# AAPPHH/image_recommender

Hardware: AMD Instinct MI355X
Metric: k-NN queries/sec + recall@10 on 1M concat vectors at 1/2/4/8 MI355X (higher is better)
Workload: dtype bf16 candidates (fp32 accumulate) + fp32 rerank, certified exact; 1 GPU; cfg3: 1M x 1968 concat(color48|sift128|dreamsim1792), cosine ranking; rows=1000000, dim=1968, k=10, queries_per_batch=1024, rows_per_gpu=1000000, parallelism=row-shard x1 + RCCL all-gather merge, queries_per_gpu=1024, tile_rows=256, tile_queries=256, row_splits=64, workgroups=256

## Files before the change

### image_recommender_amd/_lib.py

```python
from __future__ import annotations

import ctypes as C
import os
import threading
from pathlib import Path

LIB_PATH = Path(__file__).resolve().parent / "lib" / os.environ.get("IMGREC_LIB_NAME", "libimgrec.so")

KNN_OK, KNN_EINVAL, KNN_EHIP, KNN_ENOMEM, KNN_EIO, KNN_ENOSYS = 0, -1, -2, -3, -4, -5
KNN_METRIC_IP, KNN_METRIC_L2, KNN_METRIC_COSINE = 0, 1, 2
KNN_MAX_K = 32
KNN_MAX_K_LARGE = 1024
KNN_SEARCH_AUTO, KNN_SEARCH_EXACT, KNN_SEARCH_SPLIT, KNN_SEARCH_BF16, KNN_SEARCH_I8 = 0, 1, 2, 3, 4
KNN_FENCE_EAGER, KNN_FENCE_LAZY = 0, 1
COLOR_HIST_MAX_BINS = 32
INGEST_NOT_FAST, INGEST_TOO_SMALL = -1, -2
KMEANS_SPHERICAL = 1
KMEANS_STATS_PER_ITER = 8
VLAD_RAW = 1
VLAD_MAX_NN = 8
VLAD_MAX_D = 16384
VLADENC_MODEL_OUTPUT = 1
VLADENC_MAX_LAYERS = 8
VLADENC_MAX_WIDTH = 4096
VLADENC_MAX_IN = 1 << 20
VLADENC_CHUNK_ROWS = 128
VLADENC_SUPER_ROWS = 2048
VLADTRAIN_MAX_BATCH = 4096
VLADTRAIN_MAX_BATCH_FLOATS = 1 << 28
VLADTRAIN_PARAMS, VLADTRAIN_ADAM_M, VLADTRAIN_ADAM_V, VLADTRAIN_GRADS = 0, 1, 2, 3


class KmeansParams(C.Structure):
    _fields_ = [("niter", C.c_int), ("nredo", C.c_int), ("spherical", C.c_int), ("verbose", C.c_int),
                ("seed", C.c_int64), ("device", C.c_int)]

class VladTrainConfig(C.Structure):
    _fields_ = [("dropout", C.c_double), ("lr", C.c_double), ("beta1", C.c_double), ("beta2", C.c_double),
                ("adam_eps", C.c_double), ("weight_decay", C.c_double), ("corr_weight", C.c_double),
                ("umap_weight", C.c_double), ("temperature", C.c_double), ("ln_eps", C.c_double),
                ("seed", C.c_uint64)]


_vp, _i, _i64, _f, _d = C.c_void_p, C.c_int, C.c_int64, C.c_float, C.c_double
_pi64, _pf, _pi, _pd = C.POINTER(C.c_int64), C.POINTER(C.c_float), C.POINTER(C.c_int), C.POINTER(C.c_double)
SIGNATURES = {
    "knn_create": (_i, [_i, _i, _i, C.POINTER(_vp)]),
    "knn_create_multi": (_i, [_i, _i, _pi, _i, C.POINTER(_vp)]),
    "knn_num_shards": (_i, [_vp]),
    "knn_free": (_i, [_vp]),
    "knn_dim": (_i, [_vp]),
    "knn_metric": (_i, [_vp]),
    "knn_ntotal": (_i64, [_vp]),
    "knn_is_trained": (_i, [_vp]),
    "knn_set_id_offset": (_i, [_vp, _i64]),
    "knn_train": (_i, [_vp, _vp, _i64]),
    "knn_add": (_i, [_vp, _vp, _i64]),
    "knn_add_device": (_i, [_vp, _vp, _i64, _vp]),
    "knn_reserve": (_i, [_vp, _i64]),
    "knn_reset": (_i, [_vp]),
    "knn_remove_ids": (_i, [_vp, _vp, _i64, _pi64]),
    "knn_reconstruct_n": (_i, [_vp, _i64, _i64, _vp]),
    "knn_search": (_i, [_vp, _vp, _i64, _i, _vp, _vp]),
    "knn_search_device": (_i, [_vp, _vp, _i64, _i, _vp, _vp, _vp]),
    "knn_search_filtered": (_i, [_vp, _vp, _i64, _i, _vp, _i64, _vp, _vp]),
    "knn_search_filtered_device": (_i, [_vp, _vp, _i64, _i, _vp, _i64, _vp, _vp, _vp]),
    "knn_range_search": (_i, [_vp, _vp, _i64, _f, C.POINTER(_vp)]),
    "knn_range_search_device": (_i, [_vp, _vp, _i64, _f, _vp, C.POINTER(_vp)]),
    "knn_range_nq": (_i64, [_vp]),
    "knn_range_size": (_i64, [_vp]),
    "knn_range_copy": (_i, [_vp, _vp, _vp, _vp]),
    "knn_range_device": (_i, [_vp, C.POINTER(_vp), C.POINTER(_vp), C.POINTER(_vp)]),
    "knn_range_free": (_i, [_vp]),
    "knn_merge_device": (_i, [_vp, _vp, _i, _i64, _i, _i, _i, _vp, _vp, _vp]),
    "knn_packed_bytes": (_i64, [_i64, _i]),
    "knn_merge_packed_device": (_i, [_vp, _i, _i64, _i, _i, _i, _vp, _vp, _vp]),
    "ivfpq_lut_device": (_i, [_vp, _i64, _i, _i, _i, _vp, _vp, _vp]),
    "ivfpq_scan_device": (_i, [_vp, _vp, _i64, _i, _vp, _vp, _vp, _i, _i, _i, _vp, _vp, _vp]),
    "ivfpq_scan_all_device": (_i, [_vp, _vp, _i64, _i, _vp, _vp, _vp, _i, _i, _vp, _vp, _i64, _i, _vp,
                                   _vp, _vp]),
    "knn_write": (_i, [_vp, C.c_char_p]),
    "knn_read": (_i, [C.c_char_p, _i, C.POINTER(_vp)]),
    "knn_read_multi": (_i, [C.c_char_p, _pi, _i, C.POINTER(_vp)]),
    "knn_normalize_L2": (_i, [_vp, _i64, _i]),
    "knn_set_timing": (_i, [_vp, _i]),
    "knn_set_fence_mode": (_i, [_vp, _i]),
    "knn_kernel_time": (_i, [_vp, _pd, _pi]),
    "knn_plan": (_i, [_vp, _i64, _i, _pi, _pi, _pi, _pi]),
    "knn_plan_kernel": (_i, [_vp, _i64, _i, C.c_char_p, _i]),
    "knn_set_search_mode": (_i, [_vp, _i]),
    "knn_search_stats": (_i, [_vp, _pi64, _pi64, _pf]),
    "knn_search_stats2": (_i, [_vp, _pi64, _pi64, _pi64, _pf]),
    "knn_last_path": (_i, [_vp]),
    "knn_debug_i8tail": (_i, [_vp, _pi, _pi, _i64, _i64, _vp, _vp, _vp]),
    "knn_large_k_fallbacks": (_i, [_vp, C.POINTER(_i64)]),
    "knn_last_error": (C.c_char_p, []),
    "knn_version": (C.c_char_p, []),
    "kmeans_step_device": (_i, [_vp, _i64, _i, _vp, _i, _i, _vp, _vp, _vp, _vp, _vp, _vp]),
    "kmeans_split_device": (_i, [_vp, _i, _i, _vp, _pi, _vp]),
    "kmeans_train": (_i, [_vp, _i64, _i, _i, _vp, _vp, _vp, _pd, _vp]),
    "kmeans_train_device": (_i, [_vp, _i64, _i, _i, _vp, _vp, _vp, _pd, _vp, _vp]),
    "vlad_encode_device": (_i, [_vp, _i64, _vp, _i64, _i, _vp, _i, _i, _f, _i, _vp, _vp, _vp, _vp]),
    "vlad_encode": (_i, [_vp, _i64, _vp, _i64, _i, _vp, _i, _i, _f, _i, _vp, _vp, _vp, _i]),
    "vladenc_create": (_i, [_i, _pi, C.POINTER(_vp), C.POINTER(_vp), C.POINTER(_vp), C.POINTER(_vp), _f, _i,
                            C.POINTER(_vp)]),
    "vladenc_free": (_i, [_vp]),
    "vladenc_widths": (_i, [_vp, _pi, _pi]),
    "vladenc_forward_device": (_i, [_vp, _vp, _i64, _i, _vp, _vp, _vp]),
    "vladenc_forward": (_i, [_vp, _vp, _i64, _i, _vp, _vp]),
    "vladtrain_default_config": (_i, [C.POINTER(VladTrainConfig)]),
    "vladtrain_create": (_i, [_i, _pi, C.POINTER(_vp), C.POINTER(_vp), C.POINTER(_vp), C.POINTER(_vp),
                              C.POINTER(VladTrainConfig), _i, C.POINTER(_vp)]),
    "vladtrain_free": (_i, [_vp]),
    "vladtrain_step_device": (_i, [_vp, _vp, _i64, _vp, _i64, _vp, _vp]),
    "vladtrain_step": (_i, [_vp, _vp, _i64, _vp, _i64, _vp]),
    "vladtrain_grads_device": (_i, [_vp, _vp, _i64, _vp, _i64, _vp, _vp, _vp, _vp]),
    "vladtrain_grads": (_i, [_vp, _vp, _i64, _vp, _i64, _vp, _vp, _vp]),
    "vladtrain_eval_device": (_i, [_vp, _vp, _i64, _vp, _i64, _vp, _vp]),
    "vladtrain_eval": (_i, [_vp, _vp, _i64, _vp, _i64, _vp]),
    "vladtrain_get_state": (_i, [_vp, _i, C.POINTER(_vp), C.POINTER(_vp), C.POINTER(_vp), C.POINTER(_vp)]),
    "vladtrain_set_state": (_i, [_vp, _i, C.POINTER(_vp), C.POINTER(_vp), C.POINTER(_vp), C.POINTER(_vp)]),
    "vladtrain_get_step": (_i, [_vp, _pi64]),
    "vladtrain_set_step": (_i, [_vp, _i64]),
    "vladtrain_product_device": (_i, [_vp, _i64, _vp, _i64, _i64, _vp, _vp]),
    "vladtrain_workspace_bytes": (_i64, [_i, _pi, _i64]),
    "color_hist_device": (_i, [_vp, _vp, _vp, _i64, _i, _vp, _vp, _vp]),
    "color_hist_host": (_i, [_vp, _i64, _vp, _vp, _i64, _i, _i, _vp, _vp]),
    "color_hist_last_error": (C.c_char_p, []),
    "color_host_register": (_i, [_vp, _i64]),
    "color_host_unregister": (_i, [_vp]),
    "vit_add_layernorm_bf16": (_i, [_vp, _vp, _vp, _vp, _vp, _i64, _i, C.c_float, _vp]),
    "vit_quick_gelu_bf16": (_i, [_vp, _i64, _vp]),
    "vit_gelu_bf16": (_i, [_vp, _i64, _vp]),
    "vit_patchify_bf16": (_i, [_vp, _i64, _i, _i, _i, _vp, _vp, _vp, _vp]),
    "vit_tokens_f32": (_i, [_vp, _vp, _vp, _i64, _i, _i, _vp, _vp]),
    "vit_attention_bf16": (_i, [_vp, _i64, _i, _i, _i, C.c_float, _vp, _vp]),
    "vit_linear_bf16": (_i, [_vp, _vp, _vp, _i64, _i, _i, _i, _vp, _vp]),
    "vit_linear_bf16_split": (_i, [_vp, _vp, _vp, _i64, _i, _i, _i, _i, _vp, _vp]),
    "vit_linear_splits": (_i, [_i64, _i]),
    "color_hist_batch_async": (_i, [_vp, _i64, _vp, _i64, _i, _vp, _vp, _vp, _vp, _vp]),
    "ingest_parse_f32": (_i64, [_vp, _i64, _vp, _i64]),
    "ingest_concat_rows": (_i64, [C.POINTER(_vp), _pi64, _i64, _i, _pi64, _vp, _vp]),
    "ingest_concat_packed": (_i64, [_vp, _vp, _vp, _i64, _i, _vp, _vp, _vp]),
    "ingest_scan_open": (_i, [C.c_char_p, C.c_char_p, _i, _pi64, C.POINTER(_vp)]),
    "ingest_scan_next": (_i64, [_vp, _i64, _vp, _vp, _vp]),
    "ingest_scan_close": (_i, [_vp]),
    "ingest_scan_error": (C.c_char_p, []),
}


class NativeLibraryError(RuntimeError):
    """libimgrec.so is missing or failed to load — the HIP path is mandatory."""


class KnnError(RuntimeError):
    """A C-ABI call returned an error code (the message is knn_last_error())."""


_lock = threading.Lock()
_lib = None


def load() -> C.CDLL:
    global _lib
    if _lib is not None:
        return _lib
    with _lock:
        if _lib is not None:
            return _lib
        if not LIB_PATH.exists():
            raise NativeLibraryError(
                f"{LIB_PATH} not found: build it with `python -m image_recommender_amd.build` "
                "(hipcc --offload-arch=gfx950); there is no CPU fallback")
        if os.environ.get("IMGREC_NO_TORCH_PRELOAD") != "1":
            try:
                import torch
            except Exception:
                pass
        try:
            lib = C.CDLL(str(LIB_PATH), mode=C.RTLD_GLOBAL)
        except OSError as e:
            raise NativeLibraryError(f"cannot load {LIB_PATH}: {e}") from e
        for name, (res, args) in SIGNATURES.items():
            fn = getattr(lib, name)
            fn.restype = res
            fn.argtypes = args
        _lib = lib
        return lib


def last_error() -> str:
    msg = load().knn_last_error()
    return msg.decode() if msg else ""


def check(rc: int, what: str) -> int:
    if rc < 0:
        raise KnnError(f"{what} failed (code {rc}): {last_error()}")
    return rc
```

### image_recommender_amd/csrc/knn_b16w.hip

```cpp

#include <hip/hip_runtime.h>
#include <stdint.h>
#include <math.h>

#include <type_traits>

#include "knn_kernels.h"
#include "lds_dma.h"
#include "wave_ops.h"

namespace imgrec {
namespace {

typedef float f32x4 __attribute__((ext_vector_type(4)));
typedef __bf16 bf16x8 __attribute__((ext_vector_type(8)));
typedef unsigned u32x4 __attribute__((ext_vector_type(4)));
typedef float f32x2 __attribute__((ext_vector_type(2)));
typedef int i32x4 __attribute__((ext_vector_type(4)));

constexpr int kNW = 8;
constexpr int kBM = kB16BigRows;
constexpr int kBQ = kB16BigQueries;
constexpr int kQW = kBQ / kNW;
constexpr int kRB = kBM / 16;
constexpr int kBKW = 32;
constexpr int kNS = 2;
constexpr int kRowB = kBKW * 4;
constexpr int kCPR = kBKW / 4;
constexpr int kRPP = 64 / kCPR;
constexpr int kRPB = 64 / kBKW;
constexpr int kGPT = kBM / kRPP;
constexpr int kSA = kBM * kRowB;
constexpr int kSB = kBQ * kRowB;
constexpr int kStage = kSA + kSB;
constexpr int kLPW = (kBM + kBQ) / kRPP / kNW;
constexpr int kNormSlots = 4;
constexpr int kNormOff = kNS * kStage;
constexpr int kRecOff = kNormOff + kNormSlots * kBM * 4;
constexpr int kLuOff = kRecOff + kNW * kQW * kSBWords * 4;
constexpr int kLDS = kLuOff + kBQ * 2 * 4;
static_assert(kQW * kSBWords * 4 == 2048 && kSBWords == 16, "a wave's records: one dma2_agent of 2 KiB");
static_assert(kLDS == 153600, "LDS image");
constexpr int kScaleOff = kLDS;
constexpr int kQScaleOff = kScaleOff + kNormSlots * kBM * 4;
constexpr int kQNormOff = kQScaleOff + kBQ * 4;
constexpr int kLDST = kQNormOff + kBQ * 4;
static_assert(kLDST <= 160 * 1024, "LDS budget (int8 tail)");
constexpr int kQuads = 8;
#ifndef IMGREC_B16W_DEFER_Q
#define IMGREC_B16W_DEFER_Q 3
#endif
constexpr int kDeferQ = IMGREC_B16W_DEFER_Q;
static_assert(kBKW == 32 && kCPR == 8, "stage depth: two 32-deep k-steps per stage");
static_assert(kLDS <= 160 * 1024, "LDS budget");
static_assert(kLPW % 4 == 0, "pieces go out in dma4x groups of four");
static_assert(kDeferQ >= 0 && kDeferQ < kQuads - 1, "deferred DMA inside the stage's first quads");
#ifndef IMGREC_B16W_EPI_EXP
#define IMGREC_B16W_EPI_EXP 0
#endif

template <int K>
__device__ __forceinline__ void insert_mono(float (&kd)[K], int (&ki)[K], float d, int id) {
    bool c[K];
#pragma unroll
    for (int p = 0; p < K; ++p) c[p] = d < kd[p];
#pragma unroll
    for (int p = K - 1; p > 0; --p) {
        kd[p] = __builtin_amdgcn_fmed3f(kd[p - 1], d, kd[p]);
        const int nx = __builtin_unpredictable(c[p]) ? id : ki[p];
        ki[p] = __builtin_unpredictable(c[p - 1]) ? ki[p - 1] : nx;
    }
    kd[0] = __builtin_unpredictable(c[0]) ? d : kd[0];
    ki[0] = __builtin_unpredictable(c[0]) ? id : ki[0];
}

__device__ __forceinline__ bool rank_lt(float d1, int i1, float d2, int i2) {
    return i2 < 0 || d1 < d2 || (d1 == d2 && i1 < i2);
}

template <int K>
__device__ __forceinline__ void insert_any(float (&kd)[K], int (&ki)[K], float d, int id) {
#pragma unroll
    for (int p = K - 1; p > 0; --p) {
        const bool shift = rank_lt(d, id, kd[p - 1], ki[p - 1]);
        const bool here = !shift && rank_lt(d, id, kd[p], ki[p]);
        kd[p] = shift ? kd[p - 1] : (here ? d : kd[p]);
        ki[p] = shift ? ki[p - 1] : (here ? id : ki[p]);
    }
    const bool here0 = rank_lt(d, id, kd[0], ki[0]);
    kd[0] = here0 ? d : kd[0];
    ki[0] = here0 ? id : ki[0];
}

__device__ __forceinline__ float quarter_min(float x) {
    const auto r = __builtin_amdgcn_permlane16_swap(__float_as_uint(x), __float_as_uint(x), false, false);
    x = fminf(__uint_as_float(r[0]), __uint_as_float(r[1]));
    const auto s = __builtin_amdgcn_permlane32_swap(__float_as_uint(x), __float_as_uint(x), false, false);
    return fminf(__uint_as_float(s[0]), __uint_as_float(s[1]));
}
__device__ __forceinline__ float quarter_max(float x) {
    const auto r = __builtin_amdgcn_permlane16_swap(__float_as_uint(x), __float_as_uint(x), false, false);
    x = fmaxf(__uint_as_float(r[0]), __uint_as_float(r[1]));
    const auto s = __builtin_amdgcn_permlane32_swap(__float_as_uint(x), __float_as_uint(x), false, false);
    return fmaxf(__uint_as_float(s[0]), __uint_as_float(s[1]));
}

__device__ __forceinline__ uint32_t quarter_min_u(uint32_t x) {
    const auto r = __builtin_amdgcn_permlane16_swap(x, x, false, false);
    x = min(r[0], r[1]);
    const auto s = __builtin_amdgcn_permlane32_swap(x, x, false, false);
    return min(s[0], s[1]);
}
__device__ __forceinline__ uint32_t quarter_max_u(uint32_t x) {
    const auto r = __builtin_amdgcn_permlane16_swap(x, x, false, false);
    x = max(r[0], r[1]);
    const auto s = __builtin_amdgcn_permlane32_swap(x, x, false, false);
    return max(s[0], s[1]);
}

__device__ __forceinline__ uint32_t ord_bits(float k) {
    const uint32_t u = __float_as_uint(k);
    return (u & 0x80000000u) ? ~u : (u | 0x80000000u);
}
__device__ __forceinline__ float ord_float(uint32_t u) {
    return __uint_as_float((u & 0x80000000u) ? (u & 0x7fffffffu) : ~u);
}
__device__ __forceinline__ float sel8(int r, float x0, float x1, float x2, float x3, float x4, float x5,
                                      float x6, float x7) {
    const bool b0 = r & 1, b1 = r & 2, b2 = r & 4;
    const float a0 = b0 ? x1 : x0, a1 = b0 ? x3 : x2, a2 = b0 ? x5 : x4, a3 = b0 ? x7 : x6;
    const float c0 = b1 ? a1 : a0, c1 = b1 ? a3 : a2;
    return b2 ? c1 : c0;
}
__device__ __forceinline__ uint32_t umed3(uint32_t a, uint32_t b, uint32_t c) {
    return max(min(a, b), min(max(a, b), c));
}
template <int K>
__device__ __forceinline__ void insert_packed(uint32_t (&kp)[K], uint32_t u) {
#pragma unroll
    for (int p = K - 1; p > 0; --p) kp[p] = umed3(kp[p - 1], u, kp[p]);
    kp[0] = min(kp[0], u);
}
__device__ __forceinline__ float bucket_end(uint32_t u, uint32_t lowmask) {
    return u == ~0u ? INFINITY : ord_float((u | lowmask) + 1u);
}

}

#ifdef IMGREC_B16_STAMPS
__device__ unsigned long long g_b16w_stamps[8 * 256];
__device__ unsigned long long g_b16w_wg[2 * 1024];
#define B16W_STAMP(slot) do { if (stamp_on && lane == 0) { \
    unsigned long long v_ = __builtin_amdgcn_s_memtime(); g_b16w_stamps[wave * 256 + (slot)] = v_; } } while (0)
#else
#define B16W_STAMP(slot) do {} while (0)
#endif

struct I8TailArgs {
    const uint32_t* xt = nullptr;
    const float* xts = nullptr;
    const uint32_t* qt = nullptr;
    const float* qts = nullptr;
    int dwt = 0, nst_t = 0, nst_h = 0;
};

template <int KM, int L2, bool PACK>
__global__ void __launch_bounds__(512, 2)
knn_b16w_tile_kernel(const uint32_t* __restrict__ xh, const float* __restrict__ xnorm, int nrows,
                     int dw, const uint32_t* __restrict__ qh, const float* __restrict__ qnorm, int nq,
                     int nsplit, int nqb, int64_t id_offset, float* __restrict__ cand_d,
                     int64_t* __restrict__ cand_i, int ncand, int ib, uint32_t* sbound) {
    __shared__ __attribute__((aligned(16))) char smem[kLDS];
#define B16W_I8T 0
#include "knn_b16w_body.inc"
#undef B16W_I8T
}

template <int KM, int L2, bool PACK>
__global__ void __launch_bounds__(512, 2)
knn_b16w_tile_kernel_i8t(const uint32_t* __restrict__ xh, const float* __restrict__ xnorm, int nrows,
                         int dw, const uint32_t* __restrict__ qh, const float* __restrict__ qnorm, int nq,
                         int nsplit, int nqb, int64_t id_offset, float* __restrict__ cand_d,
                         int64_t* __restrict__ cand_i, int ncand, int ib, uint32_t* sbound,
                         const I8TailArgs ta) {
    __shared__ __attribute__((aligned(16))) char smem[kLDST];
#define B16W_I8T 1
    constexpr bool I8T = true;
#include "knn_b16w_body.inc"
#undef B16W_I8T
}

hipError_t launch_b16_big(const TileArgs& a, hipStream_t st) {
    if (a.wr != 2 || a.wq != 4 || a.dp % kBKW != 0 || a.nsplit < 1) return hipErrorInvalidValue;
    const auto off_ok = [&](int64_t row_bytes) {
        return ((int64_t)(kGPT - 1) * a.nsplit * kRPP + kBQ) * row_bytes + 8192 < ((int64_t)1 << 32);
    };
    if (!off_ok((int64_t)a.dp * 4)) return hipErrorInvalidValue;
    const bool i8t = a.xt != nullptr;
    I8TailArgs ta;
    if (i8t) {
        if (a.t_head < 0 || a.t_head % 64 != 0 || a.t_head > 2 * a.dp || a.t_dpt < 128 || a.t_dpt % 128 != 0 ||
            !a.xts || !a.qt || !a.qts || !off_ok(a.t_dpt))
            return hipErrorInvalidValue;
        ta.xt = reinterpret_cast<const uint32_t*>(a.xt);
        ta.xts = a.xts;
        ta.qt = reinterpret_cast<const uint32_t*>(a.qt);
        ta.qts = a.qts;
        ta.dwt = a.t_dpt / 4;
        ta.nst_t = a.t_dpt / 128;
        ta.nst_h = a.t_head / 64;
    }
    const dim3 grid((unsigned)(a.nqb * a.nsplit)), block(kNW * 64);
    const uint32_t* xh = reinterpret_cast<const uint32_t*>(a.xb);
    const uint32_t* qh = reinterpret_cast<const uint32_t*>(a.qp);
    if (a.ib < 0 || a.ib > kB16PackMaxIB) return hipErrorInvalidValue;
#define IMGREC_LAUNCH_B16W(KMV, L2V, PK)                                                             \
    do {                                                                                             \
        if (i8t)                                                                                     \
            hipLaunchKernelGGL((knn_b16w_tile_kernel_i8t<KMV, L2V, PK>), grid, block, 0, st, xh,    \
                               a.xnorm, a.nrows, a.dp, qh, a.qnorm, a.nq, a.nsplit, a.nqb,           \
                               a.id_offset, a.cand_d, a.cand_i, a.ncand, a.ib, a.sbound, ta);        \
        else                                                                                         \
            hipLaunchKernelGGL((knn_b16w_tile_kernel<KMV, L2V, PK>), grid, block, 0, st, xh,        \
                               a.xnorm, a.nrows, a.dp, qh, a.qnorm, a.nq, a.nsplit, a.nqb,           \
                               a.id_offset, a.cand_d, a.cand_i, a.ncand, a.ib, a.sbound);            \
    } while (0)
#define IMGREC_LAUNCH_B16W_K(KMV, PK)                                                               \
    do { if (a.metric == 1) IMGREC_LAUNCH_B16W(KMV, 1, PK); else IMGREC_LAUNCH_B16W(KMV, 0, PK); } while (0)
    if (a.km == 8) {
        if (a.ib > 0) IMGREC_LAUNCH_B16W_K(8, true); else IMGREC_LAUNCH_B16W_K(8, false);
    } else if (a.km == 10) {
        if (a.ib > 0) IMGREC_LAUNCH_B16W_K(10, true); else IMGREC_LAUNCH_B16W_K(10, false);
    } else {
        return hipErrorInvalidValue;
    }
#undef IMGREC_LAUNCH_B16W_K
#undef IMGREC_LAUNCH_B16W
    return hipGetLastError();
}

}


#ifdef IMGREC_B16_STAMPS
extern "C" int knn_b16w_stamps_read(unsigned long long* host) {
    return (int)hipMemcpyFromSymbol(host, HIP_SYMBOL(imgrec::g_b16w_stamps), sizeof(imgrec::g_b16w_stamps));
}
extern "C" int knn_b16w_wg_read(unsigned long long* host) {
    return (int)hipMemcpyFromSymbol(host, HIP_SYMBOL(imgrec::g_b16w_wg), sizeof(imgrec::g_b16w_wg));
}
#endif
```

### image_recommender_amd/csrc/knn_b16w_body.inc

```
#if B16W_I8T
#else

#endif
#ifdef IMGREC_B16_STAMPS
    const int wg = blockIdx.x;
    if (threadIdx.x == 0 && wg < 1024) g_b16w_wg[2 * wg] = __builtin_amdgcn_s_memrealtime();
#endif
    const int wgid = xcd_wgid();
    constexpr int kG = 4;
    const int G = (nqb % kG == 0) ? kG : nqb;
    const int qbg = wgid / (nsplit * G), rem = wgid - qbg * (nsplit * G);
    const int split = rem / G;
    const int qb = qbg * G + rem % G;
    const int ngroups = (nrows + kRPP - 1) / kRPP;
    const int cnt = split < ngroups ? (ngroups - split + nsplit - 1) / nsplit : 0;
    const int t0 = 0, t1 = (cnt + kGPT - 1) / kGPT;
    auto trow = [&](int t, int tr) {
        const int m = t * kGPT + tr / kRPP;
        return (split + (m < cnt ? m : t * kGPT) * nsplit) * kRPP + tr % kRPP;
    };

    const int lane = threadIdx.x & 63;
    const int wave = __builtin_amdgcn_readfirstlane(threadIdx.x >> 6);
    const int lc = lane & 15, lq = lane >> 4;
    int qcol[2];
    qcol[0] = qb * kBQ + wave * kQW + lc;
    qcol[1] = qcol[0] + 16;
#if B16W_I8T
    auto qcol_of = [&](int h) __attribute__((always_inline)) {
        if constexpr (!I8T) return qcol[h];
        int l = lc;
        asm volatile("" : "+v"(l));
        return qb * kBQ + wave * kQW + l + 16 * h;
    };
#endif
    float qn[2] = {0.f, 0.f};
#if B16W_I8T
    if constexpr (!I8T) {
        if (L2) { qn[0] = qnorm[qcol[0]]; qn[1] = qnorm[qcol[1]]; }
        asm volatile("" : "+v"(qn[0]), "+v"(qn[1]));
    }
    float* const lsq = reinterpret_cast<float*>(smem + (I8T ? kQScaleOff : 0)) + wave * kQW;
    float* const lqn = reinterpret_cast<float*>(smem + (I8T ? kQNormOff : 0)) + wave * kQW;
    if constexpr (I8T)
        if (lane < kQW) {
            lsq[lane] = ta.qts[qb * kBQ + wave * kQW + lane];
            lqn[lane] = L2 ? qnorm[qb * kBQ + wave * kQW + lane] : 0.f;
        }
#else
    if (L2) { qn[0] = qnorm[qcol[0]]; qn[1] = qnorm[qcol[1]]; }
    asm volatile("" : "+v"(qn[0]), "+v"(qn[1]));
#endif

    const bool isA = wave < 4;
    if (!isA) __builtin_amdgcn_s_setprio(1);
    const int pbase = (isA ? wave : wave - 4) * kLPW;
    const int prow = lane / kCPR, pchk = lane % kCPR;
    static_assert(kRPP == 8 && kRPB == 2 && kLPW % 2 == 0, "piece offset form");
#if B16W_I8T
    auto vpar_of = [&](int e, int words) {
        int ln = lane;
        asm volatile("" : "+v"(ln));
        const int prow = ln / kCPR, pchk = ln % kCPR;
#else
    uint32_t vpar[2];
#pragma unroll
    for (int e = 0; e < 2; ++e) {
#endif
        const int P = pbase + e, r = P * kRPP + prow;
        const int srow = isA ? P * nsplit * kRPP + prow : r;
#if B16W_I8T
        return (uint32_t)srow * (uint32_t)(words * 4) + 16u * (uint32_t)(pchk ^ ((r / kRPB) % kCPR));
    };
    uint32_t vpar[2] = {0u, 0u};
    if constexpr (!I8T) { vpar[0] = vpar_of(0, dw); vpar[1] = vpar_of(1, dw); }
#else
        vpar[e] = (uint32_t)srow * (uint32_t)(dw * 4) + 16u * (uint32_t)(pchk ^ ((r / kRPB) % kCPR));
    }
#endif
    const uint32_t kPS = (uint32_t)((isA ? nsplit : 1) * kRPP * dw * 4);
    auto voff_of = [&](int j) {
        return vpar[j & 1] + (uint32_t)(j & ~1) * kPS - 1024u * (uint32_t)(j & 3);
    };
    const uint32_t smem0 = lds_u32(smem);
    const uint32_t pdst = (uint32_t)((isA ? 0 : kSA) + pbase * 1024);

    const int fsw = (lc / kRPB) % kCPR;
    int aoff[2];
#pragma unroll
    for (int c = 0; c < 2; ++c) aoff[c] = lc * kRowB + 16 * ((4 * c + lq) ^ fsw);
    const int boff = kSA + wave * kQW * kRowB;

    float kd[2][KM];
    int ki[2][KM];
    uint32_t kp[2][KM];
    const uint32_t lowm = PACK ? (1u << ib) - 1u : 0u;
#pragma unroll
    for (int h = 0; h < 2; ++h)
#pragma unroll
        for (int p = 0; p < KM; ++p) {
            if constexpr (PACK) kp[h][p] = ~0u;
            else { kd[h][p] = INFINITY; ki[h][p] = -1; }
        }

    const bool sb_on = sbound != nullptr;
    uint32_t* const wrec = sbound + (size_t)(qb * kBQ + wave * kQW) * kSBWords;
    const uint32_t* const lrec = reinterpret_cast<const uint32_t*>(smem + kRecOff) + wave * (kQW * kSBWords);
    uint2* const lst = reinterpret_cast<uint2*>(smem + kLuOff) + wave * kQW;
    if (sb_on && lq == 0) {
        lst[lc] = make_uint2(__float_as_uint(INFINITY), ~0u);
        lst[lc + 16] = make_uint2(__float_as_uint(INFINITY), ~0u);
    }
    auto rec_dma = [&]() __attribute__((always_inline)) {
        dma2_agent(wrec, smem0 + (uint32_t)(kRecOff + wave * (kQW * kSBWords * 4)), (uint32_t)lane * 16u);
    };

#if B16W_I8T
    const int nst_t = I8T ? ta.nst_t : 0;
    const int nst = I8T ? ta.nst_t + ta.nst_h : dw / kBKW;
#else
    const int nst = dw / kBKW;
#endif
    const int total = (t1 - t0) * nst;
    const uint32_t* qblk = qh + (size_t)qb * kBQ * dw;
#if B16W_I8T
    const uint32_t* qblk_t = I8T ? ta.qt + (size_t)qb * kBQ * ta.dwt : nullptr;
#endif

    int c_it = t0, c_is = 0;
    const uint32_t* c_tile = isA ? xh + (size_t)trow(t0, 0) * dw : qblk;
#if B16W_I8T
    const uint32_t* c_tile_t = !I8T ? nullptr : isA ? ta.xt + (size_t)trow(t0, 0) * ta.dwt : qblk_t;
#endif
    int c_ng = (isA && t0 == t1 - 1) ? cnt - t0 * kGPT : kGPT;
    auto issue = [&](int g) __attribute__((always_inline)) {
#if B16W_I8T
        const bool tl = I8T && c_is < nst_t;
        const uint32_t* src;
        uint32_t vp0 = 0u, vp1 = 0u, ps = 0u;
        if constexpr (I8T) {
            const int rw = tl ? ta.dwt : dw;
            src = tl ? c_tile_t + c_is * kBKW : c_tile + (c_is - nst_t) * kBKW;
            vp0 = vpar_of(0, rw);
            vp1 = vpar_of(1, rw);
            ps = (uint32_t)((isA ? nsplit : 1) * kRPP * rw * 4);
        } else {
            src = c_tile + c_is * kBKW;
        }
        auto voff = [&](int j) {
            if constexpr (I8T) return ((j & 1) ? vp1 : vp0) + (uint32_t)(j & ~1) * ps - 1024u * (uint32_t)(j & 3);
            else return voff_of(j);
        };
#else
        const uint32_t* src = c_tile + c_is * kBKW;
#endif
        const uint32_t dst = smem0 + (uint32_t)((g & (kNS - 1)) * kStage) + pdst;
        if (pbase + kLPW <= c_ng || !isA) {
#pragma unroll
            for (int h = 0; h < kLPW / 4; ++h)
#if B16W_I8T
                dma4x(src, dst + 4096u * h, voff(4 * h), voff(4 * h + 1), voff(4 * h + 2),
                      voff(4 * h + 3));
#else
                dma4x(src, dst + 4096u * h, voff_of(4 * h), voff_of(4 * h + 1), voff_of(4 * h + 2),
                      voff_of(4 * h + 3));
#endif
        } else {
#pragma unroll
            for (int j = 0; j < kLPW; ++j)
                if (pbase + j < c_ng) {
                    const uint32_t d = dst + 4096u * (j / 4);
                    switch (j & 3) {
#if B16W_I8T
                        case 0: dma1<0>(src, d, voff(j)); break;
                        case 1: dma1<1024>(src, d, voff(j)); break;
                        case 2: dma1<2048>(src, d, voff(j)); break;
                        default: dma1<3072>(src, d, voff(j)); break;
#else
                        case 0: dma1<0>(src, d, voff_of(j)); break;
                        case 1: dma1<1024>(src, d, voff_of(j)); break;
                        case 2: dma1<2048>(src, d, voff_of(j)); break;
                        default: dma1<3072>(src, d, voff_of(j)); break;
#endif
                    }
                }
        }
        if (c_is == 0 && wave < 4)
            dma4_norm(xnorm + trow(c_it, wave * 64 + lane),
                      smem0 + (uint32_t)(kNormOff + ((c_it - t0) & (kNormSlots - 1)) * kBM * 4 + wave * 256));
#if B16W_I8T
        if constexpr (I8T)
            if (c_is == 0 && wave < 4)
                dma4_norm(ta.xts + trow(c_it, wave * 64 + lane),
                          smem0 + (uint32_t)(kScaleOff + ((c_it - t0) & (kNormSlots - 1)) * kBM * 4 + wave * 256));
#endif
        if (++c_is == nst) {
            c_is = 0;
            ++c_it;
            if (isA) {
                c_tile = xh + (size_t)trow(c_it, 0) * dw;
#if B16W_I8T
                if constexpr (I8T) c_tile_t = ta.xt + (size_t)trow(c_it, 0) * ta.dwt;
#endif
                c_ng = c_it == t1 - 1 ? cnt - c_it * kGPT : kGPT;
            }
        }
    };
    static_assert(kNS == 2 && kNormSlots == 4, "power-of-two ring slots");

    constexpr int kJ = (KM + 3) / 4;
    constexpr float kLo = 1.0f / 1048576.f;

    auto read_a = [&](const char* sb, int q, u32x4 (&fa)[4]) __attribute__((always_inline)) {
#pragma unroll
        for (int j = 0; j < 4; ++j)
            fa[j] = *reinterpret_cast<const u32x4*>(sb + aoff[q >> 2] + (4 * (q & 3) + j) * 16 * kRowB);
    };
    auto read_b = [&](const char* sb, int c, u32x4 (&fb)[2]) __attribute__((always_inline)) {
#pragma unroll
        for (int h = 0; h < 2; ++h) fb[h] = *reinterpret_cast<const u32x4*>(sb + aoff[c] + boff + h * 16 * kRowB);
    };
#if B16W_I8T
    auto mfma_quad = [&](auto tl_tag, f32x4 (&acc)[kRB][2], const u32x4 (&fa)[4], const u32x4 (&fb)[2], int q) __attribute__((always_inline)) {
#else
    auto mfma_quad = [&](f32x4 (&acc)[kRB][2], const u32x4 (&fa)[4], const u32x4 (&fb)[2], int q) __attribute__((always_inline)) {
#endif
#pragma unroll
        for (int j = 0; j < 4; ++j)
#pragma unroll
#if B16W_I8T
            for (int h = 0; h < 2; ++h) {
                if constexpr (decltype(tl_tag)::value)
                    acc[4 * (q & 3) + j][h] = __builtin_bit_cast(f32x4, __builtin_amdgcn_mfma_i32_16x16x64_i8(
                        __builtin_bit_cast(i32x4, fa[j]), __builtin_bit_cast(i32x4, fb[h]),
                        __builtin_bit_cast(i32x4, acc[4 * (q & 3) + j][h]), 0, 0, 0));
                else
                    acc[4 * (q & 3) + j][h] = __builtin_amdgcn_mfma_f32_16x16x32_bf16(
                        __builtin_bit_cast(bf16x8, fa[j]), __builtin_bit_cast(bf16x8, fb[h]), acc[4 * (q & 3) + j][h], 0, 0, 0);
            }
#else
            for (int h = 0; h < 2; ++h)
                acc[4 * (q & 3) + j][h] = __builtin_amdgcn_mfma_f32_16x16x32_bf16(
                    __builtin_bit_cast(bf16x8, fa[j]), __builtin_bit_cast(bf16x8, fb[h]), acc[4 * (q & 3) + j][h], 0, 0, 0);
#endif
    };

    u32x4 fa[2][4], fb[2][2];
    int g = 0;
    int pend = -1;
    if (total > 0) {
        issue(0);
        asm volatile("s_waitcnt vmcnt(0)" ::: "memory");
        barrier_lds();
        if (total > 1) issue(1);
        read_a(smem, 0, fa[0]);
        read_b(smem, 0, fb[0]);
    }
    for (int t = t0; t < t1; ++t) {
#ifdef IMGREC_B16_STAMPS
        const bool stamp_on = blockIdx.x == 100 && t - t0 < 120;
        int nit = 0;
        unsigned long long ins_cyc = 0;
#endif
        f32x4 acc[kRB][2];
#pragma unroll
        for (int rb = 0; rb < kRB; ++rb)
#pragma unroll
            for (int h = 0; h < 2; ++h) acc[rb][h] = (f32x4){0.f, 0.f, 0.f, 0.f};
        const bool rec_due = sb_on && (t - t0 < 4 || ((t - t0) & 3) == 0);
        const int nlive = (t + 1) * kGPT <= cnt ? 4 : (((cnt - t * kGPT) * kRPP + 63) >> 6);
#if B16W_I8T
        auto stage_loop = [&](auto nr_tag, auto tl_tag, int ns, int s0, bool more) __attribute__((always_inline)) {
#else
        auto stage_loop = [&](auto nr_tag) __attribute__((always_inline)) {
#endif
            constexpr int NR = decltype(nr_tag)::value, L = 2 * NR;
#if B16W_I8T
            for (int s = 0; s < ns; ++s, ++g) {
#else
            for (int s = 0; s < nst; ++s, ++g) {
#endif
                const char* sb = smem + (g & 1) * kStage;
#pragma unroll
                for (int i = 0; i + 1 < L; ++i) {
                    read_a(sb, 4 * ((i + 1) / NR) + (i + 1) % NR, fa[(i + 1) & 1]);
                    if (i == NR - 1) read_b(sb, 1, fb[1]);
#if B16W_I8T
                    mfma_quad(tl_tag, acc, fa[i & 1], fb[i / NR], 4 * (i / NR) + i % NR);
#else
                    mfma_quad(acc, fa[i & 1], fb[i / NR], 4 * (i / NR) + i % NR);
#endif
#pragma unroll
                    for (int j = 0; j < 4; ++j) {
                        __builtin_amdgcn_sched_group_barrier(0x008, 1, 0);
                        __builtin_amdgcn_sched_group_barrier(0x100, 1, 0);
                    }
                    if (i == NR - 1) {
                        __builtin_amdgcn_sched_group_barrier(0x008, 1, 0);
                        __builtin_amdgcn_sched_group_barrier(0x100, 1, 0);
                        __builtin_amdgcn_sched_group_barrier(0x008, 1, 0);
                        __builtin_amdgcn_sched_group_barrier(0x100, 1, 0);
                        __builtin_amdgcn_sched_group_barrier(0x008, 2, 0);
                    } else {
                        __builtin_amdgcn_sched_group_barrier(0x008, 4, 0);
                    }
                    __builtin_amdgcn_sched_barrier(0);
                    if (i == (kDeferQ < L - 2 ? kDeferQ : L - 2) && pend >= 0) {
                        __builtin_amdgcn_sched_barrier(0);
                        issue(pend);
                        pend = -1;
                        __builtin_amdgcn_sched_barrier(0);
                    }
                }
                __builtin_amdgcn_sched_barrier(0);
                asm volatile("s_waitcnt vmcnt(0) lgkmcnt(0)" ::: "memory");
                __builtin_amdgcn_sched_barrier(0);
                barrier_lds();
                __builtin_amdgcn_sched_barrier(0);
#if B16W_I8T
                if (s + 1 < ns || more) {
#else
                if (s + 1 < nst) {
#endif
                    const char* nb = smem + ((g + 1) & 1) * kStage;
                    read_a(nb, 0, fa[0]);
                    read_b(nb, 0, fb[0]);
                }
                if (g + 2 < total) {
                    if (isA) issue(g + 2);
                    else pend = g + 2;
                }
#if B16W_I8T
                if (rec_due && s0 + s + 2 == nst) rec_dma();
                mfma_quad(tl_tag, acc, fa[1], fb[1], 4 + NR - 1);
            }
        };
        auto tile_stages = [&](auto nr_tag) __attribute__((always_inline)) {
            if constexpr (I8T) {
                constexpr int NR = decltype(nr_tag)::value;
                stage_loop(nr_tag, std::true_type{}, nst_t, 0, nst > nst_t);
                const float* scl = reinterpret_cast<const float*>(smem + kScaleOff + ((t - t0) % kNormSlots) * kBM * 4);
                const float sq[2] = {lsq[lc], lsq[lc + 16]};
#pragma unroll
                for (int rb = 0; rb < (IMGREC_B16W_EPI_EXP == 3 ? 0 : 4 * NR); ++rb) {
                    const float4 s4 = *reinterpret_cast<const float4*>(scl + rb * 16 + 4 * lq);
                    const float sr[4] = {s4.x, s4.y, s4.z, s4.w};
#pragma unroll
                    for (int h = 0; h < 2; ++h) {
                        const i32x4 ai = __builtin_bit_cast(i32x4, acc[rb][h]);
#pragma unroll
                        for (int i = 0; i < 4; ++i) acc[rb][h][i] = (float)ai[i] * sr[i] * sq[h];
                    }
                    asm volatile("" : "+v"(acc[rb][0]), "+v"(acc[rb][1]));
                }
                stage_loop(nr_tag, std::false_type{}, nst - nst_t, nst_t, false);
            } else {
                stage_loop(nr_tag, std::false_type{}, nst, 0, false);
#else
                if (rec_due && s + 2 == nst) rec_dma();
                mfma_quad(acc, fa[1], fb[1], 4 + NR - 1);
#endif
            }
        };
        if (rec_due && nst < 2) rec_dma();
#if B16W_I8T
        if (nlive >= 4) tile_stages(std::integral_constant<int, 4>{});
        else if (nlive == 3) tile_stages(std::integral_constant<int, 3>{});
        else if (nlive == 2) tile_stages(std::integral_constant<int, 2>{});
        else tile_stages(std::integral_constant<int, 1>{});
#else
        if (nlive >= 4) stage_loop(std::integral_constant<int, 4>{});
        else if (nlive == 3) stage_loop(std::integral_constant<int, 3>{});
        else if (nlive == 2) stage_loop(std::integral_constant<int, 2>{});
        else stage_loop(std::integral_constant<int, 1>{});
#endif

        B16W_STAMP(2 * (t - t0));
#if IMGREC_B16W_EPI_EXP != 0
#pragma unroll
        for (int rb = 0; rb < kRB; ++rb)
#pragma unroll
            for (int h = 0; h < 2; ++h) asm volatile("" :: "v"(acc[rb][h]));
#endif
        const float* nrm = reinterpret_cast<const float*>(smem + kNormOff + ((t - t0) % kNormSlots) * kBM * 4);
        const bool full = (t + 1) * kGPT <= cnt && trow(t, kBM - 1) < nrows;
        auto row_ok = [&](int tr) { return t * kGPT + tr / kRPP < cnt && trow(t, tr) < nrows; };
#if B16W_I8T
        if constexpr (I8T && L2 != 0) { qn[0] = lqn[lc]; qn[1] = lqn[lc + 16]; }
#endif
        float lu[2] = {INFINITY, INFINITY};
        if (sb_on) {
#pragma unroll
            for (int h = 0; h < 2; ++h) {
                const uint4 c = *reinterpret_cast<const uint4*>(lrec + (lc + 16 * h) * kSBWords + 4 * lq);
                const uint32_t ub = quarter_max_u(lq < 3 ? max(max(c.x, c.y), max(c.z, c.w)) : 0u);
                const float cA = __uint_as_float(quarter_max_u(lq == 3 ? c.x : 0u));
                const float cB = __uint_as_float(quarter_max_u(lq == 3 ? c.y : 0u));
                const float U = ord_float(ub);
                const float L = ub >= 0xff800000u ? INFINITY : U + fmaf(cB, fabsf(U), cA);
                lu[h] = fminf(__uint_as_float(lst[lc + 16 * h].x), L);
            }
        }
        float cth[2];
        auto screen = [&]() __attribute__((always_inline)) {
#pragma unroll
            for (int h = 0; h < 2; ++h) {
                float T;
                if constexpr (PACK) T = bucket_end(min(quarter_min_u(kp[h][KM - 1]), quarter_max_u(kp[h][kJ - 1])), lowm);
                else T = fminf(quarter_min(kd[h][KM - 1]), quarter_max(kd[h][kJ - 1]));
                T = fminf(T, lu[h]);
                const float c = L2 ? 0.5f * (qn[h] - T) - kLo * (qn[h] + fabsf(T)) : -T;
#if B16W_I8T
                cth[h] = qcol_of(h) < nq ? c : INFINITY;
#else
                cth[h] = qcol[h] < nq ? c : INFINITY;
#endif
            }
        };
#pragma unroll
        for (int rg = 0; rg < 4; ++rg) {
            if (rg >= nlive || IMGREC_B16W_EPI_EXP == 1) break;
            screen();
            unsigned live = 0xffffu;
            if (!full) {
                live = 0;
#if B16W_I8T
                int lq_c = lq;
                asm volatile("" : "+v"(lq_c));
#pragma unroll
                for (int b = 0; b < 16; ++b) live |= (unsigned)row_ok((4 * rg + (b >> 2)) * 16 + 4 * lq_c + (b & 3)) << b;
#else
#pragma unroll
                for (int b = 0; b < 16; ++b) live |= (unsigned)row_ok((4 * rg + (b >> 2)) * 16 + 4 * lq + (b & 3)) << b;
#endif
            }
            unsigned msk[2] = {0u, 0u};
            float4 nr4[4];
#pragma unroll
            for (int j = 3; j >= 0; --j) {
                const int rb = 4 * rg + j;
                float4 n4 = make_float4(0.f, 0.f, 0.f, 0.f);
                if (L2) n4 = *reinterpret_cast<const float4*>(nrm + rb * 16 + 4 * lq);
                nr4[j] = n4;
                const f32x2 half2 = (f32x2){0.5f - kLo, 0.5f - kLo};
                const f32x2 hlo = (f32x2){n4.x, n4.y} * half2, hhi = (f32x2){n4.z, n4.w} * half2;
#pragma unroll
                for (int h = 0; h < 2; ++h) {
                    const f32x2 c2 = (f32x2){cth[h], cth[h]};
                    const f32x2 dhi = (L2 ? hhi + c2 : c2) - (f32x2){acc[rb][h][2], acc[rb][h][3]};
                    const f32x2 dlo = (L2 ? hlo + c2 : c2) - (f32x2){acc[rb][h][0], acc[rb][h][1]};
                    msk[h] = __builtin_amdgcn_alignbit(msk[h], __float_as_uint(dhi.y), 31);
                    msk[h] = __builtin_amdgcn_alignbit(msk[h], __float_as_uint(dhi.x), 31);
                    msk[h] = __builtin_amdgcn_alignbit(msk[h], __float_as_uint(dlo.y), 31);
                    msk[h] = __builtin_amdgcn_alignbit(msk[h], __float_as_uint(dlo.x), 31);
                }
            }
#ifdef IMGREC_B16_STAMPS
            const unsigned long long ins0 = __builtin_amdgcn_s_memtime();
#endif
#if IMGREC_B16W_EPI_EXP == 2
            asm volatile("" :: "v"(msk[0] & live), "v"(msk[1] & live));
            continue;
#endif
#pragma unroll
            for (int h = 0; h < 2; ++h) {
                const unsigned m = msk[h] & live;
                if (!__any(m != 0)) continue;
#pragma unroll
                for (int hf = 0; hf < 2; ++hf) {
                    unsigned mh = (m >> (8 * hf)) & 0xffu;
                    if (!__any(mh != 0)) continue;
                    const int rb0 = 4 * rg + 2 * hf;
                    while (__any(mh != 0)) {
#ifdef IMGREC_B16_STAMPS
                        ++nit;
#endif
                        const bool act = mh != 0u;
                        const int r8 = act ? __builtin_ctz(mh) : 0;
                        mh &= mh - 1u;
                        const int tr = (rb0 + (r8 >> 2)) * 16 + 4 * lq + (r8 & 3);
                        const float a = sel8(r8, acc[rb0][h][0], acc[rb0][h][1], acc[rb0][h][2], acc[rb0][h][3],
                                             acc[rb0 + 1][h][0], acc[rb0 + 1][h][1], acc[rb0 + 1][h][2],
                                             acc[rb0 + 1][h][3]);
                        const float4 na = nr4[2 * hf], nb = nr4[2 * hf + 1];
                        const float xn = L2 ? sel8(r8, na.x, na.y, na.z, na.w, nb.x, nb.y, nb.z, nb.w) : 0.f;
                        float kv = L2 ? fmaf(-2.f, a, qn[h] + xn) : -a;
                        if constexpr (PACK) {
                            const uint32_t ob = L2 ? ((uint32_t)max((int)__float_as_uint(kv), 0) | 0x80000000u)
                                                   : ord_bits(kv);
                            const uint32_t u = (ob & ~lowm) | (uint32_t)(t * kBM + tr);
                            insert_packed<KM>(kp[h], __builtin_unpredictable(act) ? u : ~0u);
                        } else {
                            if (L2) kv = kv < 0.f ? 0.f : kv;
                            kv = __builtin_unpredictable(act && kv < kd[h][KM - 1]) ? kv : INFINITY;
                            insert_mono<KM>(kd[h], ki[h], kv, trow(t, tr));
                        }
                    }
                }
            }
#ifdef IMGREC_B16_STAMPS
            ins_cyc += __builtin_amdgcn_s_memtime() - ins0;
#endif
        }
        if (sb_on) {
#pragma unroll
            for (int h = 0; h < 2; ++h) {
                const uint32_t best = quarter_min_u(PACK ? kp[h][0] : ord_bits(kd[h][0]));
                uint32_t pubd = lst[lc + 16 * h].y;
                const uint32_t pub = PACK ? (best | lowm) + 1u : best;
                if (lq == 0) {
#if B16W_I8T
                    const int qc = qcol_of(h);
                    if (qc < nq && pub != 0u && pub < 0xff800000u && pub < pubd) {
                        __hip_atomic_fetch_min(sbound + (size_t)qc * kSBWords + split % KM, pub,
#else
                    if (qcol[h] < nq && pub != 0u && pub < 0xff800000u && pub < pubd) {
                        __hip_atomic_fetch_min(sbound + (size_t)qcol[h] * kSBWords + split % KM, pub,
#endif
                                               __ATOMIC_RELAXED, __HIP_MEMORY_SCOPE_AGENT);
                        pubd = pub;
                    }
                    lst[lc + 16 * h] = make_uint2(__float_as_uint(lu[h]), pubd);
                }
            }
        }
        B16W_STAMP(2 * (t - t0) + 1);
#ifdef IMGREC_B16_STAMPS
        if (stamp_on && lane == 0) g_b16w_stamps[wave * 256 + 128 + (t - t0)] = (unsigned long long)nit;
        if (stamp_on && lane == 0 && t - t0 < 64) g_b16w_stamps[wave * 256 + 192 + (t - t0)] = ins_cyc;
#endif
        if (g < total) {
            read_a(smem + (g & 1) * kStage, 0, fa[0]);
            read_b(smem + (g & 1) * kStage, 0, fb[0]);
        }
    }

#ifdef IMGREC_B16_STAMPS
    if (threadIdx.x == 0 && wg < 1024) g_b16w_wg[2 * wg + 1] = __builtin_amdgcn_s_memrealtime();
#endif
#pragma unroll
    for (int x = 32; x >= 16; x >>= 1) {
#pragma unroll
        for (int h = 0; h < 2; ++h) {
            if constexpr (PACK) {
                uint32_t o[KM];
#pragma unroll
                for (int p = 0; p < KM; ++p) o[p] = (uint32_t)__shfl_xor((int)kp[h][p], x, 64);
#pragma unroll
                for (int p = 0; p < KM; ++p) insert_packed<KM>(kp[h], o[p]);
                continue;
            }
#pragma unroll
            for (int p = 0; p < KM; ++p) {
                const float od = __shfl_xor(kd[h][p], x, 64);
                const int oi = __shfl_xor(ki[h][p], x, 64);
                if (lq < x / 16 && oi >= 0 && rank_lt(od, oi, kd[h][KM - 1], ki[h][KM - 1]))
                    insert_any<KM>(kd[h], ki[h], od, oi);
            }
        }
    }
    if (lq != 0) return;
    const float lu[2] = {sb_on ? __uint_as_float(lst[lc].x) : INFINITY, sb_on ? __uint_as_float(lst[lc + 16].x) : INFINITY};
#pragma unroll
    for (int h = 0; h < 2; ++h) {
#if B16W_I8T
        const int qc = qcol_of(h);
        if (qc >= nq) continue;
#else
        if (qcol[h] >= nq) continue;
#endif
        if (sb_on && lu[h] != INFINITY)
#if B16W_I8T
            __hip_atomic_fetch_min(sbound + (size_t)qc * kSBWords + kSBFloor, ord_bits(lu[h]),
#else
            __hip_atomic_fetch_min(sbound + (size_t)qcol[h] * kSBWords + kSBFloor, ord_bits(lu[h]),
#endif
                                   __ATOMIC_RELAXED, __HIP_MEMORY_SCOPE_AGENT);
#if B16W_I8T
        const size_t base = (size_t)qc * ncand + (size_t)split * KM;
#else
        const size_t base = (size_t)qcol[h] * ncand + (size_t)split * KM;
#endif
#pragma unroll
        for (int p = 0; p < KM; ++p) {
            if constexpr (PACK) {
                const uint32_t u = kp[h][p];
                const int j = (int)(u & lowm);
                cand_d[base + p] = u == ~0u ? INFINITY : ord_float(u & ~lowm);
                cand_i[base + p] = u == ~0u ? (int64_t)-1
                                            : (int64_t)((split + (j >> 3) * nsplit) * kRPP + (j & 7)) + id_offset;
            } else {
                cand_d[base + p] = kd[h][p];
                cand_i[base + p] = ki[h][p] < 0 ? (int64_t)-1 : (int64_t)ki[h][p] + id_offset;
            }
        }
    }
```

### image_recommender_amd/csrc/knn_capi.cpp

```cpp

#include <cstdarg>
#include <cstdio>
#include <cstdlib>
#include <cstring>
#include <mutex>
#include <string>

#include "knn_index.h"
#include "knn_multi.h"

namespace imgrec {

namespace {
thread_local std::string g_err;
}

const char* test_knob(const char* name) {
    const char* e = std::getenv(name);
    if (e && *e) {
        static std::mutex mu;
        static std::string seen;
        std::lock_guard<std::mutex> lk(mu);
        const std::string tag = std::string("|") + name + "|";
        if (seen.find(tag) == std::string::npos) {
            seen += tag;
            std::fprintf(stderr, "[imgrec] %s=%s overrides a launch default (test / A-B knob, "
                                 "INTEGRATION.md)\n", name, e);
        }
    }
    return e && *e ? e : nullptr;
}

void set_err(const char* fmt, ...) {
    char buf[512];
    va_list ap;
    va_start(ap, fmt);
    vsnprintf(buf, sizeof(buf), fmt, ap);
    va_end(ap);
    g_err = buf;
}

const char* last_error() { return g_err.c_str(); }

int corpus_columns(knn_index* ix, Column<DeviceSpace>* cols, bool all) {
    int n = 0;
    cols[n++] = {&ix->xb, (size_t)ix->dp * sizeof(float)};
    cols[n++] = {&ix->xn, sizeof(float)};
    if (all || ix->xs) cols[n++] = {&ix->xs, (size_t)ix->dp * sizeof(uint32_t)};
    if (all || ix->b16_ok) cols[n++] = {&ix->xh, (size_t)ix->dpb * sizeof(uint16_t)};
    if (all || ix->b16_ok) cols[n++] = {&ix->xr, sizeof(float)};
    if (all || ix->x8) cols[n++] = {&ix->x8, (size_t)i8_row_bytes(ix->nblk8)};
    if (all || ix->x8) cols[n++] = {&ix->x8s, (size_t)ix->nblk8 * sizeof(float)};
    if (all || ix->x8) cols[n++] = {&ix->x8r, sizeof(float)};
    if (all || ix->xt) cols[n++] = {&ix->xt, (size_t)ix->xt_dpt};
    if (all || ix->xt) cols[n++] = {&ix->xts, sizeof(float)};
    if (all || ix->xt) cols[n++] = {&ix->xtm, sizeof(float4)};
    return n;
}

int reserve_rows(knn_index* ix, int64_t need, hipStream_t st) {
    if (need <= ix->cap) return KNN_OK;
    const int64_t ncap = round_up(std::max(need, ix->cap + ix->cap / 2), kTileRowsMax);
    Column<DeviceSpace> live[kCorpusColumns];
    const int n_all = corpus_columns(ix, live);
    const int n_tail = ix->xt ? 3 : 0, n = n_all - n_tail;
    const size_t old = (size_t)ix->ntotal;
    hipError_t e = hipSuccess;
    const Column<DeviceSpace>* grp = live;
    auto fill_rows = [&](int i, void* dst, const void* src) {
        const size_t row = grp[i].stride;
        if (old && src) e = hipMemcpyAsync(dst, src, old * row, hipMemcpyDeviceToDevice, st);
        if (e == hipSuccess) e = hipMemsetAsync((char*)dst + old * row, 0, ((size_t)ncap - old) * row, st);
        return e == hipSuccess ? KNN_OK : KNN_EHIP;
    };
    auto wait_rows = [&]() {
        const hipError_t es = hipStreamSynchronize(st);
        if (e == hipSuccess) e = es;
        return e == hipSuccess ? KNN_OK : KNN_EHIP;
    };
    const int rc = regrow_columns(live, n, (size_t)ncap, fill_rows, wait_rows);
    if (rc != KNN_OK && e == hipSuccess) {
        (void)hipGetLastError();
        KNN_FAIL(KNN_ENOMEM, "hipMalloc of the %lld-row corpus buffers failed", (long long)ncap);
    }
    if (rc != KNN_OK) KNN_FAIL(KNN_EHIP, "corpus regrowth failed: %s", hipGetErrorString(e));
    ix->cap = ncap;
    if (n_tail > 0) {
        grp = live + n;
        if (regrow_columns(grp, n_tail, (size_t)ncap, fill_rows, wait_rows) != KNN_OK) {
            (void)hipGetLastError();
            drop_i8tail(ix, TailCopy::Undecided);
        }
    }
    return KNN_OK;
}

static int materialise_columns(knn_index* ix, int c0, int n) {
    Column<DeviceSpace> all[kCorpusColumns];
    corpus_columns(ix, all, true);
    const int rc = regrow_columns(all + c0, n, (size_t)std::max<int64_t>(ix->cap, 1),
                                  [](int, void*, const void*) { return KNN_OK; }, []() { return KNN_OK; });
    if (rc != KNN_OK) (void)hipGetLastError();
    return rc;
}

int add_device_locked(knn_index* ix, const float* x, int64_t n, hipStream_t st) {
    if ((int64_t)(ix->ntotal + n) > (int64_t)INT32_MAX)
        KNN_FAIL(KNN_EINVAL, "a single index shard holds at most 2^31-1 rows");
    int rc = reserve_rows(ix, ix->ntotal + n, st);
    if (rc != KNN_OK) return rc;
    Column<DeviceSpace> c[kCorpusColumns];
    corpus_columns(ix, c, true);
    auto at = [&](int col) { return (char*)c[col].buf->data() + (size_t)ix->ntotal * c[col].stride; };
    float* const xb = (float*)at(kColXb);
    KNN_HIP(launch_rows_ingest(x, n, ix->d, ix->dp, n, ix->metric == KNN_METRIC_COSINE ? 1 : 0, xb,
                               (float*)at(kColXn), st));
    if (ix->xs) KNN_HIP(launch_split_rows(xb, n, ix->dp, kSplitBK, (uint32_t*)at(kColXs), st));
    if (ix->b16_ok)
        KNN_HIP(launch_bf16_rows(xb, n, ix->dp, ix->dpb, (uint16_t*)at(kColXh), (float*)at(kColXr), st));
    if (ix->x8)
        KNN_HIP(launch_i8_rows(xb, n, ix->dp, ix->nblk8, (int8_t*)at(kColX8), (float*)at(kColX8s),
                               (float*)at(kColX8r), st));
    if (ix->xt) {
        KNN_HIP(launch_i8tail_rows(xb, n, ix->dp, ix->dpb, ix->xt_head, ix->xt_dpt, (int8_t*)at(kColXt),
                                   (float*)at(kColXts), (float4*)at(kColXtm), st));
        ix->xt_tried = false;
    }
    ix->ntotal += n;
    ix->xn_max_stale = true;
    return KNN_OK;
}

int ensure_split(knn_index* ix, hipStream_t st) {
    if (ix->xs) return KNN_OK;
    if (!ix->split_ok) KNN_FAIL(KNN_EINVAL, "split search needs d >= 256; d = %d", ix->d);
    if (materialise_columns(ix, kColXs, 1) != KNN_OK)
        KNN_FAIL(KNN_ENOMEM, "hipMalloc of the %lld-row split copy failed", (long long)ix->cap);
    if (ix->ntotal > 0)
        KNN_HIP(launch_split_rows(ix->xb, ix->ntotal, ix->dp, kSplitBK, ix->xs, st));
    return KNN_OK;
}

int ensure_i8(knn_index* ix, hipStream_t st) {
    if (ix->x8) return KNN_OK;
    if (ix->nblk8 <= 0) KNN_FAIL(KNN_EINVAL, "int8 search needs 64 <= d <= 4096; d = %d", ix->d);
    if (materialise_columns(ix, kColX8, 3) != KNN_OK)
        KNN_FAIL(KNN_ENOMEM, "hipMalloc of the %lld-row int8 copy failed", (long long)ix->cap);
    ix->xn_max_stale = true;
    if (ix->ntotal > 0)
        KNN_HIP(launch_i8_rows(ix->xb, ix->ntotal, ix->dp, ix->nblk8, ix->x8, ix->x8s, ix->x8r, st));
    return KNN_OK;
}

int ensure_i8tail(knn_index* ix, hipStream_t st) {
    if (ix->xt_state != TailCopy::Undecided) return KNN_OK;
    if (ix->ntotal <= 0 || !ix->b16_ok || ix->dpb > 4096) { ix->xt_state = TailCopy::Ineligible; return KNN_OK; }
    const int nblk = ix->dpb / kB16Pad;
    DevBuf<float> dmax;
    int rc;
    if ((rc = dmax.reserve((size_t)nblk)) != KNN_OK) return rc;
    std::vector<float> hmax((size_t)nblk);
    KNN_HIP(launch_block_absmax(ix->xb, ix->ntotal, ix->dp, nblk, dmax, st));
    KNN_HIP(hipMemcpyAsync(hmax.data(), dmax, (size_t)nblk * sizeof(float), hipMemcpyDeviceToHost, st));
    KNN_HIP(hipStreamSynchronize(st));
    const int head = i8t_pick_head(hmax.data(), nblk);
    if (head < 0) { ix->xt_state = TailCopy::Ineligible; return KNN_OK; }
    ix->xt_head = head;
    ix->xt_dpt = (int)round_up(ix->dpb - head, 128);
    if (materialise_columns(ix, kColXt, 3) != KNN_OK) {
        drop_i8tail(ix, TailCopy::Ineligible);
        return KNN_OK;
    }
    KNN_HIP(hipMemsetAsync(ix->xt, 0, (size_t)ix->cap * ix->xt_dpt, st));
    KNN_HIP(hipMemsetAsync(ix->xts, 0, (size_t)ix->cap * sizeof(float), st));
    KNN_HIP(hipMemsetAsync(ix->xtm, 0, (size_t)ix->cap * sizeof(float4), st));
    ix->xn_max_stale = true;
    KNN_HIP(launch_i8tail_rows(ix->xb, ix->ntotal, ix->dp, ix->dpb, head, ix->xt_dpt, ix->xt, ix->xts,
                               ix->xtm, st));
    ix->xt_state = TailCopy::Built;
    return KNN_OK;
}

void drop_i8tail(knn_index* ix, TailCopy next) {
    ix->xt.reset(); ix->xts.reset(); ix->xtm.reset();
    ix->xt_head = ix->xt_dpt = 0;
    ix->xt_tried = false; ix->xt_state = next;
}

int create_single(int d, int metric, int device, knn_index** out) {
    *out = nullptr;
    int ndev = 0;
    if (hipGetDeviceCount(&ndev) != hipSuccess || ndev <= 0)
        KNN_FAIL(KNN_ENOSYS, "no HIP device visible");
    if (device < 0) KNN_HIP(hipGetDevice(&device));
    if (device >= ndev) KNN_FAIL(KNN_EINVAL, "device %d out of range (%d visible)", device, ndev);
    DeviceGuard g(device);
    knn_index* ix = new knn_index();
    ix->d = d;
    ix->dp = (int)round_up(d, d >= 256 ? 2 * kDepthPad : kDepthPad);
    ix->metric = metric;
    ix->device = device;
    ix->split_ok = ix->dp % 32 == 0 && d >= 256;
    ix->b16_ok = d >= 64;
    ix->dpb = (int)round_up(d, kB16Pad);
    ix->nblk8 = d >= 64 && d <= 4096 ? (d + 63) / 64 : 0;
    int cus = 0;
    if (hipDeviceGetAttribute(&cus, hipDeviceAttributeMultiprocessorCount, device) == hipSuccess &&
        cus > 0)
        ix->cus = cus;
    if (const char* e = test_knob("IMGREC_CUS")) {
        const int v = std::atoi(e);
        if (v > 0 && v < ix->cus) ix->cus = v;
    }
    if (const char* e = test_knob("IMGREC_I8_WGPCU")) {
        const int v = std::atoi(e);
        if (v > 0 && v <= 16) ix->i8_wgpcu = v;
    }
    if (const char* e = test_knob("IMGREC_MERGE_FUSE")) {
        ix->merge_fuse = *e != '0';
        ix->merge_fuse1 = *e != '0' && *e != '1';
    }
    if (const char* e = test_knob("IMGREC_CHANCE_SKIP")) ix->chance_skip = *e != '0';
    if (const char* e = test_knob("IMGREC_CHANCE_DIRECT")) ix->chance_direct_max = std::max(0, std::atoi(e));
    if (const char* e = test_knob("IMGREC_I8_HALF_K")) {
        const int v = std::atoi(e);
        ix->i8_half_k = v >= 2 ? v : 0;
    }
    if (const char* e = test_knob("IMGREC_I8_POOL")) {
        ix->i8_pool64 = std::min(64, std::max(0, std::atoi(e)));
        ix->i8_pool_forced = true;
    }
    if (const char* e = test_knob("IMGREC_I8_POOL_CH")) ix->i8_pool_ch = std::min(64, std::max(1, std::atoi(e)));
    if (const char* e = test_knob("IMGREC_DIRECT_RAW")) ix->direct_raw = std::min(2, std::max(0, std::atoi(e)));
    if (const char* e = test_knob("IMGREC_I8_FUSED_PREP")) ix->i8_fused_prep = *e != '0';
    if (const char* e = test_knob("IMGREC_RERANK_P1")) ix->rerank_p1k = *e != '0';
    if (const char* e = test_knob("IMGREC_RERANK_NW4")) ix->rerank_nw4 = *e != '0';
    if (const char* e = test_knob("IMGREC_MERGE_SINGLE")) ix->merge_single = *e != '0';
    if (const char* e = test_knob("IMGREC_STREAM_LISTS")) ix->stream_lists = *e != '0';
    if (const char* e = test_knob("IMGREC_B16W_SHARED_BOUND")) ix->shared_bound = *e != '0';
    if (const char* e = test_knob("IMGREC_B16W_I8TAIL")) {
        ix->i8tail = *e != '0';
        ix->xt_no_trial = *e == '2';
    }
    if (const char* e = test_knob("IMGREC_RANGE_CAP")) {
        const long long v = std::atoll(e);
        if (v > 0) ix->range_cap0 = (size_t)v;
    }
    if (const char* e = test_knob("IMGREC_REMOVE_CHUNK")) {
        const long long v = std::atoll(e);
        if (v > 0) ix->remove_chunk = (int64_t)v;
    }
    if (hipStreamCreateWithFlags(&ix->stream, hipStreamNonBlocking) != hipSuccess ||
        ix->fence.create() != KNN_OK) {
        if (ix->stream) (void)hipStreamDestroy(ix->stream);
        delete ix;
        KNN_FAIL(KNN_EHIP, "hipStreamCreate / hipEventCreate failed");
    }
    *out = ix;
    return KNN_OK;
}

void free_single(knn_index* ix) {
    DeviceGuard g(ix->device);
    (void)hipDeviceSynchronize();
    for (hipEvent_t e : ix->ev) (void)hipEventDestroy(e);
    (void)hipStreamDestroy(ix->stream);
    delete ix;
}

constexpr size_t kPinnedSearchBytes = 1 << 20;

int stage_queries(knn_index* ix, const float* q, int64_t nq, int k, bool pinned) {
    int rc;
    const size_t nqd = (size_t)nq * ix->d, nk = (size_t)nq * k;
    if ((rc = ix->hq.reserve(nqd)) != KNN_OK) return rc;
    if (k > 0 && (rc = ix->hd.reserve(nk)) != KNN_OK) return rc;
    if (k > 0 && (rc = ix->hi.reserve(nk)) != KNN_OK) return rc;
    if (pinned) {
        if ((rc = ix->pq.reserve(nqd)) != KNN_OK) return rc;
        if ((rc = ix->pd.reserve(nk)) != KNN_OK) return rc;
        if ((rc = ix->pi.reserve(nk)) != KNN_OK) return rc;
        std::memcpy(ix->pq, q, nqd * sizeof(float));
    }
    KNN_HIP(hipMemcpyAsync(ix->hq, pinned ? ix->pq : q, nqd * sizeof(float), hipMemcpyHostToDevice, ix->stream));
    return KNN_OK;
}

int stage_bitmap(knn_index* ix, const uint8_t* bitmap, int64_t* nbits) {
    *nbits = std::min(*nbits, ix->ntotal);
    const size_t nbytes = (size_t)((*nbits + 7) / 8);
    const int rc = ix->ft_bits.reserve(std::max<size_t>(nbytes, 1));
    if (rc != KNN_OK) return rc;
    if (nbytes) KNN_HIP(hipMemcpyAsync(ix->ft_bits, bitmap, nbytes, hipMemcpyHostToDevice, ix->stream));
    return KNN_OK;
}

int fetch_results(knn_index* ix, int64_t nq, int k, float* D, int64_t* I) {
    const size_t nk = (size_t)nq * k;
    KNN_HIP(hipMemcpyAsync(D, ix->hd, nk * sizeof(float), hipMemcpyDeviceToHost, ix->stream));
    KNN_HIP(hipMemcpyAsync(I, ix->hi, nk * sizeof(int64_t), hipMemcpyDeviceToHost, ix->stream));
    return KNN_OK;
}

int set_metric(knn_index* ix, int metric) {
    if (ix->multi) return multi_set_metric(ix, metric);
    ix->metric = metric;
    return KNN_OK;
}

int set_trained(knn_index* ix, bool trained) {
    ix->trained = trained;
    if (ix->multi) return multi_set_trained(ix, trained);
    return KNN_OK;
}

}

using namespace imgrec;

extern "C" {

const char* knn_last_error(void) { return imgrec::last_error(); }
const char* knn_version(void) {
    return "imgrec-knn 0.2 (gfx950: bf16 / split-bf16 / f32 MFMA candidates, fused top-k, "
           "device-side certificate)";
}

int knn_create(int d, int metric, int device, knn_index_t** out) {
    if (!out) KNN_FAIL(KNN_EINVAL, "out is NULL");
    *out = nullptr;
    if (d <= 0) KNN_FAIL(KNN_EINVAL, "d must be positive (got %d)", d);
    if (metric != KNN_METRIC_L2 && metric != KNN_METRIC_IP && metric != KNN_METRIC_COSINE)
        KNN_FAIL(KNN_EINVAL, "unknown metric %d", metric);
    return create_single(d, metric, device, out);
}

int knn_free(knn_index_t* ix) {
    if (!ix) return KNN_OK;
    if (ix->multi) return multi_free(ix);
    free_single(ix);
    return KNN_OK;
}

int knn_dim(const knn_index_t* ix) { return ix ? ix->d : KNN_EINVAL; }
int knn_metric(const knn_index_t* ix) { return ix ? ix->metric : KNN_EINVAL; }
int64_t knn_ntotal(const knn_index_t* ix) { return ix ? ix->ntotal : KNN_EINVAL; }
int knn_is_trained(const knn_index_t* ix) { return ix ? (ix->trained ? 1 : 0) : KNN_EINVAL; }

int knn_set_id_offset(knn_index_t* ix, int64_t off) {
    if (!ix) KNN_FAIL(KNN_EINVAL, "index is NULL");
    std::lock_guard<std::mutex> lk(ix->mu);
    ix->id_offset = off;
    return KNN_OK;
}

int knn_train(knn_index_t* ix, const float* x, int64_t n) {
    (void)x;
    if (!ix) KNN_FAIL(KNN_EINVAL, "index is NULL");
    if (n < 0) KNN_FAIL(KNN_EINVAL, "n must be >= 0");
    return set_trained(ix, true);
}

int knn_reserve(knn_index_t* ix, int64_t n) {
    if (!ix) KNN_FAIL(KNN_EINVAL, "index is NULL");
    if (ix->multi) return multi_reserve(ix, n);
    IndexOp op(ix);
    int rc = op.begin(ix->stream);
    if (rc == KNN_OK) rc = reserve_rows(ix, n, ix->stream);
    return op.finish(rc);
}

static int add_args_ok(knn_index_t* ix, const float* x, int64_t n) {
    if (!ix) KNN_FAIL(KNN_EINVAL, "index is NULL");
    if (n < 0 || (n > 0 && !x)) KNN_FAIL(KNN_EINVAL, "bad rows (n=%lld)", (long long)n);
    return KNN_OK;
}

int knn_add_device(knn_index_t* ix, const float* x, int64_t n, void* stream) {
    int rc;
    if ((rc = add_args_ok(ix, x, n)) != KNN_OK || n == 0) return rc;
    if (ix->multi) return multi_add_device(ix, x, n, (hipStream_t)stream);
    IndexOp op(ix);
    if ((rc = op.begin((hipStream_t)stream)) == KNN_OK) rc = add_device_locked(ix, x, n, op.stream());
    return op.finish(rc);
}

int knn_add(knn_index_t* ix, const float* x, int64_t n) {
    int rc;
    if ((rc = add_args_ok(ix, x, n)) != KNN_OK || n == 0) return rc;
    if (ix->multi) return multi_add(ix, x, n);
    IndexOp op(ix);
    if ((rc = op.begin_host()) != KNN_OK) return rc;
    if ((rc = reserve_rows(ix, ix->ntotal + n, ix->stream)) != KNN_OK) return rc;
    const int64_t chunk = std::max<int64_t>(1, (int64_t)(64 << 20) / ((int64_t)ix->d * 4));
    for (int64_t r0 = 0; r0 < n; r0 += chunk) {
        const int64_t cn = std::min(chunk, n - r0);
// ... 224 lines not shown
                                 (hipStream_t)stream));
        return KNN_OK;
    }
    KNN_HIP(launch_merge_strided(cD, cI, nq, nlists, kin, kin, nf + 2 * n, nf / 2 + n, k, kmetric,
                                 kmetric ? 0 : 1, D, I, (hipStream_t)stream));
    return KNN_OK;
}

int knn_set_timing(knn_index_t* ix, int enable) {
    if (!ix) KNN_FAIL(KNN_EINVAL, "index is NULL");
    if (ix->multi) return multi_set_timing(ix, enable);
    IndexOp op(ix);
    ix->timing = enable != 0;
    ix->ev_used = 0;
    return KNN_OK;
}

int knn_set_fence_mode(knn_index_t* ix, int mode) {
    if (!ix) KNN_FAIL(KNN_EINVAL, "index is NULL");
    if (mode != KNN_FENCE_EAGER && mode != KNN_FENCE_LAZY) KNN_FAIL(KNN_EINVAL, "unknown fence mode %d", mode);
    std::lock_guard<std::mutex> lk(ix->mu);
    if (ix->multi) {
        int rc = multi_set_fence_mode(ix, mode);
        if (rc != KNN_OK) return rc;
    }
    ix->fence.lazy = mode == KNN_FENCE_LAZY;
    return KNN_OK;
}

int knn_kernel_time(knn_index_t* ix, double* total_ms, int* launches) {
    if (!ix || !total_ms || !launches) KNN_FAIL(KNN_EINVAL, "NULL argument");
    if (ix->multi) return multi_kernel_time(ix, total_ms, launches);
    IndexOp op(ix);
    double tot = 0.0;
    for (size_t i = 0; i + 1 < ix->ev_used; i += 2) {
        KNN_HIP(hipEventSynchronize(ix->ev[i + 1]));
        float ms = 0.f;
        KNN_HIP(hipEventElapsedTime(&ms, ix->ev[i], ix->ev[i + 1]));
        tot += ms;
    }
    *total_ms = tot;
    *launches = (int)(ix->ev_used / 2);
    ix->ev_used = 0;
    return KNN_OK;
}

int knn_set_search_mode(knn_index_t* ix, int mode) {
    if (!ix) KNN_FAIL(KNN_EINVAL, "index is NULL");
    if (mode != KNN_SEARCH_AUTO && mode != KNN_SEARCH_EXACT && mode != KNN_SEARCH_SPLIT &&
        mode != KNN_SEARCH_BF16 && mode != KNN_SEARCH_I8)
        KNN_FAIL(KNN_EINVAL, "unknown search mode %d", mode);
    if (ix->multi) return multi_set_search_mode(ix, mode);
    std::lock_guard<std::mutex> lk(ix->mu);
    if (mode == KNN_SEARCH_SPLIT && !ix->split_ok)
        KNN_FAIL(KNN_EINVAL, "split search needs d >= 256; d = %d", ix->d);
    if (mode == KNN_SEARCH_BF16 && !ix->b16_ok)
        KNN_FAIL(KNN_EINVAL, "bf16 search needs d >= 64; d = %d", ix->d);
    if (mode == KNN_SEARCH_I8 && ix->nblk8 <= 0)
        KNN_FAIL(KNN_EINVAL, "int8 search needs 64 <= d <= 4096; d = %d", ix->d);
    ix->mode = mode;
    return KNN_OK;
}

int knn_search_stats(knn_index_t* ix, int64_t* split_queries, int64_t* fallback_queries,
                     float* max_err_ratio) {
    return knn_search_stats2(ix, split_queries, fallback_queries, nullptr, max_err_ratio);
}

int knn_search_stats2(knn_index_t* ix, int64_t* split_queries, int64_t* fallback_queries,
                      int64_t* second_chance_queries, float* max_err_ratio) {
    if (!ix || !split_queries || !fallback_queries) KNN_FAIL(KNN_EINVAL, "NULL argument");
    if (ix->multi)
        return multi_search_stats(ix, split_queries, fallback_queries, second_chance_queries,
                                  max_err_ratio);
    IndexOp op(ix);
    int64_t first_fail = 0;
    *fallback_queries = 0;
    int rc = ix->stat_valid ? op.begin_host() : KNN_OK;
    if (rc == KNN_OK) rc = read_search_stats(ix, split_queries, fallback_queries, &first_fail, max_err_ratio);
    if (second_chance_queries) *second_chance_queries = first_fail - *fallback_queries;
    return op.finish_synced(rc);
}

int knn_last_path(const knn_index_t* ix) {
    if (!ix) return KNN_EINVAL;
    return ix->multi ? multi_last_path(ix) : ix->last_path;
}

static int large_k_fallbacks_one(knn_index* ix, int64_t* n) {
    IndexOp op(ix);
    int rc = ix->lk_fail ? op.begin_host() : KNN_OK;
    if (rc == KNN_OK) rc = largek_fallbacks(ix, n);
    return op.finish_synced(rc);
}

int knn_large_k_fallbacks(const knn_index_t* cix, int64_t* n) {
    if (!cix || !n) KNN_FAIL(KNN_EINVAL, "NULL argument");
    knn_index* ix = const_cast<knn_index*>(cix);
    if (!ix->multi) return large_k_fallbacks_one(ix, n);
    *n = 0;
    for (int s = 0; s < multi_num_shards(ix); ++s) {
        int64_t v = 0;
        const int rc = large_k_fallbacks_one(const_cast<knn_index*>(multi_shard(ix, s)), &v);
        if (rc != KNN_OK) return rc;
        *n += v;
    }
    return KNN_OK;
}

static_assert((int)Route::Exact == kModeF32 && (int)Route::Split == kModeSplit && (int)Route::B16 == kModeBF16,
              "knn_plan_kernel prints a generic tile's route as its kMode");

int knn_plan(const knn_index_t* cix, int64_t nq, int k, int* tr, int* tq, int* splits, int* wgs) {
    if (!cix || !tr || !tq || !splits || !wgs) KNN_FAIL(KNN_EINVAL, "NULL argument");
    const knn_index* ix = cix->multi ? multi_shard(cix, 0) : cix;
    const Plan p = choose_route(*ix, std::min(nq, kQueryChunk), k).plan;
    *tr = p.bm; *tq = p.bq;
    *splits = p.nsplit; *wgs = p.wgs;
    return KNN_OK;
}

int knn_plan_kernel(const knn_index_t* cix, int64_t nq, int k, char* name, int cap) {
    if (!cix || !name || cap < 1) KNN_FAIL(KNN_EINVAL, "NULL argument");
    const knn_index* ix = cix->multi ? multi_shard(cix, 0) : cix;
    const int l2 = ix->metric == KNN_METRIC_L2 ? 1 : 0;
    const RoutePlan rp = choose_route(*ix, std::min(nq, kQueryChunk), k);
    const Plan& p = rp.plan;
    if (rp.route == Route::I8)
        std::snprintf(name, cap, "knn_i8_scan_kernel<%d, %d, %d>", rp.i8_inst, p.km, (ix->nblk8 + 15) / 16);
    else if (p.big)
        std::snprintf(name, cap, "knn_b16w_tile_kernel%s<%d, %d, %s>",
                      ix->xt_state == TailCopy::Built && rp.tail_ok ? "_i8t" : "", p.km, l2,
                      p.ib > 0 ? "true" : "false");
    else
        std::snprintf(name, cap, "knn_tile_topk_kernel<%d, %d, ..., %d, ...>", p.wr, p.wq, (int)rp.route);
    return KNN_OK;
}

int knn_debug_i8tail(knn_index_t* ix, int* head, int* dpt, int64_t i0, int64_t n, int8_t* codes,
                     float* scales, float* stats) {
    if (!ix) KNN_FAIL(KNN_EINVAL, "index is NULL");
    if (ix->multi) KNN_FAIL(KNN_EINVAL, "knn_debug_i8tail: single-device indexes only");
    IndexOp op(ix);
    if (ix->xt_state != TailCopy::Built || !ix->xt) KNN_FAIL(KNN_EINVAL, "the index has no int8 tail copy");
    if (i0 < 0 || n < 0 || i0 + n > ix->ntotal) KNN_FAIL(KNN_EINVAL, "rows outside [0, ntotal)");
    if (head) *head = ix->xt_head;
    if (dpt) *dpt = ix->xt_dpt;
    int rc = op.begin_host();
    auto down = [&](void* dst, const void* src, size_t row) {
        if (rc == KNN_OK && dst && n > 0)
            rc = HipStreams::fail(hipMemcpyAsync(dst, (const char*)src + (size_t)i0 * row, (size_t)n * row,
                                                 hipMemcpyDeviceToHost, ix->stream), "hipMemcpyAsync");
    };
    down(codes, ix->xt.get(), (size_t)ix->xt_dpt);
    down(scales, ix->xts.get(), sizeof(float));
    down(stats, ix->xtm.get(), sizeof(float4));
    return op.finish(rc);
}

}
```

### image_recommender_amd/csrc/knn_index.h

```cpp
#pragma once

#include <hip/hip_runtime.h>

#include <algorithm>
#include <cstdint>
#include <mutex>
#include <string>
#include <vector>

#include "dev_buf.h"
#include "knn_kernels.h"
#include "knn_plan.h"
#include "stream_fence.h"

namespace imgrec {

void set_err(const char* fmt, ...) __attribute__((format(printf, 1, 2)));
const char* test_knob(const char* name);

#define KNN_FAIL(code, ...)              \
    do {                                 \
        ::imgrec::set_err(__VA_ARGS__);  \
        return (code);                   \
    } while (0)

#define KNN_HIP(expr)                                                                  \
    do {                                                                               \
        hipError_t e_ = (expr);                                                        \
        if (e_ != hipSuccess) {                                                        \
            ::imgrec::set_err("%s failed: %s", #expr, hipGetErrorString(e_));          \
            return e_ == hipErrorOutOfMemory ? KNN_ENOMEM : KNN_EHIP;                  \
        }                                                                              \
    } while (0)

struct DeviceGuard {
    int old = -1;
    explicit DeviceGuard(int dev) {
        if (hipGetDevice(&old) != hipSuccess) old = -1;
        if (dev >= 0 && dev != old) (void)hipSetDevice(dev);
    }
    ~DeviceGuard() {
        int cur = -1;
        if (old >= 0 && hipGetDevice(&cur) == hipSuccess && cur != old) (void)hipSetDevice(old);
    }
};

inline int64_t round_up(int64_t v, int64_t m) { return (v + m - 1) / m * m; }

inline int hip_result(hipError_t e, const char* call) {
    if (e == hipSuccess) return KNN_OK;
    set_err("%s failed: %s", call, hipGetErrorString(e));
    return e == hipErrorOutOfMemory ? KNN_ENOMEM : KNN_EHIP;
}
struct DeviceSpace {
    static constexpr bool kSlack = true;
    static int alloc(void** p, size_t bytes) {
        return hip_result(hipMalloc(p, bytes), "hipMalloc((void**)p, n * sizeof(T))");
    }
    static void free(void* p) { (void)hipFree(p); }
};
struct PinnedSpace {
    static constexpr bool kSlack = false;
    static int alloc(void** p, size_t bytes) {
        return hip_result(hipHostMalloc(p, bytes, hipHostMallocDefault),
                            "hipHostMalloc(p, need_bytes, hipHostMallocDefault)");
    }
    static void free(void* p) { (void)hipHostFree(p); }
};
template <typename T> using DevBuf = Buf<T, DeviceSpace>;
template <typename T> using PinBuf = Buf<T, PinnedSpace>;
struct HipStreams {
    using Stream = hipStream_t;
    using Event = hipEvent_t;
    using DeviceScope = DeviceGuard;
    static int create_event(Event* e) { return hipEventCreateWithFlags(e, hipEventDisableTiming); }
    static void destroy_event(Event e) { (void)hipEventDestroy(e); }
    static int record(Event e, Stream s) { return hipEventRecord(e, s); }
    static int wait(Stream s, Event e) { return hipStreamWaitEvent(s, e, 0); }
    static int sync_stream(Stream s) { return hipStreamSynchronize(s); }
    static int sync_device() { return hipDeviceSynchronize(); }
    static void clear_error() { (void)hipGetLastError(); }
    static int fail(int e, const char* call) { return hip_result((hipError_t)e, call); }
};

}

using imgrec::DevBuf;
using imgrec::PinBuf;

struct knn_index : imgrec::IndexShape {
    int device = 0;
    bool merge_fuse = true;
    bool chance_skip = true;
    int chance_direct_max = 4;
    int direct_raw = 1;
    int i8_half_k = 12;
    int i8_pool64 = 4;
    int i8_pool_ch = 2;
    bool i8_pool_forced = false;
    DevBuf<int> i8_dyn;
    bool stream_lists = true;
    bool merge_single = false;
    bool shared_bound = true;
    bool rerank_nw4 = false;
    bool rerank_p1k = true;
    bool i8_fused_prep = true;
    bool merge_fuse1 = true;
    int64_t cap = 0, id_offset = 0;
    bool trained = true;
    DevBuf<float> xb;
    DevBuf<float> xn;
    DevBuf<uint32_t> xs;
    DevBuf<uint16_t> xh;
    DevBuf<float> xr;
    DevBuf<int8_t> x8;
    DevBuf<float> x8s;
    DevBuf<float> x8r;
    DevBuf<float> x8r_max;
    DevBuf<int8_t> xt;
    DevBuf<float> xts;
    DevBuf<float4> xtm;
    DevBuf<float> xt_max;
    int xt_head = 0, xt_dpt = 0;
    bool xt_tried = false;
    bool xt_no_trial = false;
    DevBuf<int8_t> qt;
    DevBuf<float> qts;
    DevBuf<float> q_eip;
    DevBuf<int8_t> q8;
    DevBuf<float> q8s;
    DevBuf<float> q8r;
    DevBuf<float> xn_max;
    DevBuf<float> xr_max;
    bool xn_max_stale = true;
    int last_path = 0;
    int64_t last_split_queries = 0;
    hipStream_t stream = nullptr;
    std::mutex mu;
    imgrec::Fence<imgrec::HipStreams> fence;
    DevBuf<float> qpad;
    DevBuf<float> qnorm;
    DevBuf<float> cand_d;
    DevBuf<int64_t> cand_i;
    DevBuf<uint32_t> qsplit;
    DevBuf<float> cand2_d;
    DevBuf<int64_t> cand2_i;
    DevBuf<int> fail;
    DevBuf<int> chance;
    DevBuf<float> sc_key;
    DevBuf<int64_t> sc_lab;
    DevBuf<unsigned> sc_meta;
    DevBuf<int> sc_done;
    DevBuf<int> stat;
    int stat_seq = 0;
    bool stat_valid = false;
    DevBuf<uint16_t> qb16;
    DevBuf<float> q_resid;
    DevBuf<float> floor;
    DevBuf<float> heads;
    DevBuf<float> mws_d;
    DevBuf<int64_t> mws_i;
    DevBuf<float> mws_f;
    DevBuf<uint32_t> sbound;
    DevBuf<float> fb_q;
    DevBuf<float> fb_qn;
    DevBuf<float> fb_cd;
    DevBuf<int64_t> fb_ci;
    DevBuf<int> tail_ctl;
    PinBuf<float> pq;
    PinBuf<float> pd;
    PinBuf<int64_t> pi;
    DevBuf<float> hq;
    DevBuf<float> hd;
    DevBuf<int64_t> hi;
    bool timing = false;
    std::vector<hipEvent_t> ev;
    size_t ev_used = 0;
    struct knn_multi* multi = nullptr;
    DevBuf<uint64_t> lk_run;
    DevBuf<int> lk_fail;
    DevBuf<uint64_t> hk_a;
    DevBuf<uint64_t> hk_b;
    DevBuf<unsigned> hk_off;
    DevBuf<char> hk_tmp;
    size_t range_cap0 = size_t(1) << 20;
    DevBuf<uint64_t> rg_ent;
    DevBuf<uint32_t> rg_entq;
    DevBuf<uint64_t> rg_seg;
    DevBuf<uint32_t> rg_cnt;
    DevBuf<uint32_t> rg_off;
    DevBuf<uint32_t> rg_cur;
    DevBuf<unsigned long long> rg_total;
    PinBuf<unsigned long long> rg_total_h;
    DevBuf<uint32_t> ft_list;
    DevBuf<uint32_t> ft_blk;
    DevBuf<uint32_t> ft_m;
    PinBuf<uint32_t> ft_m_h;
    DevBuf<uint8_t> ft_bits;
    int64_t remove_chunk = 0;
    PinBuf<uint32_t> rm_h;
    DevBuf<uint32_t> rm_pref;
};

struct knn_range_result {
    int device = 0;
    int64_t nq = 0, size = 0;
    DevBuf<int64_t> lims;
    DevBuf<float> D;
    DevBuf<int64_t> I;
    hipEvent_t done = nullptr;
};

namespace imgrec {

const char* last_error();
int set_metric(knn_index* ix, int metric);
int set_trained(knn_index* ix, bool trained);
struct IndexOp : OpScope<HipStreams> {
    explicit IndexOp(knn_index* ix) : OpScope(ix->mu, ix->device, ix->fence, ix->stream) {}
};
int stage_queries(knn_index* ix, const float* q, int64_t nq, int k, bool pinned = false);
int stage_bitmap(knn_index* ix, const uint8_t* bitmap, int64_t* nbits);
int fetch_results(knn_index* ix, int64_t nq, int k, float* D, int64_t* I);
enum { kColXb, kColXn, kColXs, kColXh, kColXr, kColX8, kColX8s, kColX8r, kColXt, kColXts, kColXtm, kCorpusColumns };
int corpus_columns(knn_index* ix, Column<DeviceSpace>* cols, bool all = false);
int reserve_rows(knn_index* ix, int64_t need, hipStream_t st);
int add_device_locked(knn_index* ix, const float* x, int64_t n, hipStream_t st);
int ensure_split(knn_index* ix, hipStream_t st);
int ensure_i8(knn_index* ix, hipStream_t st);
int ensure_i8tail(knn_index* ix, hipStream_t st);
void drop_i8tail(knn_index* ix, imgrec::TailCopy next);
int create_single(int d, int metric, int device, knn_index** out);
void free_single(knn_index* ix);
int search_locked(knn_index* ix, const float* q, int64_t nq, int k, float* D, int64_t* I,
                  hipStream_t st);
int timed_begin(knn_index* ix, hipStream_t st, hipEvent_t* e1);
int read_search_stats(knn_index* ix, int64_t* split_q, int64_t* fallback_q, int64_t* first_fail,
                      float* ratio);
int largek_search(knn_index* ix, const float* q, int64_t nq, int k, float* D, int64_t* I,
                  hipStream_t st);
bool stream_lists_ok(const knn_index* ix, int64_t nq);
int stream_splits(const knn_index* ix);
hipError_t launch_stream_lists(const knn_index* ix, const float* qpad, const float* qnorm, int64_t nq,
                               int metric, int sp, float* cd, int64_t* ci, hipStream_t st);
int largek_fallbacks(knn_index* ix, int64_t* n);
hipError_t launch_merge_large(const float* cD, const int64_t* cI, int nlists, int64_t nq, int kin,
                              int64_t sd, int64_t si, int k, int metric, float* D, int64_t* I,
                              hipStream_t st);
int hugek_search(knn_index* ix, const float* q, int64_t nq, int k, float* D, int64_t* I,
                 hipStream_t st);
hipError_t sort_u64_segments(uint64_t* in, uint64_t* out, int64_t total, int nseg, const unsigned* off,
                             unsigned end_bit, DevBuf<char>& tmp, hipStream_t st);
hipError_t sort_equal_segments(uint64_t* in, uint64_t* out, int nseg, int64_t seg, unsigned end_bit,
                               unsigned* off, DevBuf<char>& tmp, hipStream_t st);
hipError_t launch_merge_huge(const float* cD, const int64_t* cI, int nlists, int64_t nq, int kin,
                             int64_t sd, int64_t si, int k, int metric, float* D, int64_t* I,
                             hipStream_t st);
hipError_t launch_merge_any(const float* cD, const int64_t* cI, int nlists, int64_t nq, int kin,
                            int64_t sd, int64_t si, int k, int metric, float* D, int64_t* I,
                            hipStream_t st);
int range_search_locked(knn_index* ix, const float* q, int64_t nq, float radius, hipStream_t st,
                        knn_range_result** out);
int range_result_from_host(int device, int64_t nq, const int64_t* lims, const float* D, const int64_t* I,
                           hipStream_t st, knn_range_result** out);
void range_result_free(knn_range_result* r);
int filtered_search_locked(knn_index* ix, const float* q, int64_t nq, int k, const uint8_t* bits,
                           int64_t nbits, const int64_t* lmap, float* D, int64_t* I, hipStream_t st);
int compact_rows(knn_index* ix, const uint8_t* bits, int64_t nbits, const int64_t* lmap, bool invert,
                 hipStream_t st);
int remove_rows_locked(knn_index* ix, const uint8_t* bits, int64_t nbits, const int64_t* lmap,
                       int64_t* extra, hipStream_t st, int64_t* nremoved);
hipError_t launch_renumber_labels(int64_t* lab, int64_t n, const uint32_t* words, const uint32_t* pref,
                                  int64_t nbits, int64_t removed, hipStream_t st);

}
```

### image_recommender_amd/csrc/knn_kernels.h

```cpp
#pragma once

#include <hip/hip_runtime.h>
#include <stdint.h>

#include "knn_consts.h"

namespace imgrec {

constexpr int kModeF32 = 0;
constexpr int kModeSplit = 1;
constexpr int kModeBF16 = 2;
constexpr int kModeI8 = 3;

struct TileArgs {
    int wr, wq, km;
    int wb = 4;
    int sbk = 0;
    int mode = kModeF32;
    const float* xb;
    const float* xnorm;
    int nrows, dp;
    const float* qp;
    const float* qnorm;
    int nq;
    int metric;
    int ntiles, nsplit, nqb;
    int64_t id_offset;
    float* cand_d;
    int64_t* cand_i;
    int ncand;
    int ib = 0;
    uint32_t* sbound = nullptr;
    const int8_t* xt = nullptr;
    const float* xts = nullptr;
    const int8_t* qt = nullptr;
    const float* qts = nullptr;
    int t_head = 0, t_dpt = 0;
};

constexpr int kSBWords = 16, kSBCoef = 12, kSBFloor = 14;

struct SharedBoundPrep {
    uint32_t* rec = nullptr;
    const float* qnorm = nullptr;
    const float* xn_max = nullptr;
    const float* xr_max = nullptr;
    float c_acc = 0.f, c_fp = 0.f, c_trunc = 0.f;
    int metric = 0, km = 0;
};

struct I8TailPrep {
    int8_t* codes = nullptr;
    float* scale = nullptr;
    float* e_ip = nullptr;
    const float* xt_max = nullptr;
    const float* xn_max = nullptr;
    int head = 0, dpt = 0;
    float c_acc = 0.f;
};

constexpr int kRerankWavesHost = 8;

struct RerankArgs {
    int mode;
    const float* qp;
    const float* qnorm;
    int dp;
    const float* xb;
    const float* xn;
    const float* xn_max;
    int64_t id_offset;
    float* cd;
    int64_t* ci;
    int kc;
    int64_t nq;
    int k, metric;
    float c_trunc = 0.f;
    float c_split, c_fp;
    const float* q_resid;
    const float* xr_max;
    const float* e_ip = nullptr;
    float* floor;
    const uint32_t* sbound = nullptr;
    const float* l1_d = nullptr;
    const int64_t* l1_i = nullptr;
    const float* l1_floor = nullptr;
    int l1_G = 0;
    int l0_lists = 0;
    int s_lists = 0;
    int nw = 0;
    int p1 = 0;
    int chance_skip = 0;
    int direct = 0;
    const float* heads = nullptr;
    int heads_n = 0;
    float* D;
    int64_t* I;
    int* stats;
    int* fail_list;
    int* chance_list = nullptr;
    const float* raw_d = nullptr;
    const int64_t* raw_i = nullptr;
    int raw_lists = 0, raw_km = 0;
    int64_t raw_stride_q = 0;
    int* tail_ctl = nullptr;
    int sc_slices = 1;
    float* sc_key = nullptr;
    int64_t* sc_lab = nullptr;
    unsigned* sc_meta = nullptr;
    int* sc_done = nullptr;
};

struct TailArgs {
    RerankArgs r;
    int parity, first;
    int* stat;
    const float* qpad;
    const float* qnorm;
    int dp, nrows, ntiles, metric;
    const float* xb;
    const float* xn;
    int64_t id_offset;
    float* fq;
    float* fqn;
    float* fcd;
    int64_t* fci;
    int* ticket;
    int km, lists_km;
};

struct I8Args {
    const int8_t* codes;
    const float* scales;
    const float* xnorm;
    int nrows, nblk;
    const int8_t* qcodes;
    const float* qscales;
    const float* qnorm;
    int nq, km, nsplit, l2;
    int64_t id_offset;
    float* cand_d;
    int64_t* cand_i;
    int ncand;
    const float* qsrc;
    int d, dp, normalize;
    float* qpad;
    float* qnorm_out;
    float* qresid;
    int* zero_ctl = nullptr;
    float* heads = nullptr;
    int raw16 = 0;
    int half_k = 0;
    int* dyn = nullptr;
    int pool = 0, pool_ch = 1;
};
__host__ __device__ inline int i8_slot(int nblk, int b, int c) {
    const int g = b >> 4, m = nblk - 16 * g < 16 ? nblk - 16 * g : 16;
    return 64 * g + m * c + (b & 15);
}
hipError_t launch_i8_rows(const float* xb, int64_t n, int dp, int nblk, int8_t* codes, float* scales,
                          float* resid, hipStream_t st);
hipError_t launch_i8_scan(const I8Args& a, hipStream_t st);
hipError_t launch_i8_query_prep(const float* src, int64_t n, int d, int dp, int64_t n_pad,
                                int normalize, int nblk, float* dst, float* norms, int8_t* codes,
                                float* scales, float* resid, hipStream_t st);

hipError_t launch_rows_ingest(const float* src, int64_t n, int d, int dp, int64_t n_pad,
                              int normalize, float* dst, float* norms, hipStream_t st);
hipError_t launch_tile_topk(const TileArgs& a, hipStream_t st);
hipError_t launch_b16_big(const TileArgs& a, hipStream_t st);
hipError_t launch_merge(const float* cd, const int64_t* ci, int64_t nq, int nlists, int kin,
                        int64_t stride_q, int64_t stride_l, int k, int metric, int negate_in,
                        float* D, int64_t* I, hipStream_t st);
hipError_t launch_merge_strided(const float* cd, const int64_t* ci, int64_t nq, int nlists, int kin,
                                int64_t stride_q, int64_t stride_l, int64_t stride_li, int k,
                                int metric, int negate_in, float* D, int64_t* I, hipStream_t st);
hipError_t launch_merge_candidates(const float* cd, const int64_t* ci, int64_t nq, int nlists,
                                   int kin, int64_t stride_q, int64_t stride_l, int kout,
                                   int64_t id_offset, float* D, int64_t* I, float* floor,
                                   float* ws_d, int64_t* ws_i, float* ws_floor, hipStream_t st,
                                   int* l1_G = nullptr);
hipError_t launch_fill_empty(float* D, int64_t* I, int64_t n, int metric, hipStream_t st);
hipError_t launch_iota64(int64_t* dst, int64_t n, int64_t start, hipStream_t st);
hipError_t launch_map_labels(int64_t* I, int64_t n, const int64_t* lmap, int64_t offset,
                             hipStream_t st);

hipError_t launch_split_rows(const float* src, int64_t n, int dp, int bk, uint32_t* dst,
                             hipStream_t st);
hipError_t launch_rerank_certify(const RerankArgs& a, hipStream_t st);
hipError_t launch_cert_tail(const TailArgs& a, int grid, hipStream_t st);
constexpr int kTailWGPerCU = 1;
hipError_t launch_gather_rows(const float* src, const float* src_norm, int dp, const int* list,
                              int64_t n, int64_t n_pad, float* dst, float* dst_norm, hipStream_t st);
hipError_t launch_scatter_results(const float* sd, const int64_t* si, const int* list, int64_t n,
                                  int k, float* D, int64_t* I, hipStream_t st);
hipError_t launch_bf16_rows(const float* src, int64_t n, int dp, int dpb, uint16_t* dst,
                            float* resid, hipStream_t st, const SharedBoundPrep* sb = nullptr);
hipError_t launch_query_prep_b16(const float* src, int64_t n, int d, int dp, int dpb, int64_t n_pad,
                                 int normalize, float* dst, float* norms, uint16_t* qb, float* resid,
                                 hipStream_t st, const SharedBoundPrep* sb = nullptr,
                                 const I8TailPrep* tp = nullptr);
hipError_t launch_block_absmax(const float* xb, int64_t n, int dp, int nblk, float* out, hipStream_t st);
hipError_t launch_i8tail_rows(const float* xb, int64_t n, int dp, int dpb, int head, int dpt,
                              int8_t* codes, float* scale, float4* stat, hipStream_t st);
hipError_t launch_i8tail_max(const float4* stat, int64_t n, float* out, hipStream_t st);
hipError_t launch_max_norm(const float* xn, int64_t n, float* out, hipStream_t st);

hipError_t sort_u64_segments(uint64_t* in, uint64_t* out, int64_t total, int nseg, const unsigned* off,
                             unsigned end_bit, void** tmp, size_t* tmp_cap, bool async_tmp, hipStream_t st);
hipError_t launch_sorted_write(const uint64_t* sorted, int64_t seg, int nq, int k, int metric, int rb,
                               int64_t id_offset, bool label_is_row, float* D, int64_t* I, hipStream_t st);
hipError_t launch_ivfpq_scan_all(const float* lut, const int64_t* probes, int64_t nq, int nprobe,
                                 const int64_t* list_off, const uint16_t* codes, const int64_t* ids,
                                 int m, int ksub, const int64_t* probe_off, const uint32_t* seg_off,
                                 int64_t total, int k, float* D, int64_t* I, hipStream_t st);
hipError_t launch_ivfpq_lut(const float* resid, int64_t nr, int d, int m, int ksub,
                            const float* cbt, float* lut, hipStream_t st);
hipError_t launch_ivfpq_scan(const float* lut, const int64_t* probes, int64_t nq, int nprobe,
                             const int64_t* list_off, const uint16_t* codes, const int64_t* ids,
                             int m, int ksub, int k, float* D, int64_t* I, hipStream_t st);

}
```

### image_recommender_amd/csrc/knn_plan.cpp

```cpp
#include <algorithm>
#include <cmath>
#include <cstdlib>
#include <vector>

#include "knn_plan.h"

namespace imgrec {

static Plan tiled(Plan p, int64_t ntotal, int64_t nq, int target, int lists) {
    p.nqb = (int)((nq + p.bq - 1) / p.bq);
    p.nq_pad = p.nqb * p.bq;
    p.ntiles = (int)((ntotal + p.bm - 1) / p.bm);
    p.nsplit = std::max(1, std::min((target + p.nqb - 1) / p.nqb, p.ntiles));
    p.ncand = p.nsplit * lists * p.km;
    p.wgs = p.nqb * p.nsplit;
    return p;
}

Plan make_plan(int64_t ntotal, int64_t nq, int k, int cus) {
    Plan p{};
    p.km = fallback_km(k);
    int wg_per_cu;
    if (nq <= 32) { p.wr = 2; p.wq = 1; wg_per_cu = 3; }
    else if (nq <= 128) { p.wr = 2; p.wq = 2; wg_per_cu = 2; }
    else { p.wr = 1; p.wq = 4; wg_per_cu = 2; }
    p.bm = p.wr * 128; p.bq = p.wq * 32;
    return tiled(p, ntotal, nq, cus * wg_per_cu, p.wr * 2);
}

int fallback_km(int k) { return k <= 8 ? 8 : (k <= 10 ? 10 : (k <= 16 ? 16 : 32)); }

Plan make_split_plan(int64_t ntotal, int64_t nq, int kc, int cus) {
    Plan p{};
    p.km = kc; p.wr = 1; p.wq = 4;
    p.bm = p.wr * 32 * kSplitWB; p.bq = p.wq * 32;
    return tiled(p, ntotal, nq, cus * 2, p.wr * 2);
}

int split_kc(int k) { return k <= 10 ? 16 : (k <= 16 ? 32 : 0); }

float split_coef(int dp) {
    return (float)(3.1 * std::ldexp(1.0, -16) + 1.02 * (15.0 * (dp / 16) + 16.0) * std::ldexp(1.0, -23));
}
float rerank_coef(int dp) {
    return (float)(1.02 * (4.0 * ((dp + 255) / 256) + 8.0) * std::ldexp(1.0, -24));
}

float b16_acc_coef(int dpb) {
    return (float)(1.02 * (5.0 * (dpb / 16) + 16.0) * std::ldexp(1.0, -23));
}
float i8t_acc_coef(int head) {
    return (float)(1.02 * (5.0 * (head / 16) + 16.0 + 3.0) * std::ldexp(1.0, -23));
}

int i8t_pick_head(const float* blkmax, int nblk) {
    for (int j = 0; j < nblk; ++j) {
        std::vector<float> v(blkmax + j, blkmax + nblk);
        std::nth_element(v.begin(), v.begin() + (v.size() - 1) / 2, v.end());
        const float med = v[(v.size() - 1) / 2];
        bool ok = true;
        for (int b = j; b < nblk && ok; ++b) ok = blkmax[b] <= 2.f * med && 2.f * blkmax[b] >= med;
        if (!ok) continue;
        const int head = 64 * j, dpb = 64 * nblk;
        return dpb - head >= kI8TMinTail && head <= dpb / 2 ? head : -1;
    }
    return -1;
}

float i8_acc_coef(int nblk) {
    return (float)(1.02 * (16.0 + 4.0 * ((nblk + 15) / 16)) * std::ldexp(1.0, -23));
}

Plan make_i8_plan(int64_t ntotal, int64_t nq, int k, int cus, int wgpcu, int nblk) {
    const int kI8WGPCU = wgpcu > 0 ? wgpcu : (nq == 1 && nblk >= 24 ? 1 : nq <= 2 ? 2 : 3);
    Plan p{};
    p.km = b16_km(k);
    p.wr = 1; p.wq = 1; p.bm = 8;
    p.bq = (int)nq; p.nqb = 1; p.nq_pad = (int)nq;
    const int64_t groups = (ntotal + 7) / 8;
    p.ntiles = (int)groups;
    p.nsplit = (int)std::max<int64_t>(1, std::min<int64_t>((int64_t)cus * kI8WGPCU, groups));
    p.ncand = p.nsplit * p.km;
    p.wgs = p.nsplit;
    return p;
}

int b16_km(int k) { return k <= 16 ? 16 : 32; }

constexpr int kB16NarrowQ = 32;

Plan make_b16_plan(int64_t ntotal, int64_t nq, int k, int cus, int dpb) {
    Plan p{};
    if (nq >= kB16BigMinQ && k <= 10 && dpb <= 16384) {
        p.big = true;
        p.km = k <= 8 ? 8 : 10;
        p.wr = 2; p.wq = 4;
        p.bm = kB16BigRows; p.bq = kB16BigQueries;
        p = tiled(p, ntotal, nq, cus, 1);
        const int64_t groups = (ntotal + 7) / 8, cnt = (groups + p.nsplit - 1) / p.nsplit;
        const int64_t idx_max = (cnt + 31) / 32 * 256 - 1;
        int ib = 1;
        while ((int64_t{1} << ib) <= idx_max) ++ib;
        p.ib = ib <= kB16PackMaxIB ? ib : 0;
        return p;
    }
    p.km = b16_km(k);
    const bool narrow = nq <= kB16NarrowQ;
    p.wr = narrow ? 2 : kB16WR;
    p.wq = narrow ? 1 : kB16WQ;
    p.bm = p.wr * 32 * kB16WB; p.bq = p.wq * 32;
    return tiled(p, ntotal, nq, cus * kB16WGPCU, p.wr * 2);
}

namespace {

bool b16_serves(const IndexShape& ix) {
    return ix.b16_ok && (ix.mode == KNN_SEARCH_BF16 || ix.mode == KNN_SEARCH_AUTO || ix.mode == KNN_SEARCH_I8);
}

constexpr int kI8AutoQ = 8;
constexpr int kI8MinBlocks = 8;
bool i8_wins_8q(int nblk) { return (nblk >= 14 && nblk <= 16) || nblk >= 23; }
constexpr int64_t kI8SmallCopyBytes = 64ll << 20;
bool i8_serves(const IndexShape& ix, int64_t nq) {
    if (ix.nblk8 <= 0 || nq > kI8MaxQ) return false;
    if (ix.mode == KNN_SEARCH_I8) return true;
    if (ix.mode != KNN_SEARCH_AUTO || nq > kI8AutoQ) return false;
    const int64_t i8_row = i8_row_bytes(ix.nblk8) + 4 * ix.nblk8;
    const bool wide_enough = nq <= 2 ? true : nq <= 4 ? ix.nblk8 >= kI8MinBlocks : i8_wins_8q(ix.nblk8);
    return !ix.b16_ok || wide_enough || ix.ntotal * i8_row <= kI8SmallCopyBytes;
}

bool split_serves(const IndexShape& ix, int64_t nq, int k) {
    if (!ix.split_ok || ix.mode == KNN_SEARCH_EXACT || split_kc(k) == 0) return false;
    if (ix.mode == KNN_SEARCH_SPLIT) return true;
    return (ix.mode == KNN_SEARCH_AUTO || ix.mode == KNN_SEARCH_I8) && nq > 128 && ix.ntotal >= 16384;
}

}

RoutePlan choose_route(const IndexShape& ix, int64_t nq, int k) {
    RoutePlan r{};
    const bool cand = k <= KNN_MAX_K;
    if (cand && i8_serves(ix, nq)) {
        r.route = Route::I8;
        r.plan = make_i8_plan(ix.ntotal, nq, k, ix.cus, ix.i8_wgpcu, ix.nblk8);
        r.i8_inst = nq <= 2 ? (int)nq : (nq <= 4 ? 4 : 8);
    } else if (cand && b16_serves(ix)) {
        r.route = Route::B16;
        r.plan = make_b16_plan(ix.ntotal, nq, k, ix.cus, ix.dpb);
        r.tail_ok = r.plan.big && ix.i8tail && ix.xt_state != TailCopy::Ineligible && ix.dpb <= 4096 &&
                    ix.ntotal > 0 && (ix.mode == KNN_SEARCH_AUTO || ix.mode == KNN_SEARCH_I8);
    } else if (split_serves(ix, nq, k)) {
        r.route = Route::Split;
        r.plan = make_split_plan(ix.ntotal, nq, split_kc(k), ix.cus);
    } else {
        r.route = Route::Exact;
        r.plan = make_plan(ix.ntotal, nq, k, ix.cus);
    }
    return r;
}

}
```

### image_recommender_amd/csrc/knn_plan.h

```cpp
#pragma once

#include <cstdint>

#include "../../include/imgrec_knn.h"
#include "knn_consts.h"

namespace imgrec {

struct Plan {
    int wr, wq, km, bm, bq;
    int nqb, nq_pad, ntiles, nsplit, ncand, wgs;
    bool big;
    int ib;
};
constexpr int64_t kQueryChunk = 8192;
Plan make_plan(int64_t ntotal, int64_t nq, int k, int cus);
Plan make_split_plan(int64_t ntotal, int64_t nq, int kc, int cus);
Plan make_b16_plan(int64_t ntotal, int64_t nq, int k, int cus, int dpb);
constexpr int kFallbackWR = 2;
int fallback_km(int k);
int split_kc(int k);
float split_coef(int dp);
float rerank_coef(int dp);
float b16_acc_coef(int dpb);
float i8t_acc_coef(int head);
int i8t_pick_head(const float* blkmax, int nblk);
constexpr int kI8TMinTail = 512;
constexpr int kI8MaxQ = 8;
float i8_acc_coef(int nblk);
Plan make_i8_plan(int64_t ntotal, int64_t nq, int k, int cus, int wgpcu, int nblk);
constexpr int kI8WGPCUDefault = 0;
constexpr int kB16Cand = 64;
int b16_km(int k);

enum class TailCopy { Undecided, Built, Ineligible };

struct IndexShape {
    int d = 0, dp = 0, metric = KNN_METRIC_L2, cus = 256, mode = KNN_SEARCH_AUTO;
    int dpb = 0;
    int nblk8 = 0;
    int i8_wgpcu = kI8WGPCUDefault;
    bool split_ok = false, b16_ok = false;
    bool i8tail = true;
    TailCopy xt_state = TailCopy::Undecided;
    int64_t ntotal = 0;
};

enum class Route { Exact = 0, Split = 1, B16 = 2, I8 = 3 };
struct RoutePlan {
    Route route;
    Plan plan;
    bool tail_ok;
    int i8_inst;
};
RoutePlan choose_route(const IndexShape& ix, int64_t nq, int k);

}
```

### image_recommender_amd/csrc/knn_refine.hip

```cpp

#include <hip/hip_runtime.h>
#include <stdint.h>
#include <float.h>
#include <math.h>

#include <algorithm>
#include <type_traits>

#include "knn_certify.h"
#include "knn_kernels.h"
#include "wave_ops.h"

namespace imgrec {

__device__ __forceinline__ uint32_t bf16_rne(float x) {
    const uint32_t u = __float_as_uint(x);
    return (u + 0x7fffu + ((u >> 16) & 1u)) >> 16;
}

__global__ void __launch_bounds__(256)
split_rows_kernel(const float* __restrict__ src, int64_t n, int dp, int bk,
                  uint32_t* __restrict__ dst) {
    const int per_row = dp / 8;
    const int ks = bk / 16;
    const int64_t t = (int64_t)blockIdx.x * blockDim.x + threadIdx.x;
    if (t >= n * per_row) return;
    const int64_t row = t / per_row;
    const int r = (int)(t - row * per_row);
    const int j = r / (2 * ks), h = (r / ks) & 1, s = r % ks;
    const float* x = src + row * dp + j * bk + 16 * s + 8 * h;
    const float4 v0 = *reinterpret_cast<const float4*>(x);
    const float4 v1 = *reinterpret_cast<const float4*>(x + 4);
    const float e[8] = {v0.x, v0.y, v0.z, v0.w, v1.x, v1.y, v1.z, v1.w};
    uint32_t hi[4], lo[4];
#pragma unroll
    for (int p = 0; p < 4; ++p) {
        const uint32_t h0 = bf16_rne(e[2 * p]), h1 = bf16_rne(e[2 * p + 1]);
        const uint32_t l0 = bf16_rne(e[2 * p] - __uint_as_float(h0 << 16));
        const uint32_t l1 = bf16_rne(e[2 * p + 1] - __uint_as_float(h1 << 16));
        hi[p] = h0 | (h1 << 16);
        lo[p] = l0 | (l1 << 16);
    }
    uint32_t* o = dst + row * dp + j * bk + (h * 2 * ks + 2 * s) * 4;
    *reinterpret_cast<uint4*>(o) = make_uint4(hi[0], hi[1], hi[2], hi[3]);
    *reinterpret_cast<uint4*>(o + 4) = make_uint4(lo[0], lo[1], lo[2], lo[3]);
}

__global__ void __launch_bounds__(256)
bf16_rows_kernel(const float* __restrict__ src, int64_t n, int dp, int dpb,
                 uint16_t* __restrict__ dst, float* __restrict__ resid, const SharedBoundPrep sb) {
    const int64_t row = (int64_t)blockIdx.x * 4 + (threadIdx.x >> 6);
    const int lane = threadIdx.x & 63;
    if (row >= n) return;
    const float* x = src + row * dp;
    uint16_t* o = dst + row * dpb;
    float acc = 0.f;
    for (int c = lane; c < dpb / 8; c += 64) {
        float e[8];
        if (8 * c + 8 <= dp) {
            const float4 v0 = *reinterpret_cast<const float4*>(x + 8 * c);
            const float4 v1 = *reinterpret_cast<const float4*>(x + 8 * c + 4);
            e[0] = v0.x; e[1] = v0.y; e[2] = v0.z; e[3] = v0.w;
            e[4] = v1.x; e[5] = v1.y; e[6] = v1.z; e[7] = v1.w;
        } else {
#pragma unroll
            for (int j = 0; j < 8; ++j) e[j] = (8 * c + j < dp) ? x[8 * c + j] : 0.f;
        }
        uint32_t w[4];
#pragma unroll
        for (int p = 0; p < 4; ++p) {
            const uint32_t h0 = bf16_rne(e[2 * p]), h1 = bf16_rne(e[2 * p + 1]);
            const float r0 = e[2 * p] - __uint_as_float(h0 << 16);
            const float r1 = e[2 * p + 1] - __uint_as_float(h1 << 16);
            acc = fmaf(r0, r0, acc);
            acc = fmaf(r1, r1, acc);
            w[p] = h0 | (h1 << 16);
        }
        *reinterpret_cast<uint4*>(o + 8 * c) = make_uint4(w[0], w[1], w[2], w[3]);
    }
#pragma unroll
    for (int off = 32; off > 0; off >>= 1) acc += __shfl_xor(acc, off, 64);
    if (lane == 0) resid[row] = sqrtf(acc);
    if (sb.rec) shared_bound_reset(sb, row, lane, sb.qnorm[row], sqrtf(acc));
}

__global__ void __launch_bounds__(256)
block_absmax_kernel(const float* __restrict__ xb, int64_t n, int dp, int nblk, float* __restrict__ out) {
    const int64_t r0 = (int64_t)blockIdx.x * 256, r1 = r0 + 256 < n ? r0 + 256 : n;
    for (int j = threadIdx.x; j < 64 * nblk; j += 256) {
        float m = 0.f;
        if (j < dp)
            for (int64_t r = r0; r < r1; ++r) m = fmaxf(m, fabsf(xb[r * dp + j]));
#pragma unroll
        for (int off = 32; off > 0; off >>= 1) m = fmaxf(m, __shfl_xor(m, off, 64));
        if ((threadIdx.x & 63) == 0) atomicMax(reinterpret_cast<unsigned*>(out) + j / 64, __float_as_uint(m));
    }
}

__device__ __forceinline__ void load_chunk8(const float* x, int c, int dp, float (&e)[8]) {
    if (8 * c + 8 <= dp) {
        const float4 v0 = *reinterpret_cast<const float4*>(x + 8 * c);
        const float4 v1 = *reinterpret_cast<const float4*>(x + 8 * c + 4);
        e[0] = v0.x; e[1] = v0.y; e[2] = v0.z; e[3] = v0.w;
        e[4] = v1.x; e[5] = v1.y; e[6] = v1.z; e[7] = v1.w;
    } else {
#pragma unroll
        for (int j = 0; j < 8; ++j) e[j] = (8 * c + j < dp) ? x[8 * c + j] : 0.f;
    }
}

__global__ void __launch_bounds__(256)
i8tail_rows_kernel(const float* __restrict__ src, int64_t n, int dp, int dpb, int head, int dpt,
                   int8_t* __restrict__ codes, float* __restrict__ scales, float4* __restrict__ stat) {
    const int64_t row = (int64_t)blockIdx.x * 4 + (threadIdx.x >> 6);
    const int lane = threadIdx.x & 63;
    if (row >= n) return;
    const float* x = src + row * dp;
    const int hc = head / 8;
    float amax = 0.f, nh = 0.f, nt = 0.f, rh = 0.f, rt = 0.f;
    for (int c = lane; c < dpb / 8; c += 64) {
        float e[8];
        load_chunk8(x, c, dp, e);
#pragma unroll
        for (int t = 0; t < 8; ++t) {
            if (c < hc) {
                const float r = e[t] - __uint_as_float(bf16_rne(e[t]) << 16);
                nh = fmaf(e[t], e[t], nh);
                rh = fmaf(r, r, rh);
            } else {
                nt = fmaf(e[t], e[t], nt);
                amax = fmaxf(amax, fabsf(e[t]));
            }
        }
    }
#pragma unroll
    for (int off = 32; off > 0; off >>= 1) amax = fmaxf(amax, __shfl_xor(amax, off, 64));
    const float sc = amax / 127.f, inv = amax > 0.f ? 127.f / amax : 0.f;
    int8_t* oc = codes + row * dpt;
    for (int c = hc + lane; c < hc + dpt / 8; c += 64) {
        uint32_t w[2] = {0u, 0u};
        if (c < dpb / 8) {
            float e[8];
            load_chunk8(x, c, dp, e);
#pragma unroll
            for (int t = 0; t < 8; ++t) {
                const float cf = fminf(fmaxf(rintf(e[t] * inv), -127.f), 127.f);
                const float r = fmaf(-sc, cf, e[t]);
                rt = fmaf(r, r, rt);
                w[t >> 2] |= ((uint32_t)(int)cf & 0xffu) << (8 * (t & 3));
            }
        }
        *reinterpret_cast<uint2*>(oc + 8 * (c - hc)) = make_uint2(w[0], w[1]);
    }
#pragma unroll
    for (int off = 32; off > 0; off >>= 1) {
        nh += __shfl_xor(nh, off, 64);
        nt += __shfl_xor(nt, off, 64);
        rh += __shfl_xor(rh, off, 64);
        rt += __shfl_xor(rt, off, 64);
    }
    if (lane == 0) {
        const float up = 1.f + 1.0f / 512.f;
        scales[row] = sc;
        stat[row] = make_float4(sqrtf(rt) * up, sqrtf(rh) * up, sqrtf(nt) * up, sqrtf(nh) * up);
    }
}

__global__ void i8tail_max_kernel(const float4* __restrict__ stat, int64_t n, float* __restrict__ out) {
    float4 m = make_float4(0.f, 0.f, 0.f, 0.f);
    for (int64_t i = (int64_t)blockIdx.x * blockDim.x + threadIdx.x; i < n;
         i += (int64_t)gridDim.x * blockDim.x) {
        const float4 v = stat[i];
        m = make_float4(fmaxf(m.x, v.x), fmaxf(m.y, v.y), fmaxf(m.z, v.z), fmaxf(m.w, v.w));
    }
#pragma unroll
    for (int off = 32; off > 0; off >>= 1) {
        m.x = fmaxf(m.x, __shfl_xor(m.x, off, 64));
        m.y = fmaxf(m.y, __shfl_xor(m.y, off, 64));
        m.z = fmaxf(m.z, __shfl_xor(m.z, off, 64));
        m.w = fmaxf(m.w, __shfl_xor(m.w, off, 64));
    }
    if ((threadIdx.x & 63) == 0) {
        unsigned* o = reinterpret_cast<unsigned*>(out);
        atomicMax(o, __float_as_uint(m.x));
        atomicMax(o + 1, __float_as_uint(m.y));
        atomicMax(o + 2, __float_as_uint(m.z));
        atomicMax(o + 3, __float_as_uint(m.w));
    }
}

template <int IT>
__global__ void __launch_bounds__(256)
query_prep_b16_kernel(const float* __restrict__ src, int64_t n, int d, int dp, int dpb,
                      int64_t n_pad, int normalize, float* __restrict__ dst,
                      float* __restrict__ norms, uint16_t* __restrict__ qb,
                      float* __restrict__ resid, const SharedBoundPrep sb, const I8TailPrep tp) {
    const int64_t row = (int64_t)blockIdx.x * 4 + (threadIdx.x >> 6);
    const int lane = threadIdx.x & 63;
    if (row >= n_pad) return;
    const bool real = row < n;
    const float* s = src + row * d;
    float e[IT][8];
#pragma unroll
    for (int it = 0; it < IT; ++it) {
        const int j0 = 8 * (lane + 64 * it);
        if (real && (d & 3) == 0 && j0 + 8 <= d) {
            const float4 v0 = *reinterpret_cast<const float4*>(s + j0);
            const float4 v1 = *reinterpret_cast<const float4*>(s + j0 + 4);
            e[it][0] = v0.x; e[it][1] = v0.y; e[it][2] = v0.z; e[it][3] = v0.w;
            e[it][4] = v1.x; e[it][5] = v1.y; e[it][6] = v1.z; e[it][7] = v1.w;
        } else {
#pragma unroll
            for (int t = 0; t < 8; ++t) e[it][t] = (real && j0 + t < d) ? s[j0 + t] : 0.f;
        }
    }
    float scale = 1.f;
    if (normalize) {
        float acc = 0.f;
#pragma unroll
        for (int it = 0; it < IT; ++it)
#pragma unroll
            for (int t = 0; t < 8; ++t) acc = fmaf(e[it][t], e[it][t], acc);
#pragma unroll
        for (int off = 32; off > 0; off >>= 1) acc += __shfl_xor(acc, off, 64);
        if (acc > 0.f) scale = (float)(1.0 / (double)sqrtf(acc));
    }
    float nacc = 0.f, racc = 0.f;
    float* o = dst + row * dp;
    uint16_t* ob = qb + row * dpb;
#pragma unroll
    for (int it = 0; it < IT; ++it) {
        const int c = lane + 64 * it;
        if (8 * c >= dpb) continue;
        float v[8];
        uint32_t w[4];
#pragma unroll
        for (int t = 0; t < 8; ++t) {
            v[t] = normalize ? e[it][t] * scale : e[it][t];
            nacc = fmaf(v[t], v[t], nacc);
        }
#pragma unroll
        for (int p2 = 0; p2 < 4; ++p2) {
            const uint32_t h0 = bf16_rne(v[2 * p2]), h1 = bf16_rne(v[2 * p2 + 1]);
            const float r0 = v[2 * p2] - __uint_as_float(h0 << 16);
            const float r1 = v[2 * p2 + 1] - __uint_as_float(h1 << 16);
            racc = fmaf(r0, r0, racc);
            racc = fmaf(r1, r1, racc);
            w[p2] = h0 | (h1 << 16);
        }
        *reinterpret_cast<uint4*>(ob + 8 * c) = make_uint4(w[0], w[1], w[2], w[3]);
        if (8 * c < dp) {
            *reinterpret_cast<float4*>(o + 8 * c) = make_float4(v[0], v[1], v[2], v[3]);
            *reinterpret_cast<float4*>(o + 8 * c + 4) = make_float4(v[4], v[5], v[6], v[7]);
        }
    }
#pragma unroll
    for (int off = 32; off > 0; off >>= 1) {
        nacc += __shfl_xor(nacc, off, 64);
        racc += __shfl_xor(racc, off, 64);
    }
    if (lane == 0) {
        norms[row] = nacc;
        resid[row] = sqrtf(racc);
    }
    float e_ip_q = -1.f;
    if (tp.codes) {
        const int hc = tp.head / 8;
        float amax = 0.f, nh = 0.f, nt = 0.f, rh = 0.f;
#pragma unroll
        for (int it = 0; it < IT; ++it) {
            const int c = lane + 64 * it;
            if (8 * c >= dpb) continue;
#pragma unroll
            for (int t = 0; t < 8; ++t) {
                const float v = normalize ? e[it][t] * scale : e[it][t];
                if (c < hc) {
                    const float r = v - __uint_as_float(bf16_rne(v) << 16);
                    nh = fmaf(v, v, nh);
                    rh = fmaf(r, r, rh);
                } else {
                    nt = fmaf(v, v, nt);
                    amax = fmaxf(amax, fabsf(v));
                }
            }
        }
#pragma unroll
        for (int off = 32; off > 0; off >>= 1) amax = fmaxf(amax, __shfl_xor(amax, off, 64));
        const float sc = amax / 127.f, inv = amax > 0.f ? 127.f / amax : 0.f;
        float rt = 0.f;
        int8_t* oc = tp.codes + row * tp.dpt;
#pragma unroll
        for (int it = 0; it < IT; ++it) {
            const int c = lane + 64 * it;
            if (8 * c >= dpb || c < hc) continue;
            uint32_t w[2] = {0u, 0u};
#pragma unroll
            for (int t = 0; t < 8; ++t) {
                const float v = normalize ? e[it][t] * scale : e[it][t];
                const float cf = fminf(fmaxf(rintf(v * inv), -127.f), 127.f);
                const float r = fmaf(-sc, cf, v);
                rt = fmaf(r, r, rt);
                w[t >> 2] |= ((uint32_t)(int)cf & 0xffu) << (8 * (t & 3));
            }
            *reinterpret_cast<uint2*>(oc + 8 * (c - hc)) = make_uint2(w[0], w[1]);
        }
        for (int c = dpb / 8 + lane; c < hc + tp.dpt / 8; c += 64)
            *reinterpret_cast<uint2*>(oc + 8 * (c - hc)) = make_uint2(0u, 0u);
#pragma unroll
        for (int off = 32; off > 0; off >>= 1) {
            nh += __shfl_xor(nh, off, 64);
            nt += __shfl_xor(nt, off, 64);
            rh += __shfl_xor(rh, off, 64);
            rt += __shfl_xor(rt, off, 64);
        }
        const float up = 1.f + 1.0f / 512.f;
        const float* m = tp.xt_max;
        e_ip_q = i8tail_e_ip(sqrtf(nacc) * up, sqrtf(nt) * up, sqrtf(nh) * up, sqrtf(rt) * up, sqrtf(rh) * up,
                             m[0], m[1], m[2], m[3], sqrtf(*tp.xn_max) * up, tp.c_acc);
        if (lane == 0) {
            tp.scale[row] = sc;
            tp.e_ip[row] = e_ip_q;
        }
    }
    if (sb.rec) shared_bound_reset(sb, row, lane, nacc, sqrtf(racc), e_ip_q);
}

template <int IT, bool SL, int NW>
__global__ void __launch_bounds__(NW * 64) __attribute__((amdgpu_waves_per_eu(4)))
rerank_certify_kernel(const RerankArgs a) {
    __shared__ float skey[64];
    __shared__ int64_t slab[64];
    const int lane = threadIdx.x & 63;
    const int wave = threadIdx.x >> 6;
    const int64_t q = blockIdx.x;
    const int dp = a.dp, kc = a.kc, k = a.k, metric = a.metric;
    const int64_t id_offset = a.id_offset;
    if (a.tail_ctl && blockIdx.x == 0 && threadIdx.x < 4) a.tail_ctl[threadIdx.x] = 0;
    RR_STAMP(0);
    const int n4 = dp / 4;
    const float4* q4 = reinterpret_cast<const float4*>(a.qp + q * dp);
    float4 qr[IT > 0 ? IT : 1];
    if constexpr (IT > 0) {
#pragma unroll
        for (int it = 0; it < IT; ++it) {
            const int i = lane + 64 * it;
            qr[it] = i < n4 ? q4[i] : make_float4(0.f, 0.f, 0.f, 0.f);
        }
    }
#ifdef IMGREC_TAIL_STAMPS
    asm volatile("s_waitcnt vmcnt(0)" ::: "memory");
    RR_STAMP(5);
#endif
    const bool fused = NW == kRerankWaves && (a.l1_G > 0 || (SL && a.s_lists > 0));
    __shared__ float s_mkey[64];
    __shared__ int64_t s_mlab[64];
    __shared__ __attribute__((aligned(16))) uint64_t s_ent[kRerankWaves * 64];
    __shared__ float s_floor;
    __shared__ uint64_t s_sel[kRerankWaves][64 + 256];
    __shared__ float s_gfl[kRerankWaves];
    if (SL && fused && a.s_lists > 0) {
        constexpr uint64_t kEmpty = ~0ull;
        constexpr int NT = kRerankWaves * 64;
        const int t = threadIdx.x, KIN = a.raw_km, L = a.s_lists, E = L * KIN;
        const float* rd = a.raw_d + q * a.raw_stride_q;
        const int64_t* ri = a.raw_i + q * a.raw_stride_q;
        uint64_t* lead = &s_sel[0][0];
        uint64_t* surv = &s_sel[0][0] + 128;
        __shared__ uint64_t s_U;
        __shared__ int s_cnt;
        uint64_t v[2] = {kEmpty, kEmpty};
        float fl = INFINITY;
        int nlead = 0, nval = 0;
#pragma unroll
        for (int h = 0; h < 2; ++h) {
            const int e = t + NT * h;
            if (e < E) {
                const int64_t lb = ri[e];
                const float kv = rd[e];
                if (lb >= 0) {
                    v[h] = ((uint64_t)key_bits_ordered(kv) << 32) | (uint32_t)(lb - id_offset);
                    ++nval;
                    if (e % KIN == KIN - 1) fl = fminf(fl, kv);
                }
                const int p = e % KIN;
                if (p < 2) {
                    lead[(e / KIN) * 2 + p] = v[h];
                    nlead += v[h] != kEmpty ? 1 : 0;
                }
            }
        }
        if (t == 0) s_cnt = 0;
#pragma unroll
        for (int off = 32; off > 0; off >>= 1) fl = fminf(fl, __shfl_xor(fl, off, 64));
        if (lane == 0) s_gfl[wave] = fl;
        int nlead_all = 0, nval_all = 0;
        {
            __shared__ int s_nl[kRerankWaves], s_nv[kRerankWaves];
            const int wl = wave_sum_i32(nlead), wv = wave_sum_i32(nval);
            if (lane == 0) { s_nl[wave] = wl; s_nv[wave] = wv; }
            __syncthreads();
#pragma unroll
            for (int i = 0; i < kRerankWaves; ++i) { nlead_all += s_nl[i]; nval_all += s_nv[i]; }
        }
        const int K = min(kc, nval_all);
        if (nlead_all >= kc) {
#pragma unroll
            for (int h = 0; h < 2; ++h) {
                const int e = t + NT * h;
                if (e < E && e % KIN < 2 && v[h] != kEmpty) {
                    int r = 0;
                    for (int j = 0; j < 2 * L; ++j) r += lead[j] < v[h] ? 1 : 0;
                    if (r == kc - 1) s_U = v[h];
                }
            }
        } else if (t == 0) {
            s_U = kEmpty - 1;
        }
        __syncthreads();
        const uint64_t U = s_U;
#pragma unroll
        for (int h = 0; h < 2; ++h)
            if (v[h] <= U) surv[atomicAdd(&s_cnt, 1)] = v[h];
        __syncthreads();
        const int C = s_cnt;
#pragma unroll
        for (int h = 0; h < 2; ++h) {
            if (v[h] <= U) {
                int r = 0;
                for (int j = 0; j < C; ++j) r += surv[j] < v[h] ? 1 : 0;
                if (r < K) {
                    const float kv = key_from_ordered((uint32_t)(v[h] >> 32));
                    const int64_t lb = (int64_t)(uint32_t)v[h] + id_offset;
                    s_mkey[r] = kv; s_mlab[r] = lb;
                    a.cd[q * kc + r] = kv; a.ci[q * kc + r] = lb;
                }
            }
        }
        if (t >= K && t < kc) {
            s_mkey[t] = FLT_MAX; s_mlab[t] = -1;
            a.cd[q * kc + t] = FLT_MAX; a.ci[q * kc + t] = -1;
        }
        if (wave == 0) {
            float f = lane < kRerankWaves ? s_gfl[lane] : INFINITY;
// ... 201 lines not shown
#pragma unroll
        for (int off = 32; off > 0; off >>= 1) r = fmaxf(r, __shfl_xor(r, off, 64));
        if (lane == 0 && m > 0) atomicMax(reinterpret_cast<unsigned*>(a.stats + 1), __float_as_uint(r));
    }

    const int lo_tau = __shfl((int)(lab & 0xffffffff), kc - 1, 64);
    const int hi_tau = __shfl((int)(lab >> 32), kc - 1, 64);
    const int64_t lab_tau = ((int64_t)hi_tau << 32) | (uint32_t)lo_tau;
    float tau = (lab_tau >= 0 && nvalid >= kc) ? __shfl(ak, kc - 1, 64) : INFINITY;
    if (fused) tau = fminf(tau, s_floor);
    else if (a.floor) tau = fminf(tau, a.floor[q]);
    tau = fminf(tau, sfloor);
    const float a_out = __shfl(ak, min(m, 63), 64);
    if (m < nvalid) tau = fminf(tau, a_out);
    bool failed = false;
    if (tau != INFINITY) {
        float sk = (inP && rank == k - 1) ? key : -INFINITY;
#pragma unroll
        for (int off = 32; off > 0; off >>= 1) sk = fmaxf(sk, __shfl_xor(sk, off, 64));
        failed = !(m >= k && (tau - B.bound_a(tau)) > (sk + B.bound_f(sk)));
    }
    if (failed && lane == 0) {
        atomicAdd(a.stats + 2, 1);
        if (a.raw_d) a.chance_list[atomicAdd(a.stats + 3, 1)] = (int)q;
        else a.fail_list[atomicAdd(a.stats, 1)] = (int)q;
    }
}

__global__ void __launch_bounds__(256)
gather_rows_kernel(const float* __restrict__ src, const float* __restrict__ src_norm, int dp,
                   const int* __restrict__ list, int64_t n, int64_t n_pad,
                   float* __restrict__ dst, float* __restrict__ dst_norm) {
    const int64_t row = (int64_t)blockIdx.x * 4 + (threadIdx.x >> 6);
    const int lane = threadIdx.x & 63;
    if (row >= n_pad) return;
    float* o = dst + row * dp;
    if (row >= n) {
        for (int j = lane; j < dp; j += 64) o[j] = 0.f;
        if (lane == 0) dst_norm[row] = 0.f;
        return;
    }
    const float* s = src + (int64_t)list[row] * dp;
    for (int j = lane; j < dp; j += 64) o[j] = s[j];
    if (lane == 0) dst_norm[row] = src_norm[list[row]];
}

__global__ void __launch_bounds__(256)
scatter_results_kernel(const float* __restrict__ sd, const int64_t* __restrict__ si,
                       const int* __restrict__ list, int64_t n, int k, float* __restrict__ D,
                       int64_t* __restrict__ I) {
    const int64_t t = (int64_t)blockIdx.x * blockDim.x + threadIdx.x;
    if (t >= n * k) return;
    const int64_t r = t / k;
    const int j = (int)(t - r * k);
    D[(int64_t)list[r] * k + j] = sd[t];
    I[(int64_t)list[r] * k + j] = si[t];
}

__global__ void max_norm_kernel(const float* __restrict__ xn, int64_t n, float* __restrict__ out) {
    float m = 0.f;
    for (int64_t i = (int64_t)blockIdx.x * blockDim.x + threadIdx.x; i < n;
         i += (int64_t)gridDim.x * blockDim.x)
        m = fmaxf(m, xn[i]);
#pragma unroll
    for (int off = 32; off > 0; off >>= 1) m = fmaxf(m, __shfl_xor(m, off, 64));
    if ((threadIdx.x & 63) == 0) atomicMax(reinterpret_cast<unsigned*>(out), __float_as_uint(m));
}

hipError_t launch_split_rows(const float* src, int64_t n, int dp, int bk, uint32_t* dst,
                             hipStream_t st) {
    if (n <= 0) return hipSuccess;
    if ((bk != 16 && bk != 32) || dp % bk != 0) return hipErrorInvalidValue;
    const int64_t threads = n * (dp / 8);
    hipLaunchKernelGGL(split_rows_kernel, dim3((unsigned)((threads + 255) / 256)), dim3(256), 0, st,
                       src, n, dp, bk, dst);
    return hipGetLastError();
}

#ifdef IMGREC_TAIL_STAMPS
extern "C" int knn_rerank_stamps_read(unsigned long long* host) {
    return (int)hipMemcpyFromSymbol(host, HIP_SYMBOL(imgrec::g_rr_stamps), sizeof(imgrec::g_rr_stamps));
}
#endif

hipError_t launch_rerank_certify(const RerankArgs& a, hipStream_t st) {
    if (a.nq <= 0) return hipSuccess;
    if (a.kc > 64 || a.k > a.kc || a.k > 64 || a.dp % 4 != 0 || !a.stats || !a.fail_list)
        return hipErrorInvalidValue;
    if (a.l1_G > 0 && (16 * a.l1_G > kRerankWaves * 64 || !a.floor)) return hipErrorInvalidValue;
    if (a.l1_G > 0 && a.l0_lists == 0 && (!a.l1_d || !a.l1_i || !a.l1_floor)) return hipErrorInvalidValue;
    if (a.l0_lists > 0 && (a.l1_G != (a.l0_lists + 63) / 64 || a.l1_G > kRerankWaves ||
                           a.raw_km != 16 || !a.raw_d || !a.raw_i))
        return hipErrorInvalidValue;
    if (a.raw_d && (!a.raw_i || !a.chance_list || a.raw_km < a.k || a.raw_lists <= 0))
        return hipErrorInvalidValue;
    if (a.s_lists > 0 && (a.s_lists > 64 || a.raw_km > 16 || a.raw_lists != a.s_lists || !a.raw_d ||
                          !a.floor || !a.cd || !a.ci || a.l1_G > 0))
        return hipErrorInvalidValue;
    if (a.nw != 0 && (a.nw != 4 || a.s_lists > 0 || a.l1_G > 0 || a.chance_skip))
        return hipErrorInvalidValue;
#define IMGREC_RERANK(ITV)                                                                          \
    do {                                                                                            \
        if (a.nw == 4)                                                                              \
            hipLaunchKernelGGL((rerank_certify_kernel<ITV, false, 4>), dim3((unsigned)a.nq),         \
                               dim3(4 * 64), 0, st, a);                                             \
        else if (a.s_lists > 0)                                                                     \
            hipLaunchKernelGGL((rerank_certify_kernel<ITV, true, kRerankWaves>), dim3((unsigned)a.nq), \
                               dim3(kRerankWaves * 64), 0, st, a);                                  \
        else                                                                                        \
            hipLaunchKernelGGL((rerank_certify_kernel<ITV, false, kRerankWaves>), dim3((unsigned)a.nq), \
                               dim3(kRerankWaves * 64), 0, st, a);                                  \
    } while (0)
    if (a.dp <= 512) IMGREC_RERANK(2);
    else if (a.dp <= 1024) IMGREC_RERANK(4);
    else if (a.dp <= 2048) IMGREC_RERANK(8);
    else IMGREC_RERANK(0);
#undef IMGREC_RERANK
    return hipGetLastError();
}

hipError_t launch_gather_rows(const float* src, const float* src_norm, int dp, const int* list,
                              int64_t n, int64_t n_pad, float* dst, float* dst_norm, hipStream_t st) {
    if (n_pad <= 0) return hipSuccess;
    hipLaunchKernelGGL(gather_rows_kernel, dim3((unsigned)((n_pad + 3) / 4)), dim3(256), 0, st, src,
                       src_norm, dp, list, n, n_pad, dst, dst_norm);
    return hipGetLastError();
}

hipError_t launch_scatter_results(const float* sd, const int64_t* si, const int* list, int64_t n,
                                  int k, float* D, int64_t* I, hipStream_t st) {
    if (n <= 0) return hipSuccess;
    hipLaunchKernelGGL(scatter_results_kernel, dim3((unsigned)((n * k + 255) / 256)), dim3(256), 0,
                       st, sd, si, list, n, k, D, I);
    return hipGetLastError();
}

hipError_t launch_bf16_rows(const float* src, int64_t n, int dp, int dpb, uint16_t* dst,
                            float* resid, hipStream_t st, const SharedBoundPrep* sb) {
    if (n <= 0) return hipSuccess;
    if (dpb % 8 != 0 || dp % 8 != 0 || dpb < dp) return hipErrorInvalidValue;
    if (sb && sb->rec && !sb->qnorm) return hipErrorInvalidValue;
    hipLaunchKernelGGL(bf16_rows_kernel, dim3((unsigned)((n + 3) / 4)), dim3(256), 0, st, src, n, dp,
                       dpb, dst, resid, sb ? *sb : SharedBoundPrep{});
    return hipGetLastError();
}

hipError_t launch_query_prep_b16(const float* src, int64_t n, int d, int dp, int dpb, int64_t n_pad,
                                 int normalize, float* dst, float* norms, uint16_t* qb, float* resid,
                                 hipStream_t st, const SharedBoundPrep* sb, const I8TailPrep* tp) {
    if (n_pad <= 0) return hipSuccess;
    if (dpb % 8 != 0 || dp % 16 != 0 || dpb < dp || dp < d) return hipErrorInvalidValue;
    if (tp && tp->codes &&
        (tp->head % 64 != 0 || tp->head < 0 || tp->head >= dpb || tp->dpt % 128 != 0 ||
         tp->dpt < dpb - tp->head || !tp->scale || !tp->e_ip || !tp->xt_max || !tp->xn_max))
        return hipErrorInvalidValue;
    const dim3 grid((unsigned)((n_pad + 3) / 4)), block(256);
#define IMGREC_QPREP(ITV) hipLaunchKernelGGL((query_prep_b16_kernel<ITV>), grid, block, 0, st, src, n, \
                                             d, dp, dpb, n_pad, normalize, dst, norms, qb, resid,      \
                                             sb ? *sb : SharedBoundPrep{}, tp ? *tp : I8TailPrep{})
    if (dpb <= 512) IMGREC_QPREP(1);
    else if (dpb <= 1024) IMGREC_QPREP(2);
    else if (dpb <= 2048) IMGREC_QPREP(4);
    else if (dpb <= 4096) IMGREC_QPREP(8);
    else return hipErrorInvalidValue;
#undef IMGREC_QPREP
    return hipGetLastError();
}

hipError_t launch_block_absmax(const float* xb, int64_t n, int dp, int nblk, float* out, hipStream_t st) {
    hipError_t e = hipMemsetAsync(out, 0, (size_t)nblk * sizeof(float), st);
    if (e != hipSuccess || n <= 0) return e;
    hipLaunchKernelGGL(block_absmax_kernel, dim3((unsigned)((n + 255) / 256)), dim3(256), 0, st, xb, n, dp,
                       nblk, out);
    return hipGetLastError();
}

hipError_t launch_i8tail_rows(const float* xb, int64_t n, int dp, int dpb, int head, int dpt,
                              int8_t* codes, float* scale, float4* stat, hipStream_t st) {
    if (n <= 0) return hipSuccess;
    if (dpb % 64 != 0 || dp % 8 != 0 || dpb < dp || head % 64 != 0 || head < 0 || head >= dpb ||
        dpt % 128 != 0 || dpt < dpb - head)
        return hipErrorInvalidValue;
    hipLaunchKernelGGL(i8tail_rows_kernel, dim3((unsigned)((n + 3) / 4)), dim3(256), 0, st, xb, n, dp, dpb,
                       head, dpt, codes, scale, stat);
    return hipGetLastError();
}

hipError_t launch_i8tail_max(const float4* stat, int64_t n, float* out, hipStream_t st) {
    hipError_t e = hipMemsetAsync(out, 0, 4 * sizeof(float), st);
    if (e != hipSuccess || n <= 0) return e;
    const int64_t blocks = std::min<int64_t>(1024, (n + 255) / 256);
    hipLaunchKernelGGL(i8tail_max_kernel, dim3((unsigned)blocks), dim3(256), 0, st, stat, n, out);
    return hipGetLastError();
}

hipError_t launch_max_norm(const float* xn, int64_t n, float* out, hipStream_t st) {
    hipError_t e = hipMemsetAsync(out, 0, sizeof(float), st);
    if (e != hipSuccess || n <= 0) return e;
    const int64_t blocks = std::min<int64_t>(1024, (n + 255) / 256);
    hipLaunchKernelGGL(max_norm_kernel, dim3((unsigned)blocks), dim3(256), 0, st, xn, n, out);
    return hipGetLastError();
}

}
```

### image_recommender_amd/csrc/knn_search.cpp

```cpp
#include <cmath>
#include <cstdlib>
#include <cstring>

#include "knn_index.h"

namespace imgrec {

int timed_begin(knn_index* ix, hipStream_t st, hipEvent_t* e1) {
    *e1 = nullptr;
    if (!ix->timing) return KNN_OK;
    if (ix->ev_used + 2 > ix->ev.size()) {
        for (int i = 0; i < 64; ++i) {
            hipEvent_t e;
            KNN_HIP(hipEventCreate(&e));
            ix->ev.push_back(e);
        }
    }
    KNN_HIP(hipEventRecord(ix->ev[ix->ev_used], st));
    *e1 = ix->ev[ix->ev_used + 1];
    ix->ev_used += 2;
    return KNN_OK;
}

namespace {
// ... 80 lines not shown
    int rc;
    if ((rc = ix->fb_q.reserve((size_t)cap_rows * ix->dp)) != KNN_OK) return rc;
    if ((rc = ix->fb_qn.reserve((size_t)cap_rows)) != KNN_OK) return rc;
    if ((rc = ix->fb_cd.reserve(ncap)) != KNN_OK) return rc;
    if ((rc = ix->fb_ci.reserve(ncap)) != KNN_OK) return rc;
    if ((rc = ix->tail_ctl.reserve((size_t)4 + cap_rows / 32)) != KNN_OK) return rc;
    r.stats = ix->stat + 4 * parity;
    r.fail_list = ix->fail;
    r.chance_list = ix->chance;
    if (r.raw_d) {
        static const int kSlices = [] {
            const char* e = std::getenv("IMGREC_SC_SLICES");
            const int v = e ? std::atoi(e) : 0;
            return v > 0 ? v : 64;
        }();
        r.sc_slices = std::max(1, std::min({kSlices, 64, r.raw_lists, 1024 / k}));
        const size_t ns = (size_t)nq * r.sc_slices * k;
        if ((rc = ix->sc_key.reserve(ns)) != KNN_OK) return rc;
        if ((rc = ix->sc_lab.reserve(ns)) != KNN_OK) return rc;
        if ((rc = ix->sc_meta.reserve((size_t)nq * r.sc_slices * 4)) != KNN_OK) return rc;
        const size_t c0 = ix->sc_done.cap();
        if ((rc = ix->sc_done.reserve((size_t)nq)) != KNN_OK) return rc;
        if (ix->sc_done.cap() != c0)
            KNN_HIP(hipMemsetAsync(ix->sc_done, 0, ix->sc_done.cap() * sizeof(int), st));
        r.sc_key = ix->sc_key; r.sc_lab = ix->sc_lab; r.sc_meta = ix->sc_meta; r.sc_done = ix->sc_done;
    }
    r.tail_ctl = ix->tail_ctl;
    r.chance_skip = ix->chance_skip && r.raw_d && nq <= ix->cus ? 1 : 0;
    r.p1 = ix->rerank_p1k && nq > ix->cus ? k : 0;
    r.nw = ix->rerank_nw4 && nq > ix->cus && r.l1_G == 0 && r.s_lists == 0 && !r.chance_skip ? 4 : 0;
    if (!r.direct) KNN_HIP(launch_rerank_certify(r, st));
    TailArgs t{};
    t.r = r;
    t.parity = parity;
    t.first = first ? 1 : 0;
    t.stat = ix->stat;
    t.qpad = qpad;
    t.qnorm = qnorm;
    t.dp = ix->dp;
    t.nrows = (int)ix->ntotal;
    t.ntiles = (int)((ix->ntotal + bm - 1) / bm);
    t.metric = kmetric_of(ix);
    t.xb = ix->xb;
    t.xn = ix->xn;
    t.id_offset = ix->id_offset;
    t.fq = ix->fb_q;
    t.fqn = ix->fb_qn;
    t.fcd = ix->fb_cd;
    t.fci = ix->fb_ci;
    t.ticket = ix->tail_ctl + 4;
    t.km = km;
    t.lists_km = lists_km;
    const hipError_t e = launch_cert_tail(t, grid, st);
    if (e != hipSuccess) {
        (void)hipMemsetAsync(ix->stat, 0, 12 * sizeof(int), st);
        ix->stat_seq = 0;
        KNN_FAIL(KNN_EHIP, "certificate tail launch failed: %s", hipGetErrorString(e));
    }
    ++ix->stat_seq;
    ix->stat_valid = true;
    ix->last_split_queries += nq;
    return KNN_OK;
}

bool fuse_merge_level2(const knn_index* ix, int64_t nq) {
    return ix->merge_fuse && nq <= ix->cus;
}

bool fuse_merge_level1(const knn_index* ix, int64_t nq, int nlists, int km) {
    return fuse_merge_level2(ix, nq) && ix->merge_fuse1 && km == 16 && nlists > 64 &&
           nlists <= 64 * kRerankWavesHost;
}

bool fuse_merge_single(const knn_index* ix, int nlists, int km) {
    return ix->merge_single && nlists <= 64 && km <= 16;
}

int grow_cand(knn_index* ix, int64_t nq, int ncand, int kc, bool floor) {
    int rc;
    if ((rc = ix->cand_d.reserve((size_t)nq * ncand)) != KNN_OK) return rc;
    if ((rc = ix->cand_i.reserve((size_t)nq * ncand)) != KNN_OK) return rc;
    if ((rc = ix->cand2_d.reserve((size_t)nq * kc)) != KNN_OK) return rc;
    if ((rc = ix->cand2_i.reserve((size_t)nq * kc)) != KNN_OK) return rc;
    return floor ? ix->floor.reserve((size_t)nq) : KNN_OK;
}

RerankArgs rerank_args(const knn_index* ix, int mode, const float* qpad, const float* qnorm,
                       int64_t nq, int k, int kc, float* D, int64_t* I) {
    RerankArgs r{};
    r.mode = mode;
    r.qp = qpad; r.qnorm = qnorm; r.dp = ix->dp; r.xb = ix->xb; r.xn = ix->xn;
    r.xn_max = ix->xn_max; r.id_offset = ix->id_offset; r.kc = kc; r.nq = nq; r.k = k;
    r.metric = kmetric_of(ix); r.c_fp = rerank_coef(ix->dp); r.D = D; r.I = I;
    return r;
}

int merge_for_rerank(knn_index* ix, int64_t nq, int nlists, int km, int ncand, bool single,
                     RerankArgs* r, hipStream_t st) {
    const int kc = r->kc, ngrp = (nlists + 63) / 64;
    int rc;
    if (ngrp > 1) {
        if ((rc = ix->mws_d.reserve((size_t)nq * ngrp * kc)) != KNN_OK) return rc;
        if ((rc = ix->mws_i.reserve((size_t)nq * ngrp * kc)) != KNN_OK) return rc;
        if ((rc = ix->mws_f.reserve((size_t)nq * ngrp)) != KNN_OK) return rc;
    }
    int l1G = 0;
    const bool l0 = !single && fuse_merge_level1(ix, nq, nlists, km);
    if (l0) l1G = ngrp;
    else if (!single)
        KNN_HIP(launch_merge_candidates(ix->cand_d, ix->cand_i, nq, nlists, km, ncand, km, kc,
                                        ix->id_offset, ix->cand2_d, ix->cand2_i, ix->floor,
                                        ix->mws_d, ix->mws_i, ix->mws_f, st,
                                        fuse_merge_level2(ix, nq) ? &l1G : nullptr));
    r->cd = ix->cand2_d; r->ci = ix->cand2_i; r->floor = ix->floor;
    if (single) r->s_lists = nlists;
    if (l1G > 0) { r->l1_d = ix->mws_d; r->l1_i = ix->mws_i; r->l1_floor = ix->mws_f; r->l1_G = l1G; }
    if (l0) r->l0_lists = nlists;
    return KNN_OK;
}

int shared_bound_prep(knn_index* ix, const Plan& p, const float* qnorm, hipStream_t st,
                      SharedBoundPrep* sb) {
    *sb = SharedBoundPrep{};
    if (!ix->shared_bound || !p.big) return KNN_OK;
    int rc;
    if ((rc = refresh_maxima(ix, st)) != KNN_OK) return rc;
    if ((rc = ix->sbound.reserve((size_t)p.nq_pad * kSBWords)) != KNN_OK) return rc;
    sb->rec = ix->sbound;
    sb->qnorm = qnorm;
    sb->xn_max = ix->xn_max;
    sb->xr_max = ix->xr_max;
    sb->c_acc = b16_acc_coef(ix->dpb);
    sb->c_fp = rerank_coef(ix->dp);
    sb->c_trunc = p.ib > 0 ? (float)std::ldexp(1.0, p.ib - 23) : 0.f;
    sb->metric = kmetric_of(ix);
    sb->km = p.km;
    return KNN_OK;
}

bool stream_capturing(hipStream_t st) {
    hipStreamCaptureStatus s = hipStreamCaptureStatusNone;
    if (hipStreamIsCapturing(st, &s) != hipSuccess) { (void)hipGetLastError(); return false; }
    return s != hipStreamCaptureStatusNone;
}

int i8tail_prep(knn_index* ix, const RoutePlan& rp, hipStream_t st, I8TailPrep* tp) {
    *tp = I8TailPrep{};
    if (!rp.tail_ok) return KNN_OK;
    const Plan& p = rp.plan;
    if (ix->xt_state == TailCopy::Undecided && stream_capturing(st)) return KNN_OK;
    int rc;
    if ((rc = ensure_i8tail(ix, st)) != KNN_OK || ix->xt_state != TailCopy::Built) return rc;
    if ((rc = refresh_maxima(ix, st)) != KNN_OK) return rc;
    if ((rc = ix->qt.reserve((size_t)p.nq_pad * ix->xt_dpt)) != KNN_OK) return rc;
    if ((rc = ix->qts.reserve((size_t)p.nq_pad)) != KNN_OK) return rc;
    if ((rc = ix->q_eip.reserve((size_t)p.nq_pad)) != KNN_OK) return rc;
    tp->codes = ix->qt; tp->scale = ix->qts; tp->e_ip = ix->q_eip;
    tp->xt_max = ix->xt_max; tp->xn_max = ix->xn_max;
    tp->head = ix->xt_head; tp->dpt = ix->xt_dpt;
    tp->c_acc = i8t_acc_coef(ix->xt_head);
    return KNN_OK;
}

int i8tail_trial(knn_index* ix, int64_t nq, hipStream_t st) {
    if (stream_capturing(st)) return KNN_OK;
    int acc[4] = {0, 0, 0, 0};
    KNN_HIP(hipMemcpyAsync(acc, ix->stat + 8, sizeof(acc), hipMemcpyDeviceToHost, st));
    KNN_HIP(hipStreamSynchronize(st));
    ix->xt_tried = true;
    const int64_t reruns = acc[0];
    if (reruns * 32 <= nq) return KNN_OK;
    drop_i8tail(ix, TailCopy::Ineligible);
    return KNN_OK;
}

int b16_chunk(knn_index* ix, const Plan& p, const float* qpad, const float* qnorm, int64_t nq, int k,
              float* D, int64_t* I, hipStream_t st, bool q_ready, bool first, bool i8t) {
    const int kmetric = kmetric_of(ix);
    const int kc = kB16Cand;
    const int km = p.km;
    int rc;
    if ((rc = refresh_maxima(ix, st)) != KNN_OK) return rc;
    if ((rc = ix->qb16.reserve((size_t)p.nq_pad * ix->dpb)) != KNN_OK) return rc;
    if ((rc = ix->q_resid.reserve((size_t)p.nq_pad)) != KNN_OK) return rc;
    if ((rc = grow_cand(ix, nq, p.ncand, kc, true)) != KNN_OK) return rc;
    if ((rc = grow_stats(ix, nq, st)) != KNN_OK) return rc;
    SharedBoundPrep sb;
    if ((rc = shared_bound_prep(ix, p, qnorm, st, &sb)) != KNN_OK) return rc;
    if (!q_ready)
        KNN_HIP(launch_bf16_rows(qpad, p.nq_pad, ix->dp, ix->dpb, ix->qb16, ix->q_resid, st, &sb));
    TileArgs a{};
    a.wr = p.wr; a.wq = p.wq; a.km = km; a.wb = kB16WB; a.mode = kModeBF16;
    a.xb = reinterpret_cast<const float*>(ix->xh.get()); a.xnorm = ix->xn; a.nrows = (int)ix->ntotal;
    a.dp = ix->dpb / 2; a.qp = reinterpret_cast<const float*>(ix->qb16.get()); a.qnorm = qnorm;
    a.nq = (int)nq; a.metric = kmetric; a.ntiles = p.ntiles; a.nsplit = p.nsplit; a.nqb = p.nqb;
    a.id_offset = ix->id_offset; a.cand_d = ix->cand_d; a.cand_i = ix->cand_i; a.ncand = p.ncand;
    a.ib = p.big ? p.ib : 0;
    a.sbound = sb.rec;
    if (i8t) {
        if (!p.big || !q_ready || ix->xt_state != TailCopy::Built)
            KNN_FAIL(KNN_EINVAL, "int8 tail without its query prep");
        a.xt = ix->xt; a.xts = ix->xts; a.qt = ix->qt; a.qts = ix->qts;
        a.t_head = ix->xt_head; a.t_dpt = ix->xt_dpt;
    }
    KNN_TIMED(ix, st, p.big ? launch_b16_big(a, st) : launch_tile_topk(a, st));
    const int nlists = p.ncand / km;
    RerankArgs r = rerank_args(ix, kModeBF16, qpad, qnorm, nq, k, kc, D, I);
    r.c_split = b16_acc_coef(ix->dpb);
    r.c_trunc = a.ib > 0 ? (float)std::ldexp(1.0, a.ib - 23) : 0.f;
    r.q_resid = ix->q_resid; r.xr_max = ix->xr_max;
    if (i8t) r.e_ip = ix->q_eip;
    r.sbound = a.sbound;
    if ((rc = merge_for_rerank(ix, nq, nlists, km, p.ncand, fuse_merge_single(ix, nlists, km), &r,
                               st)) != KNN_OK)
        return rc;
    r.raw_d = ix->cand_d; r.raw_i = ix->cand_i; r.raw_lists = nlists; r.raw_km = km;
    r.raw_stride_q = p.ncand;
    return certify_chunk(ix, r, qpad, qnorm, nq, k, D, I, st, first);
}

int i8_chunk(knn_index* ix, const Plan& p, const float* qraw, const float* qpad, const float* qnorm,
             int64_t nq, int k, float* D, int64_t* I, hipStream_t st, bool first) {
    const int kmetric = kmetric_of(ix);
    const int kc = kB16Cand;
    const bool direct = ix->chance_direct_max > 0 && nq <= ix->chance_direct_max && k <= 64;
    const bool raw = direct && nq <= 4 &&
                     (ix->direct_raw == 2 || (ix->direct_raw == 1 && 16 * p.nsplit <= 4096));
    const int ncand = raw ? p.nsplit * 16 * p.km : p.ncand;
    int rc;
    if ((rc = ensure_i8(ix, st)) != KNN_OK) return rc;
    if ((rc = refresh_maxima(ix, st)) != KNN_OK) return rc;
    if ((rc = grow_cand(ix, nq, ncand, kc, true)) != KNN_OK) return rc;
    if ((rc = grow_stats(ix, nq, st)) != KNN_OK) return rc;
    I8Args a{};
    a.codes = ix->x8; a.scales = ix->x8s; a.xnorm = ix->xn; a.nrows = (int)ix->ntotal;
    a.nblk = ix->nblk8; a.nq = (int)nq;
    if (qraw) {
        a.qsrc = qraw; a.d = ix->d; a.dp = ix->dp;
        a.normalize = ix->metric == KNN_METRIC_COSINE ? 1 : 0;
        a.qpad = const_cast<float*>(qpad); a.qnorm_out = const_cast<float*>(qnorm); a.qresid = ix->q8r;
    } else {
        a.qcodes = ix->q8; a.qscales = ix->q8s; a.qnorm = qnorm;
    }
    a.km = p.km;
    a.nsplit = p.nsplit; a.l2 = kmetric; a.id_offset = ix->id_offset; a.cand_d = ix->cand_d;
    a.cand_i = ix->cand_i; a.ncand = ncand; a.raw16 = raw ? 1 : 0;
    if (p.nsplit == 2 * ix->cus) a.half_k = ix->i8_half_k;
    if (ix->i8_pool64 > 0 && nq <= 2 && p.km == 16 &&
        (ix->i8_pool_forced || (nq == 1 && p.nsplit == ix->cus))) {
        if (!ix->i8_dyn) {
            if ((rc = ix->i8_dyn.reserve(2)) != KNN_OK) return rc;
            KNN_HIP(hipMemsetAsync(ix->i8_dyn, 0, 2 * sizeof(int), st));
        }
        a.dyn = ix->i8_dyn;
        a.pool = (int)((ix->ntotal + 7) / 8 * ix->i8_pool64 / 64);
        a.pool_ch = ix->i8_pool_ch;
        a.half_k = 0;
    }
    if (direct) {
        if ((rc = ix->tail_ctl.reserve((size_t)4 + round_up(nq, 32) / 32)) != KNN_OK)
            return rc;
        a.zero_ctl = ix->tail_ctl;
        if ((rc = ix->heads.reserve((size_t)nq * p.nsplit)) != KNN_OK) return rc;
        a.heads = ix->heads;
    }
    KNN_TIMED(ix, st, launch_i8_scan(a, st));
    const int nlists = p.nsplit;
    RerankArgs r = rerank_args(ix, kModeI8, qpad, qnorm, nq, k, kc, D, I);
    r.c_split = i8_acc_coef(ix->nblk8);
    r.q_resid = ix->q8r; r.xr_max = ix->x8r_max;
    r.raw_d = ix->cand_d; r.raw_i = ix->cand_i; r.raw_lists = raw ? 16 * nlists : nlists;
    r.raw_km = p.km;
    r.raw_stride_q = ncand;
    if (direct) {
        r.direct = 1;
        r.heads = ix->heads;
        r.heads_n = nlists;
    } else if ((rc = merge_for_rerank(ix, nq, nlists, p.km, ncand, false, &r, st)) != KNN_OK) {
        return rc;
    }
    return certify_chunk(ix, r, qpad, qnorm, nq, k, D, I, st, first);
}

int split_chunk(knn_index* ix, const Plan& p, const float* qpad, const float* qnorm, int64_t nq, int k,
                float* D, int64_t* I, hipStream_t st, bool first) {
    const int kmetric = kmetric_of(ix);
    const int kc = p.km;
    int rc;
    if ((rc = ensure_split(ix, st)) != KNN_OK) return rc;
    if ((rc = refresh_maxima(ix, st)) != KNN_OK) return rc;
    if ((rc = ix->qsplit.reserve((size_t)p.nq_pad * ix->dp)) != KNN_OK) return rc;
    if ((rc = grow_cand(ix, nq, p.ncand, kc, false)) != KNN_OK) return rc;
    if ((rc = grow_stats(ix, nq, st)) != KNN_OK) return rc;
    KNN_HIP(launch_split_rows(qpad, p.nq_pad, ix->dp, kSplitBK, ix->qsplit, st));
    TileArgs a{};
    a.wr = p.wr; a.wq = p.wq; a.km = kc;
    a.xb = reinterpret_cast<const float*>(ix->xs.get()); a.xnorm = ix->xn; a.nrows = (int)ix->ntotal;
    a.dp = ix->dp; a.qp = reinterpret_cast<const float*>(ix->qsplit.get()); a.qnorm = qnorm;
    a.nq = (int)nq; a.metric = kmetric; a.ntiles = p.ntiles; a.nsplit = p.nsplit; a.nqb = p.nqb;
    a.id_offset = ix->id_offset; a.cand_d = ix->cand_d; a.cand_i = ix->cand_i;
    a.ncand = p.ncand; a.mode = kModeSplit;
    a.wb = kSplitWB; a.sbk = kSplitBK;
    KNN_TIMED(ix, st, launch_tile_topk(a, st));
    KNN_HIP(launch_merge(ix->cand_d, ix->cand_i, nq, p.ncand / kc, kc, p.ncand, kc, kc, 1, 0,
                         ix->cand2_d, ix->cand2_i, st));
    RerankArgs r = rerank_args(ix, kModeSplit, qpad, qnorm, nq, k, kc, D, I);
    r.cd = ix->cand2_d; r.ci = ix->cand2_i;
    r.c_split = split_coef(ix->dp);
    r.raw_d = ix->cand_d; r.raw_i = ix->cand_i; r.raw_lists = p.ncand / kc; r.raw_km = kc;
    r.raw_stride_q = p.ncand;
    return certify_chunk(ix, r, qpad, qnorm, nq, k, D, I, st, first);
}
// ... 92 lines not shown
```

### include/imgrec_knn.h

```cpp
#ifndef IMGREC_KNN_H
#define IMGREC_KNN_H

#include <stdint.h>

#ifdef __cplusplus
extern "C" {
#endif

typedef struct knn_index knn_index_t;

enum knn_metric {
    KNN_METRIC_IP = 0,
    KNN_METRIC_L2 = 1,
    KNN_METRIC_COSINE = 2
};

enum knn_error {
    KNN_OK = 0,
    KNN_EINVAL = -1,
    KNN_EHIP = -2,
    KNN_ENOMEM = -3,
    KNN_EIO = -4,
    KNN_ENOSYS = -5
};

enum knn_search_mode {
    KNN_SEARCH_AUTO = 0,
    KNN_SEARCH_EXACT = 1,
    KNN_SEARCH_SPLIT = 2,
    KNN_SEARCH_BF16 = 3,
    KNN_SEARCH_I8 = 4
};

#define KNN_MAX_K 32
#define KNN_MAX_K_LARGE 1024

int knn_create(int d, int metric, int device, knn_index_t** out);
int knn_create_multi(int d, int metric, const int* devices, int ndev, knn_index_t** out);
int knn_num_shards(const knn_index_t* index);
int knn_free(knn_index_t* index);

int knn_dim(const knn_index_t* index);
int knn_metric(const knn_index_t* index);
int64_t knn_ntotal(const knn_index_t* index);
int knn_is_trained(const knn_index_t* index);

int knn_set_id_offset(knn_index_t* index, int64_t id_offset);

int knn_train(knn_index_t* index, const float* x, int64_t n);

int knn_add(knn_index_t* index, const float* x_host, int64_t n);
int knn_add_device(knn_index_t* index, const float* x_dev, int64_t n, void* stream);
int knn_reserve(knn_index_t* index, int64_t n);
int knn_reset(knn_index_t* index);

int knn_remove_ids(knn_index_t* index, const uint8_t* bitmap_host, int64_t nbits, int64_t* nremoved);

int knn_reconstruct_n(const knn_index_t* index, int64_t i0, int64_t n, float* x_host);

int knn_search(knn_index_t* index, const float* q_host, int64_t nq, int k,
               float* D_host, int64_t* I_host);
int knn_search_device(knn_index_t* index, const float* q_dev, int64_t nq, int k,
                      float* D_dev, int64_t* I_dev, void* stream);

typedef struct knn_range_result knn_range_result_t;
int knn_range_search(knn_index_t* index, const float* q_host, int64_t nq, float radius,
                     knn_range_result_t** out);
int knn_range_search_device(knn_index_t* index, const float* q_dev, int64_t nq, float radius,
                            void* stream, knn_range_result_t** out);
int64_t knn_range_nq(const knn_range_result_t* result);
int64_t knn_range_size(const knn_range_result_t* result);
int knn_range_copy(const knn_range_result_t* result, int64_t* lims, float* D, int64_t* I);
int knn_range_device(const knn_range_result_t* result, const int64_t** lims, const float** D,
                     const int64_t** I);
int knn_range_free(knn_range_result_t* result);

int knn_search_filtered(knn_index_t* index, const float* q_host, int64_t nq, int k,
                        const uint8_t* bitmap_host, int64_t nbits, float* D_host, int64_t* I_host);
int knn_search_filtered_device(knn_index_t* index, const float* q_dev, int64_t nq, int k,
                               const uint8_t* bitmap_dev, int64_t nbits, float* D_dev,
                               int64_t* I_dev, void* stream);

int knn_merge_device(const float* cand_D, const int64_t* cand_I, int nlists, int64_t nq, int kin,
                     int k, int metric, float* D_dev, int64_t* I_dev, void* stream);

int64_t knn_packed_bytes(int64_t nq, int k);
int knn_merge_packed_device(const void* packed, int nlists, int64_t nq, int kin, int k, int metric,
                            float* D_dev, int64_t* I_dev, void* stream);

int knn_write(const knn_index_t* index, const char* path);
int knn_read(const char* path, int device, knn_index_t** out);
int knn_read_multi(const char* path, const int* devices, int ndev, knn_index_t** out);

int knn_normalize_L2(float* x_host, int64_t n, int d);

int knn_set_timing(knn_index_t* index, int enable);

enum knn_fence_mode { KNN_FENCE_EAGER = 0, KNN_FENCE_LAZY = 1 };
int knn_set_fence_mode(knn_index_t* index, int mode);
int knn_kernel_time(knn_index_t* index, double* total_ms, int* launches);

int knn_set_search_mode(knn_index_t* index, int mode);
int knn_search_stats(knn_index_t* index, int64_t* split_queries, int64_t* fallback_queries,
                     float* max_err_ratio);
int knn_search_stats2(knn_index_t* index, int64_t* split_queries, int64_t* fallback_queries,
                      int64_t* second_chance_queries, float* max_err_ratio);

int knn_last_path(const knn_index_t* index);

int knn_large_k_fallbacks(const knn_index_t* index, int64_t* queries);

int knn_plan(const knn_index_t* index, int64_t nq, int k, int* tile_rows, int* tile_queries,
             int* splits, int* workgroups);

int knn_plan_kernel(const knn_index_t* index, int64_t nq, int k, char* name, int cap);

int knn_debug_i8tail(knn_index_t* index, int* head, int* dpt, int64_t i0, int64_t n, int8_t* codes,
                     float* scales, float* stats);

const char* knn_last_error(void);
const char* knn_version(void);

#ifdef __cplusplus
}
#endif

#endif
```

Baseline: 492,400 queries/s.

## Store int8 tail and bf16 head in one joint row buffer

The int8-tail copy now holds each row as one joint buffer: the int8 tail codes followed by the bf16 head words. The tile kernel streams a single source with one row stride instead of switching between the bf16 matrix and the separate tail matrix per stage. This removes per-stage pointer and offset selection and the second stream of row addresses, at the cost of duplicating the bf16 head inside the tail buffer and using more memory. It also adds loop-timing instrumentation behind a stamps macro and a debug accessor for the joint rows.

```diff
diff --git a/image_recommender_amd/_lib.py b/image_recommender_amd/_lib.py
--- a/image_recommender_amd/_lib.py
+++ b/image_recommender_amd/_lib.py
@@ -93,6 +93,7 @@
     "knn_search_stats2": (_i, [_vp, _pi64, _pi64, _pi64, _pf]),
     "knn_last_path": (_i, [_vp]),
     "knn_debug_i8tail": (_i, [_vp, _pi, _pi, _i64, _i64, _vp, _vp, _vp]),
+    "knn_debug_i8tail_rows": (_i, [_vp, _i64, _i64, _pi, _vp]),
     "knn_large_k_fallbacks": (_i, [_vp, C.POINTER(_i64)]),
     "knn_last_error": (C.c_char_p, []),
     "knn_version": (C.c_char_p, []),
diff --git a/image_recommender_amd/csrc/knn_b16w.hip b/image_recommender_amd/csrc/knn_b16w.hip
--- a/image_recommender_amd/csrc/knn_b16w.hip
+++ b/image_recommender_amd/csrc/knn_b16w.hip
@@ -6,6 +6,7 @@
 #include <type_traits>
 
 #include "knn_kernels.h"
+#include "knn_plan.h"
 #include "lds_dma.h"
 #include "wave_ops.h"
 
@@ -152,16 +153,21 @@
 __device__ unsigned long long g_b16w_wg[2 * 1024];
 #define B16W_STAMP(slot) do { if (stamp_on && lane == 0) { \
     unsigned long long v_ = __builtin_amdgcn_s_memtime(); g_b16w_stamps[wave * 256 + (slot)] = v_; } } while (0)
+__device__ unsigned long long g_b16w_loop[6 * 1024];
+#define B16W_LOOP_BEGIN() const unsigned long long lc0_ = __builtin_amdgcn_s_memtime(), \
+                                                   lr0_ = __builtin_amdgcn_s_memrealtime()
+#define B16W_LOOP_END(kind, n) do { lp_cyc[kind] += __builtin_amdgcn_s_memtime() - lc0_; \
+    lp_rt[kind] += __builtin_amdgcn_s_memrealtime() - lr0_; lp_n[kind] += (unsigned long long)(n); } while (0)
 #else
 #define B16W_STAMP(slot) do {} while (0)
+#define B16W_LOOP_BEGIN() do {} while (0)
+#define B16W_LOOP_END(kind, n) do {} while (0)
 #endif
 
 struct I8TailArgs {
-    const uint32_t* xt = nullptr;
     const float* xts = nullptr;
-    const uint32_t* qt = nullptr;
     const float* qts = nullptr;
-    int dwt = 0, nst_t = 0, nst_h = 0;
+    int nst_t = 0;
 };
 
 template <int KM, int L2, bool PACK>
@@ -198,27 +204,27 @@
     if (!off_ok((int64_t)a.dp * 4)) return hipErrorInvalidValue;
     const bool i8t = a.xt != nullptr;
     I8TailArgs ta;
-    if (i8t) {
-        if (a.t_head < 0 || a.t_head % 64 != 0 || a.t_head > 2 * a.dp || a.t_dpt < 128 || a.t_dpt % 128 != 0 ||
-            !a.xts || !a.qt || !a.qts || !off_ok(a.t_dpt))
-            return hipErrorInvalidValue;
-        ta.xt = reinterpret_cast<const uint32_t*>(a.xt);
-        ta.xts = a.xts;
-        ta.qt = reinterpret_cast<const uint32_t*>(a.qt);
-        ta.qts = a.qts;
-        ta.dwt = a.t_dpt / 4;
-        ta.nst_t = a.t_dpt / 128;
-        ta.nst_h = a.t_head / 64;
-    }
     const dim3 grid((unsigned)(a.nqb * a.nsplit)), block(kNW * 64);
     const uint32_t* xh = reinterpret_cast<const uint32_t*>(a.xb);
     const uint32_t* qh = reinterpret_cast<const uint32_t*>(a.qp);
+    int dw = a.dp;
+    if (i8t) {
+        if (a.t_head < 0 || a.t_head % 64 != 0 || a.t_head > 2 * a.dp || a.t_dpt < 128 || a.t_dpt % 128 != 0 ||
+            !a.xts || !a.qt || !a.qts || !off_ok(i8t_joint_row_bytes(a.t_head, a.t_dpt)))
+            return hipErrorInvalidValue;
+        xh = reinterpret_cast<const uint32_t*>(a.xt);
+        qh = reinterpret_cast<const uint32_t*>(a.qt);
+        dw = i8t_joint_row_bytes(a.t_head, a.t_dpt) / 4;
+        ta.xts = a.xts;
+        ta.qts = a.qts;
+        ta.nst_t = i8t_tail_stages(a.t_dpt);
+    }
     if (a.ib < 0 || a.ib > kB16PackMaxIB) return hipErrorInvalidValue;
 #define IMGREC_LAUNCH_B16W(KMV, L2V, PK)                                                             \
     do {                                                                                             \
         if (i8t)                                                                                     \
             hipLaunchKernelGGL((knn_b16w_tile_kernel_i8t<KMV, L2V, PK>), grid, block, 0, st, xh,    \
-                               a.xnorm, a.nrows, a.dp, qh, a.qnorm, a.nq, a.nsplit, a.nqb,           \
+                               a.xnorm, a.nrows, dw, qh, a.qnorm, a.nq, a.nsplit, a.nqb,             \
                                a.id_offset, a.cand_d, a.cand_i, a.ncand, a.ib, a.sbound, ta);        \
         else                                                                                         \
             hipLaunchKernelGGL((knn_b16w_tile_kernel<KMV, L2V, PK>), grid, block, 0, st, xh,        \
@@ -249,4 +255,7 @@
 extern "C" int knn_b16w_wg_read(unsigned long long* host) {
     return (int)hipMemcpyFromSymbol(host, HIP_SYMBOL(imgrec::g_b16w_wg), sizeof(imgrec::g_b16w_wg));
 }
-#endif
+extern "C" int knn_b16w_loop_read(unsigned long long* host) {
+    return (int)hipMemcpyFromSymbol(host, HIP_SYMBOL(imgrec::g_b16w_loop), sizeof(imgrec::g_b16w_loop));
+}
+#endif
diff --git a/image_recommender_amd/csrc/knn_b16w_body.inc b/image_recommender_amd/csrc/knn_b16w_body.inc
--- a/image_recommender_amd/csrc/knn_b16w_body.inc
+++ b/image_recommender_amd/csrc/knn_b16w_body.inc
@@ -5,6 +5,7 @@
 #ifdef IMGREC_B16_STAMPS
     const int wg = blockIdx.x;
     if (threadIdx.x == 0 && wg < 1024) g_b16w_wg[2 * wg] = __builtin_amdgcn_s_memrealtime();
+    unsigned long long lp_cyc[2] = {0, 0}, lp_rt[2] = {0, 0}, lp_n[2] = {0, 0};
 #endif
     const int wgid = xcd_wgid();
     constexpr int kG = 4;
@@ -57,27 +58,13 @@
     const int pbase = (isA ? wave : wave - 4) * kLPW;
     const int prow = lane / kCPR, pchk = lane % kCPR;
     static_assert(kRPP == 8 && kRPB == 2 && kLPW % 2 == 0, "piece offset form");
-#if B16W_I8T
-    auto vpar_of = [&](int e, int words) {
-        int ln = lane;
-        asm volatile("" : "+v"(ln));
-        const int prow = ln / kCPR, pchk = ln % kCPR;
-#else
     uint32_t vpar[2];
 #pragma unroll
     for (int e = 0; e < 2; ++e) {
-#endif
         const int P = pbase + e, r = P * kRPP + prow;
         const int srow = isA ? P * nsplit * kRPP + prow : r;
-#if B16W_I8T
-        return (uint32_t)srow * (uint32_t)(words * 4) + 16u * (uint32_t)(pchk ^ ((r / kRPB) % kCPR));
-    };
-    uint32_t vpar[2] = {0u, 0u};
-    if constexpr (!I8T) { vpar[0] = vpar_of(0, dw); vpar[1] = vpar_of(1, dw); }
-#else
         vpar[e] = (uint32_t)srow * (uint32_t)(dw * 4) + 16u * (uint32_t)(pchk ^ ((r / kRPB) % kCPR));
     }
-#endif
     const uint32_t kPS = (uint32_t)((isA ? nsplit : 1) * kRPP * dw * 4);
     auto voff_of = [&](int j) {
         return vpar[j & 1] + (uint32_t)(j & ~1) * kPS - 1024u * (uint32_t)(j & 3);
@@ -115,73 +102,41 @@
         dma2_agent(wrec, smem0 + (uint32_t)(kRecOff + wave * (kQW * kSBWords * 4)), (uint32_t)lane * 16u);
     };
 
-#if B16W_I8T
-    const int nst_t = I8T ? ta.nst_t : 0;
-    const int nst = I8T ? ta.nst_t + ta.nst_h : dw / kBKW;
-#else
     const int nst = dw / kBKW;
+#if B16W_I8T
+    const int nst_t = ta.nst_t;
 #endif
     const int total = (t1 - t0) * nst;
     const uint32_t* qblk = qh + (size_t)qb * kBQ * dw;
-#if B16W_I8T
-    const uint32_t* qblk_t = I8T ? ta.qt + (size_t)qb * kBQ * ta.dwt : nullptr;
-#endif
 
     int c_it = t0, c_is = 0;
     const uint32_t* c_tile = isA ? xh + (size_t)trow(t0, 0) * dw : qblk;
-#if B16W_I8T
-    const uint32_t* c_tile_t = !I8T ? nullptr : isA ? ta.xt + (size_t)trow(t0, 0) * ta.dwt : qblk_t;
-#endif
     int c_ng = (isA && t0 == t1 - 1) ? cnt - t0 * kGPT : kGPT;
     auto issue = [&](int g) __attribute__((always_inline)) {
 #if B16W_I8T
-        const bool tl = I8T && c_is < nst_t;
-        const uint32_t* src;
-        uint32_t vp0 = 0u, vp1 = 0u, ps = 0u;
-        if constexpr (I8T) {
-            const int rw = tl ? ta.dwt : dw;
-            src = tl ? c_tile_t + c_is * kBKW : c_tile + (c_is - nst_t) * kBKW;
-            vp0 = vpar_of(0, rw);
-            vp1 = vpar_of(1, rw);
-            ps = (uint32_t)((isA ? nsplit : 1) * kRPP * rw * 4);
-        } else {
-            src = c_tile + c_is * kBKW;
-        }
-        auto voff = [&](int j) {
-            if constexpr (I8T) return ((j & 1) ? vp1 : vp0) + (uint32_t)(j & ~1) * ps - 1024u * (uint32_t)(j & 3);
-            else return voff_of(j);
+        uint32_t vp[2] = {vpar[0], vpar[1]};
+        if constexpr (!PACK) asm volatile("" : "+v"(vp[0]), "+v"(vp[1]));
+        auto voff_of = [&](int j) {
+            return vp[j & 1] + (uint32_t)(j & ~1) * kPS - 1024u * (uint32_t)(j & 3);
         };
-#else
+#endif
         const uint32_t* src = c_tile + c_is * kBKW;
-#endif
         const uint32_t dst = smem0 + (uint32_t)((g & (kNS - 1)) * kStage) + pdst;
         if (pbase + kLPW <= c_ng || !isA) {
 #pragma unroll
             for (int h = 0; h < kLPW / 4; ++h)
-#if B16W_I8T
-                dma4x(src, dst + 4096u * h, voff(4 * h), voff(4 * h + 1), voff(4 * h + 2),
-                      voff(4 * h + 3));
-#else
                 dma4x(src, dst + 4096u * h, voff_of(4 * h), voff_of(4 * h + 1), voff_of(4 * h + 2),
                       voff_of(4 * h + 3));
-#endif
         } else {
 #pragma unroll
             for (int j = 0; j < kLPW; ++j)
                 if (pbase + j < c_ng) {
                     const uint32_t d = dst + 4096u * (j / 4);
                     switch (j & 3) {
-#if B16W_I8T
-                        case 0: dma1<0>(src, d, voff(j)); break;
-                        case 1: dma1<1024>(src, d, voff(j)); break;
-                        case 2: dma1<2048>(src, d, voff(j)); break;
-                        default: dma1<3072>(src, d, voff(j)); break;
-#else
                         case 0: dma1<0>(src, d, voff_of(j)); break;
                         case 1: dma1<1024>(src, d, voff_of(j)); break;
                         case 2: dma1<2048>(src, d, voff_of(j)); break;
                         default: dma1<3072>(src, d, voff_of(j)); break;
-#endif
                     }
                 }
         }
@@ -199,9 +154,6 @@
             ++c_it;
             if (isA) {
                 c_tile = xh + (size_t)trow(c_it, 0) * dw;
-#if B16W_I8T
-                if constexpr (I8T) c_tile_t = ta.xt + (size_t)trow(c_it, 0) * ta.dwt;
-#endif
                 c_ng = c_it == t1 - 1 ? cnt - c_it * kGPT : kGPT;
             }
         }
@@ -338,7 +290,7 @@
         auto tile_stages = [&](auto nr_tag) __attribute__((always_inline)) {
             if constexpr (I8T) {
                 constexpr int NR = decltype(nr_tag)::value;
-                stage_loop(nr_tag, std::true_type{}, nst_t, 0, nst > nst_t);
+                { B16W_LOOP_BEGIN(); stage_loop(nr_tag, std::true_type{}, nst_t, 0, nst > nst_t); B16W_LOOP_END(0, nst_t); }
                 const float* scl = reinterpret_cast<const float*>(smem + kScaleOff + ((t - t0) % kNormSlots) * kBM * 4);
                 const float sq[2] = {lsq[lc], lsq[lc + 16]};
 #pragma unroll
@@ -353,7 +305,7 @@
                     }
                     asm volatile("" : "+v"(acc[rb][0]), "+v"(acc[rb][1]));
                 }
-                stage_loop(nr_tag, std::false_type{}, nst - nst_t, nst_t, false);
+                { B16W_LOOP_BEGIN(); stage_loop(nr_tag, std::false_type{}, nst - nst_t, nst_t, false); B16W_LOOP_END(1, nst - nst_t); }
             } else {
                 stage_loop(nr_tag, std::false_type{}, nst, 0, false);
 #else
@@ -369,10 +321,16 @@
         else if (nlive == 2) tile_stages(std::integral_constant<int, 2>{});
         else tile_stages(std::integral_constant<int, 1>{});
 #else
+#ifdef IMGREC_B16_STAMPS
+        B16W_LOOP_BEGIN();
+#endif
         if (nlive >= 4) stage_loop(std::integral_constant<int, 4>{});
         else if (nlive == 3) stage_loop(std::integral_constant<int, 3>{});
         else if (nlive == 2) stage_loop(std::integral_constant<int, 2>{});
         else stage_loop(std::integral_constant<int, 1>{});
+#ifdef IMGREC_B16_STAMPS
+        B16W_LOOP_END(1, nst);
+#endif
 #endif
 
         B16W_STAMP(2 * (t - t0));
@@ -537,6 +495,13 @@
 
 #ifdef IMGREC_B16_STAMPS
     if (threadIdx.x == 0 && wg < 1024) g_b16w_wg[2 * wg + 1] = __builtin_amdgcn_s_memrealtime();
+    if (threadIdx.x == 0 && wg < 1024)
+#pragma unroll
+        for (int i = 0; i < 2; ++i) {
+            g_b16w_loop[6 * wg + 3 * i] = lp_cyc[i];
+            g_b16w_loop[6 * wg + 3 * i + 1] = lp_rt[i];
+            g_b16w_loop[6 * wg + 3 * i + 2] = lp_n[i];
+        }
 #endif
 #pragma unroll
     for (int x = 32; x >= 16; x >>= 1) {
diff --git a/image_recommender_amd/csrc/knn_capi.cpp b/image_recommender_amd/csrc/knn_capi.cpp
--- a/image_recommender_amd/csrc/knn_capi.cpp
+++ b/image_recommender_amd/csrc/knn_capi.cpp
@@ -52,7 +52,7 @@
     if (all || ix->x8) cols[n++] = {&ix->x8, (size_t)i8_row_bytes(ix->nblk8)};
     if (all || ix->x8) cols[n++] = {&ix->x8s, (size_t)ix->nblk8 * sizeof(float)};
     if (all || ix->x8) cols[n++] = {&ix->x8r, sizeof(float)};
-    if (all || ix->xt) cols[n++] = {&ix->xt, (size_t)ix->xt_dpt};
+    if (all || ix->xt) cols[n++] = {&ix->xt, (size_t)ix->xt_row};
     if (all || ix->xt) cols[n++] = {&ix->xts, sizeof(float)};
     if (all || ix->xt) cols[n++] = {&ix->xtm, sizeof(float4)};
     return n;
@@ -122,7 +122,7 @@
         KNN_HIP(launch_i8_rows(xb, n, ix->dp, ix->nblk8, (int8_t*)at(kColX8), (float*)at(kColX8s),
                                (float*)at(kColX8r), st));
     if (ix->xt) {
-        KNN_HIP(launch_i8tail_rows(xb, n, ix->dp, ix->dpb, ix->xt_head, ix->xt_dpt, (int8_t*)at(kColXt),
+        KNN_HIP(launch_i8tail_rows(xb, n, ix->dp, ix->dpb, ix->xt_head, ix->xt_dpt, ix->xt_row, (int8_t*)at(kColXt),
                                    (float*)at(kColXts), (float4*)at(kColXtm), st));
         ix->xt_tried = false;
     }
@@ -167,15 +167,16 @@
     if (head < 0) { ix->xt_state = TailCopy::Ineligible; return KNN_OK; }
     ix->xt_head = head;
     ix->xt_dpt = (int)round_up(ix->dpb - head, 128);
-    if (materialise_columns(ix, kColXt, 3) != KNN_OK) {
+    ix->xt_row = i8t_joint_row_bytes(head, ix->xt_dpt);
+    if (ix->xt_alloc_fail || materialise_columns(ix, kColXt, 3) != KNN_OK) {
         drop_i8tail(ix, TailCopy::Ineligible);
         return KNN_OK;
     }
-    KNN_HIP(hipMemsetAsync(ix->xt, 0, (size_t)ix->cap * ix->xt_dpt, st));
+    KNN_HIP(hipMemsetAsync(ix->xt, 0, (size_t)ix->cap * ix->xt_row, st));
     KNN_HIP(hipMemsetAsync(ix->xts, 0, (size_t)ix->cap * sizeof(float), st));
     KNN_HIP(hipMemsetAsync(ix->xtm, 0, (size_t)ix->cap * sizeof(float4), st));
     ix->xn_max_stale = true;
-    KNN_HIP(launch_i8tail_rows(ix->xb, ix->ntotal, ix->dp, ix->dpb, head, ix->xt_dpt, ix->xt, ix->xts,
+    KNN_HIP(launch_i8tail_rows(ix->xb, ix->ntotal, ix->dp, ix->dpb, head, ix->xt_dpt, ix->xt_row, ix->xt, ix->xts,
                                ix->xtm, st));
     ix->xt_state = TailCopy::Built;
     return KNN_OK;
@@ -183,7 +184,7 @@
 
 void drop_i8tail(knn_index* ix, TailCopy next) {
     ix->xt.reset(); ix->xts.reset(); ix->xtm.reset();
-    ix->xt_head = ix->xt_dpt = 0;
+    ix->xt_head = ix->xt_dpt = ix->xt_row = 0;
     ix->xt_tried = false; ix->xt_state = next;
 }
 
@@ -242,6 +243,7 @@
         ix->i8tail = *e != '0';
         ix->xt_no_trial = *e == '2';
     }
+    if (const char* e = test_knob("IMGREC_I8TAIL_ALLOC_FAIL")) ix->xt_alloc_fail = *e != '0';
     if (const char* e = test_knob("IMGREC_RANGE_CAP")) {
         const long long v = std::atoll(e);
         if (v > 0) ix->range_cap0 = (size_t)v;
@@ -772,10 +774,29 @@
             rc = HipStreams::fail(hipMemcpyAsync(dst, (const char*)src + (size_t)i0 * row, (size_t)n * row,
                                                  hipMemcpyDeviceToHost, ix->stream), "hipMemcpyAsync");
     };
-    down(codes, ix->xt.get(), (size_t)ix->xt_dpt);
+    if (rc == KNN_OK && codes && n > 0)
+        rc = HipStreams::fail(hipMemcpy2DAsync(codes, (size_t)ix->xt_dpt,
+                                               (const char*)ix->xt.get() + (size_t)i0 * ix->xt_row,
+                                               (size_t)ix->xt_row, (size_t)ix->xt_dpt, (size_t)n,
+                                               hipMemcpyDeviceToHost, ix->stream), "hipMemcpy2DAsync");
     down(scales, ix->xts.get(), sizeof(float));
     down(stats, ix->xtm.get(), sizeof(float4));
     return op.finish(rc);
 }
 
-}
+int knn_debug_i8tail_rows(knn_index_t* ix, int64_t i0, int64_t n, int* row_bytes, uint8_t* rows) {
+    if (!ix) KNN_FAIL(KNN_EINVAL, "index is NULL");
+    if (ix->multi) KNN_FAIL(KNN_EINVAL, "knn_debug_i8tail_rows: single-device indexes only");
+    IndexOp op(ix);
+    if (ix->xt_state != TailCopy::Built || !ix->xt) KNN_FAIL(KNN_EINVAL, "the index has no int8 tail copy");
+    if (i0 < 0 || n < 0 || i0 + n > ix->ntotal) KNN_FAIL(KNN_EINVAL, "rows outside [0, ntotal)");
+    if (row_bytes) *row_bytes = ix->xt_row;
+    int rc = op.begin_host();
+    if (rc == KNN_OK && rows && n > 0)
+        rc = HipStreams::fail(hipMemcpyAsync(rows, (const char*)ix->xt.get() + (size_t)i0 * ix->xt_row,
+                                             (size_t)n * ix->xt_row, hipMemcpyDeviceToHost, ix->stream),
+                              "hipMemcpyAsync");
+    return op.finish(rc);
+}
+
+}
diff --git a/image_recommender_amd/csrc/knn_index.h b/image_recommender_amd/csrc/knn_index.h
--- a/image_recommender_amd/csrc/knn_index.h
+++ b/image_recommender_amd/csrc/knn_index.h
@@ -122,8 +122,10 @@
     DevBuf<float4> xtm;
     DevBuf<float> xt_max;
     int xt_head = 0, xt_dpt = 0;
+    int xt_row = 0;
     bool xt_tried = false;
     bool xt_no_trial = false;
+    bool xt_alloc_fail = false;
     DevBuf<int8_t> qt;
     DevBuf<float> qts;
     DevBuf<float> q_eip;
diff --git a/image_recommender_amd/csrc/knn_kernels.h b/image_recommender_amd/csrc/knn_kernels.h
--- a/image_recommender_amd/csrc/knn_kernels.h
+++ b/image_recommender_amd/csrc/knn_kernels.h
@@ -55,7 +55,7 @@
     float* e_ip = nullptr;
     const float* xt_max = nullptr;
     const float* xn_max = nullptr;
-    int head = 0, dpt = 0;
+    int head = 0, dpt = 0, row = 0;
     float c_acc = 0.f;
 };
 
@@ -201,7 +201,7 @@
                                  hipStream_t st, const SharedBoundPrep* sb = nullptr,
                                  const I8TailPrep* tp = nullptr);
 hipError_t launch_block_absmax(const float* xb, int64_t n, int dp, int nblk, float* out, hipStream_t st);
-hipError_t launch_i8tail_rows(const float* xb, int64_t n, int dp, int dpb, int head, int dpt,
+hipError_t launch_i8tail_rows(const float* xb, int64_t n, int dp, int dpb, int head, int dpt, int row_bytes,
                               int8_t* codes, float* scale, float4* stat, hipStream_t st);
 hipError_t launch_i8tail_max(const float4* stat, int64_t n, float* out, hipStream_t st);
 hipError_t launch_max_norm(const float* xn, int64_t n, float* out, hipStream_t st);
diff --git a/image_recommender_amd/csrc/knn_plan.cpp b/image_recommender_amd/csrc/knn_plan.cpp
--- a/image_recommender_amd/csrc/knn_plan.cpp
+++ b/image_recommender_amd/csrc/knn_plan.cpp
@@ -65,6 +65,16 @@
         return dpb - head >= kI8TMinTail && head <= dpb / 2 ? head : -1;
     }
     return -1;
+}
+
+int i8t_joint_row_bytes(int head, int dpt) {
+    if (head < 0 || head % 64 != 0 || dpt < kI8TStageBytes || dpt % kI8TStageBytes != 0) return -1;
+    return dpt + 2 * head;
+}
+int i8t_tail_stages(int dpt) { return dpt / kI8TStageBytes; }
+int i8t_row_stages(int head, int dpt) {
+    const int rb = i8t_joint_row_bytes(head, dpt);
+    return rb < 0 ? -1 : rb / kI8TStageBytes;
 }
 
 float i8_acc_coef(int nblk) {
diff --git a/image_recommender_amd/csrc/knn_plan.h b/image_recommender_amd/csrc/knn_plan.h
--- a/image_recommender_amd/csrc/knn_plan.h
+++ b/image_recommender_amd/csrc/knn_plan.h
@@ -26,6 +26,10 @@
 float i8t_acc_coef(int head);
 int i8t_pick_head(const float* blkmax, int nblk);
 constexpr int kI8TMinTail = 512;
+int i8t_joint_row_bytes(int head, int dpt);
+int i8t_tail_stages(int dpt);
+int i8t_row_stages(int head, int dpt);
+constexpr int kI8TStageBytes = 128;
 constexpr int kI8MaxQ = 8;
 float i8_acc_coef(int nblk);
 Plan make_i8_plan(int64_t ntotal, int64_t nq, int k, int cus, int wgpcu, int nblk);
diff --git a/image_recommender_amd/csrc/knn_refine.hip b/image_recommender_amd/csrc/knn_refine.hip
--- a/image_recommender_amd/csrc/knn_refine.hip
+++ b/image_recommender_amd/csrc/knn_refine.hip
@@ -111,32 +111,36 @@
 
 __global__ void __launch_bounds__(256)
 i8tail_rows_kernel(const float* __restrict__ src, int64_t n, int dp, int dpb, int head, int dpt,
-                   int8_t* __restrict__ codes, float* __restrict__ scales, float4* __restrict__ stat) {
+                   int row_bytes, int8_t* __restrict__ codes, float* __restrict__ scales, float4* __restrict__ stat) {
     const int64_t row = (int64_t)blockIdx.x * 4 + (threadIdx.x >> 6);
     const int lane = threadIdx.x & 63;
     if (row >= n) return;
     const float* x = src + row * dp;
     const int hc = head / 8;
     float amax = 0.f, nh = 0.f, nt = 0.f, rh = 0.f, rt = 0.f;
+    int8_t* oc = codes + row * row_bytes;
     for (int c = lane; c < dpb / 8; c += 64) {
         float e[8];
         load_chunk8(x, c, dp, e);
+        uint32_t hw[4] = {0u, 0u, 0u, 0u};
 #pragma unroll
         for (int t = 0; t < 8; ++t) {
             if (c < hc) {
-                const float r = e[t] - __uint_as_float(bf16_rne(e[t]) << 16);
+                const uint32_t hb = bf16_rne(e[t]);
+                const float r = e[t] - __uint_as_float(hb << 16);
                 nh = fmaf(e[t], e[t], nh);
                 rh = fmaf(r, r, rh);
+                hw[t >> 1] |= hb << (16 * (t & 1));
             } else {
                 nt = fmaf(e[t], e[t], nt);
                 amax = fmaxf(amax, fabsf(e[t]));
             }
         }
+        if (c < hc) *reinterpret_cast<uint4*>(oc + dpt + 16 * c) = make_uint4(hw[0], hw[1], hw[2], hw[3]);
     }
 #pragma unroll
     for (int off = 32; off > 0; off >>= 1) amax = fmaxf(amax, __shfl_xor(amax, off, 64));
     const float sc = amax / 127.f, inv = amax > 0.f ? 127.f / amax : 0.f;
-    int8_t* oc = codes + row * dpt;
     for (int c = hc + lane; c < hc + dpt / 8; c += 64) {
         uint32_t w[2] = {0u, 0u};
         if (c < dpb / 8) {
@@ -267,28 +271,32 @@
     if (tp.codes) {
         const int hc = tp.head / 8;
         float amax = 0.f, nh = 0.f, nt = 0.f, rh = 0.f;
+        int8_t* oc = tp.codes + row * tp.row;
 #pragma unroll
         for (int it = 0; it < IT; ++it) {
             const int c = lane + 64 * it;
             if (8 * c >= dpb) continue;
+            uint32_t hw[4] = {0u, 0u, 0u, 0u};
 #pragma unroll
             for (int t = 0; t < 8; ++t) {
                 const float v = normalize ? e[it][t] * scale : e[it][t];
                 if (c < hc) {
-                    const float r = v - __uint_as_float(bf16_rne(v) << 16);
+                    const uint32_t hb = bf16_rne(v);
+                    const float r = v - __uint_as_float(hb << 16);
                     nh = fmaf(v, v, nh);
                     rh = fmaf(r, r, rh);
+                    hw[t >> 1] |= hb << (16 * (t & 1));
                 } else {
                     nt = fmaf(v, v, nt);
                     amax = fmaxf(amax, fabsf(v));
                 }
             }
+            if (c < hc) *reinterpret_cast<uint4*>(oc + tp.dpt + 16 * c) = make_uint4(hw[0], hw[1], hw[2], hw[3]);
         }
 #pragma unroll
         for (int off = 32; off > 0; off >>= 1) amax = fmaxf(amax, __shfl_xor(amax, off, 64));
         const float sc = amax / 127.f, inv = amax > 0.f ? 127.f / amax : 0.f;
         float rt = 0.f;
-        int8_t* oc = tp.codes + row * tp.dpt;
 #pragma unroll
         for (int it = 0; it < IT; ++it) {
             const int c = lane + 64 * it;
@@ -796,7 +804,7 @@
     if (dpb % 8 != 0 || dp % 16 != 0 || dpb < dp || dp < d) return hipErrorInvalidValue;
     if (tp && tp->codes &&
         (tp->head % 64 != 0 || tp->head < 0 || tp->head >= dpb || tp->dpt % 128 != 0 ||
-         tp->dpt < dpb - tp->head || !tp->scale || !tp->e_ip || !tp->xt_max || !tp->xn_max))
+         tp->dpt < dpb - tp->head || tp->row != tp->dpt + 2 * tp->head || !tp->scale || !tp->e_ip || !tp->xt_max || !tp->xn_max))
         return hipErrorInvalidValue;
     const dim3 grid((unsigned)((n_pad + 3) / 4)), block(256);
 #define IMGREC_QPREP(ITV) hipLaunchKernelGGL((query_prep_b16_kernel<ITV>), grid, block, 0, st, src, n, \
@@ -819,14 +827,14 @@
     return hipGetLastError();
 }
 
-hipError_t launch_i8tail_rows(const float* xb, int64_t n, int dp, int dpb, int head, int dpt,
+hipError_t launch_i8tail_rows(const float* xb, int64_t n, int dp, int dpb, int head, int dpt, int row_bytes,
                               int8_t* codes, float* scale, float4* stat, hipStream_t st) {
     if (n <= 0) return hipSuccess;
     if (dpb % 64 != 0 || dp % 8 != 0 || dpb < dp || head % 64 != 0 || head < 0 || head >= dpb ||
-        dpt % 128 != 0 || dpt < dpb - head)
+        dpt % 128 != 0 || dpt < dpb - head || row_bytes != dpt + 2 * head)
         return hipErrorInvalidValue;
     hipLaunchKernelGGL(i8tail_rows_kernel, dim3((unsigned)((n + 3) / 4)), dim3(256), 0, st, xb, n, dp, dpb,
-                       head, dpt, codes, scale, stat);
+                       head, dpt, row_bytes, codes, scale, stat);
     return hipGetLastError();
 }
 
diff --git a/image_recommender_amd/csrc/knn_search.cpp b/image_recommender_amd/csrc/knn_search.cpp
--- a/image_recommender_amd/csrc/knn_search.cpp
+++ b/image_recommender_amd/csrc/knn_search.cpp
@@ -256,12 +256,12 @@
     int rc;
     if ((rc = ensure_i8tail(ix, st)) != KNN_OK || ix->xt_state != TailCopy::Built) return rc;
     if ((rc = refresh_maxima(ix, st)) != KNN_OK) return rc;
-    if ((rc = ix->qt.reserve((size_t)p.nq_pad * ix->xt_dpt)) != KNN_OK) return rc;
+    if ((rc = ix->qt.reserve((size_t)p.nq_pad * ix->xt_row)) != KNN_OK) return rc;
     if ((rc = ix->qts.reserve((size_t)p.nq_pad)) != KNN_OK) return rc;
     if ((rc = ix->q_eip.reserve((size_t)p.nq_pad)) != KNN_OK) return rc;
     tp->codes = ix->qt; tp->scale = ix->qts; tp->e_ip = ix->q_eip;
     tp->xt_max = ix->xt_max; tp->xn_max = ix->xn_max;
-    tp->head = ix->xt_head; tp->dpt = ix->xt_dpt;
+    tp->head = ix->xt_head; tp->dpt = ix->xt_dpt; tp->row = ix->xt_row;
     tp->c_acc = i8t_acc_coef(ix->xt_head);
     return KNN_OK;
 }
diff --git a/include/imgrec_knn.h b/include/imgrec_knn.h
--- a/include/imgrec_knn.h
+++ b/include/imgrec_knn.h
@@ -117,6 +117,7 @@
 
 int knn_debug_i8tail(knn_index_t* index, int* head, int* dpt, int64_t i0, int64_t n, int8_t* codes,
                      float* scales, float* stats);
+int knn_debug_i8tail_rows(knn_index_t* index, int64_t i0, int64_t n, int* row_bytes, uint8_t* rows);
 
 const char* knn_last_error(void);
 const char* knn_version(void);
```

Measured after the change: 534,700 queries/s (median of 6 runs). 1.09x the previous value.
